# HpWang-whu/RoReg

Hardware: AMD Instinct MI355X
Metric: pair-registrations/sec (higher is better)
Workload: dtype f32 (every f32 operand enters the fp16 matrix cores as hi + lo fp16 under a per-keypoint power-of-two block scale: <= 22 significant bits relative to a CONSERVATIVE per-keypoint bound -- measured on the extractor: the bound sits 2^2..2^6 above the keypoint's true coefficient maximum (config.f16x2_sc

## Files before the change

include/roreg_hip.h:

```cpp
#ifndef ROREG_HIP_H
#define ROREG_HIP_H

#include <stdint.h>
#include <stddef.h>

#ifdef __cplusplus
extern "C" {
#endif

#define ROREG_ABI_VERSION 6
int roreg_abi_version(void);
const char *roreg_last_error(void);

int roreg_set_group_tables(const int32_t *P_host, const int32_t *Nei_host, const double *R_host);

size_t roreg_group_conv_packed_size(int Cin, int Cout, int KS);
int roreg_group_conv_pack_weights(const float *W_host , int Cin, int Cout, int KS,
                                  float *wpack_host );
size_t roreg_group_conv_workspace_size(int B, int Cin, int Cout, int Lin, int Lout, int KS);
int roreg_group_conv(const float *x, const float *wpack, const float *bias,
                     const float *bn_scale, const float *bn_shift, const float *residual,
                     float *out, const int32_t *gather,
                     int B, int Cin, int Cout, int Lin, int Lout, int KS,
                     float *workspace, size_t workspace_floats, void *stream);

int roreg_group_conv_split(const float *x, const void *wsplit, const float *bias, const float *bn_scale, const float *bn_shift,
                           float *out, const int32_t *gather,
                           const int32_t *lds_order , int lds_stride,
                           int B, int Cin, int Cout, int Lin, int Lout, int KS, void *stream);

int roreg_dense_split(const float *x, const void *wsplit, const float *bias, const float *scale, const float *shift,
                      const float *residual, int residual_stride, float *out, int B, int K, int O, void *stream);

int roreg_group_conv_f16x2(const float *x, const void *wsplit2, int w_exp, const float *bias, const float *bn_scale, const float *bn_shift,
                           float act_smax, float act_tmax, const float *in_rowmax_dev, float *out, float *out_rowmax_dev,
                           const int32_t *gather, const int32_t *lds_order , int lds_stride,
                           int B, int Cin, int Cout, int Lin, int Lout, int KS, void *stream);
int roreg_dense_f16x2(const float *x, const void *wsplit2, int w_exp, const float *bias, const float *scale, const float *shift,
                      float act_smax, float act_tmax, const float *in_rowmax_dev, const float *residual, int residual_stride, float *out,
                      float *out_rowmax_dev, int B, int K, int O, void *stream);
int roreg_group_conv_f16x2_packed(const uint32_t *x_words, const void *wsplit2, int w_exp, const float *bias, const float *in_bound_dev,
                                  float *out, float *out_rowmax_dev, const int32_t *gather, const int32_t *lds_order, int lds_stride,
                                  int B, int Cin, int Cout, int Lin, int Lout, int KS, void *stream);

int roreg_gf_finalize(const float *eqv_raw, void *eqv, int eqv_bf16 ,
                      float *inv, int B, void *stream);

int roreg_det_score(const float *enc, float *scores, int B, void *stream);

int roreg_inv_descriptor(const void *eqv, int eqv_bf16 , float *inv, int N,
                         void *stream);

int roreg_nn_search(const float *src, const int64_t *src_rows, int m,
                    const float *tgt, const int64_t *tgt_rows, int n, int F,
                    int64_t *idx_out, float *dist_out, uint64_t *scratch, void *stream);

int roreg_nn_search_ex(const float *src, const int64_t *src_rows, int m,
                       const float *tgt, const int64_t *tgt_rows, int n, int F, int squared,
                       int64_t *idx_out, float *dist_out, uint64_t *scratch, void *stream);

int roreg_pdist(const float *A, int m, const float *B, int n, int F, int squared, float *out, void *stream);

typedef struct {
    const float *desc0, *desc1;
    const int64_t *rows0, *rows1;
    int32_t m0, m1;
} roreg_match_task;
size_t roreg_mutual_match_batch_workspace(int n_tasks, int max_m);
int roreg_mutual_match_batch(const roreg_match_task *tasks_dev, int n_tasks, int max_m, int64_t *match_out, int32_t *counts_out,
                             void *workspace, size_t workspace_bytes, void *stream);

size_t roreg_knn_search_workspace(int m, int n);
int roreg_knn_search(const float *src, int m, const float *tgt, int n, int F, int k,
                     int64_t *idx_out, void *workspace , size_t workspace_bytes, void *stream);

int roreg_knn_search_ex(const float *src, int m, const float *tgt, int n, int F, int k, int squared, int64_t *idx_out, float *dist_out,
                        void *workspace, size_t workspace_bytes, void *stream);

size_t roreg_knn_search_seg_workspace(long long m_total, int n_seg, int max_m, int max_n);
int roreg_knn_search_seg(const float *src, const float *tgt, const int32_t *seg_src, const int32_t *seg_tgt, int n_seg, long long m_total,
                         int max_m, int max_n, int F, int k, int64_t *idx_out, void *workspace, size_t workspace_bytes, void *stream);

int roreg_mutual_matches(const int64_t *nn01, const int64_t *nn10, int m, int n ,
                         const int64_t *sample0, const int64_t *sample1,
                         int64_t *match_out, int32_t *count_out, void *stream);

int roreg_des2r(const float *feats1, const int64_t *rows1, const float *feats0, const int64_t *rows0,
                int M, int64_t *idx_out, float *cor_out, void *stream);

int roreg_group_corr(const float *perm_feats, const int64_t *perm_rows, const float *bcast_feats, const int64_t *bcast_rows,
                     int M, int transpose_table, int64_t *idx_out, float *cor_out, void *stream);

int roreg_group_corr_mfma(const float *perm_feats, const int64_t *perm_rows, const float *bcast_feats, const int64_t *bcast_rows, int M,
                          int transpose_table, float *cor_out, void *stream);

int roreg_set_des2r_tables(int transpose_table , const uint8_t *ia_host,
                           const uint8_t *ib_host, const uint8_t *cnt_host, const float *NT_host);
int roreg_group_corr_irrep(const float *perm_coefs, const int64_t *perm_rows, const float *bcast_coefs, const int64_t *bcast_rows, int M,
                           int transpose_table, float *cor_out, void *stream);
int roreg_des2r_irrep(const float *coef1, const int64_t *rows1, const float *coef0, const int64_t *rows0, const void *feats1,
                      const void *feats0, int feat_bf16, int M, int64_t *idx_out, void *stream);
int roreg_des2r_recheck_count(int reset, int32_t *count_out);
int roreg_feat_coefs(const void *x, int x_bf16, float *out, int B, int C, int split, void *stream);

int roreg_et_gather(const void *before0, const void *before1, const void *after0, const void *after1,
                    int feat_bf16 ,
                    const int64_t *rows0, const int64_t *rows1, const int64_t *pre_idx, int M,
                    float *x_out, void *stream);

int roreg_quat_to_trans(const float *q, const int64_t *anchor, const double *keys0, const int64_t *rows0,
                        const double *keys1, const int64_t *rows1, int M,
                        double *Trans_out, float *quat_out, void *stream);

int roreg_ransac_score(const double *k0, const double *k1, const double *w, int w_f32, int M,
                       const double *Trans, const int64_t *hyp_rows, int H, double ird,
                       double *overlap_out, int32_t *best_out, uint8_t *mask_out, void *stream);

int roreg_refine(const double *k0, const double *k1, const double *w, int w_f32, int M,
                 const double *T_in, int t_in_stride ,
                 const double *Trans, const int64_t *hyp_rows, const int32_t *best,
                 double dist, double *T_out, double *stats_out ,
                 void *stream);

typedef struct {
    const void *before0, *before1, *after0, *after1;
    const double *keys0, *keys1;
    const int64_t *matches;
    const int64_t *sel;
    int32_t n, pad_;
    int64_t off;
    const float *coef0, *coef1;
} roreg_lt_task;
int roreg_lt_prepare_batch(const roreg_lt_task *tasks_dev, int n_tasks, int max_n, int flags, int64_t *dr_out, float *x_out,
                           const float *bn_scale , const float *bn_shift, float *x_bound_out , void *stream);
int roreg_lt_finish_batch(const roreg_lt_task *tasks_dev, int n_tasks, int max_n, const float *q_all, const int64_t *dr_all,
                          double *Trans_out, void *stream);
int roreg_role_max(const void *before, const void *after, int feat_bf16, const float *bn_scale , const float *bn_shift, float *out,
                   int N, void *stream);
int roreg_row_bound_roles(const void *x_spatial, int x_bf16, float *bound_out, const float *role_scale, const float *role_shift, float *role_out, int B,
                          void *stream);
int roreg_inv_descriptor_roles(const void *eqv, int eqv_bf16, float *inv, const float *role_scale, const float *role_shift, float *role_out, int N,
                               void *stream);
int roreg_lt_prepare_rows(const roreg_lt_task *tasks_dev, const float *const *roles_dev, int n_tasks, int max_n, int flags, int64_t *dr_out,
                          uint64_t *rows_out, float *x_bound_out, void *stream);

typedef struct {
    const double *keys0, *keys1;
    const int64_t *matches;
    const double *w;
    const double *Trans;
    const int64_t *hyp_rows;
    int32_t M, H;
    int64_t koff;
} roreg_ransac_task;
size_t roreg_ransac_batch_workspace(int n_tasks, long long total_M, int max_H);
int roreg_ransac_batch(const roreg_ransac_task *tasks_dev, int n_tasks, long long total_M, int max_M, int max_H, double ird,
                       int w_f32 ,
                       int32_t *best_out, double *T1_out, double *stats1_out, double *T2_out, double *stats2_out,
                       void *workspace, size_t workspace_bytes, void *stream);

int roreg_refine_batch(const roreg_ransac_task *tasks_dev, const int32_t *sel_dev, int n_sel, long long total_M, const double *T_in,
                       double dist, int w_f32, double *T_out, double *stats_out, const void *workspace, void *stream);

int roreg_mt_shuffle_prefix(const uint32_t *seeds, int n_jobs, const int32_t *sizes, int per_job, int take, int64_t *out, int n_threads);

int roreg_mt_stream_shuffle_prefix(uint32_t *key, int32_t *pos, const int32_t *sizes, int n_lists, int take, int64_t *out);

int roreg_yohoc_draw(const uint32_t *words, long long n_words, const double *cdf, const int32_t *bin_size, int max_iter, int max_tries,
                     int32_t *bin_out, int64_t *pick_out, int32_t *n_hyp_out, long long *words_used);

typedef struct {
    const void *src;
    const int64_t *rows;
    void *dst;
    int32_t n, pad_;
} roreg_gather_task;
int roreg_gather_rows_batch(const roreg_gather_task *tasks_dev, int n_tasks, int max_n, int row_bytes, void *stream);

int roreg_gather_rows_f64(const double *src, const int64_t *rows, int M, int width, double *out, void *stream);

size_t roreg_topk_dot_workspace_size(int m, int n, int k);
int roreg_topk_dot(const float *A, int m, const float *B, int n, int k, int64_t *idx_out, float *val_out ,
                   float *ws, size_t ws_floats, const int32_t *segA, const int32_t *segB, int n_seg, int max_m, int max_n, void *stream);

int roreg_linear(const float *x, int L, int Cin, const float *W , const float *b, int Cout, float *y, void *stream);
int roreg_linear_path(int path);
int roreg_linear_cat3(const float *pos , const float *table , const int64_t *idx ,
                      const float *conf , int m, int k, const float *W , const float *b, int Cout, float *y, void *stream);
int roreg_linear_mfma(const float *x, int L, int Cin, const float *W , const float *b, int Cout, float *y, void *stream);

int roreg_instnorm_stats(const float *h, int L, int C, float eps, float *mean_rstd, double *ws, const int32_t *seg_off, int n_seg,
                         int mult, void *stream);

int roreg_mlp_tail(const float *h, int L, int Cmid, const float *mean_rstd, const float *W2 , const float *b2,
                   float *y, const int32_t *seg_off, int n_seg, int mult, void *stream);
int roreg_mlp_tail_mfma(const float *h, int L, int Cmid, const float *mean_rstd, const float *W2 , const float *b2,
                   float *y, const int32_t *seg_off, int n_seg, int mult, void *stream);

int roreg_context_colmax(const float *R, int L, const int32_t *seg_off, int n_seg, int max_len, float *ctx_out, float *ws, void *stream);

int roreg_knn_attention(const float *qp, const float *kp, const float *vp, const int64_t *idx, int k_is_table, int v_is_table,
                        int m, int k, float *x_out, void *stream);

int roreg_rm_elementwise(int op, const float *a, const float *b, const float *c, const int64_t *idx, int L, int k, int C,
                         float *out, float *ws, void *stream);

size_t roreg_sinkhorn_workspace_size(int m, int n);
int roreg_sinkhorn(const float *src_final, int m, const float *tgt_final, int n, float alpha, int iters, float *Z_out,
                   int64_t *matches0, int64_t *matches1, float *mscores0, float *mscores1, float *ws, size_t ws_floats, void *stream);

size_t roreg_sinkhorn_batch_workspace_size(int n_seg, int max_m, int max_n, long long total_m, long long total_n);
int roreg_sinkhorn_batch_consts(const int32_t *seg_src_host, const int32_t *seg_tgt_host, int n_seg, float *consts_host);
int roreg_sinkhorn_batch(const float *src_final, const float *tgt_final, const int32_t *seg_src, const int32_t *seg_tgt,
                         const int32_t *seg_src_host, const int32_t *seg_tgt_host, const float *consts, int n_seg, float alpha, int iters,
                         int64_t *matches0, int64_t *matches1, float *mscores0, float *mscores1, float *ws, size_t ws_floats,
                         void *stream);

size_t roreg_sinkhorn_batch2_workspace_size(int n_seg, int max_m, int max_n, long long total_m, long long total_n);
int roreg_sinkhorn_batch2(const float *src_final, const float *tgt_final, const int32_t *seg_src, const int32_t *seg_tgt,
                          const int32_t *seg_src_host, const int32_t *seg_tgt_host, const float *consts, int n_seg, float alpha, int iters,
                          int64_t *matches0, int64_t *matches1, float *mscores0, float *mscores1, float *ws, size_t ws_floats,
                          int recompute, void *stream);
size_t roreg_sinkhorn_batch3_workspace_size(int n_seg, int max_m, int max_n, long long total_m, long long total_n, int recompute, int want_Z);
int roreg_sinkhorn_batch3(const float *src_final, const float *tgt_final, const int32_t *seg_src, const int32_t *seg_tgt,
                          const int32_t *seg_src_host, const int32_t *seg_tgt_host, const float *consts, int n_seg, float alpha, int iters,
                          int64_t *matches0, int64_t *matches1, float *mscores0, float *mscores1, float *ws, size_t ws_floats,
                          int recompute, float *Z_out, void *stream);
int roreg_write_files(const char *const *paths, const void *const *headers, const int32_t *header_len, const void *const *data,
                      const int64_t *nbytes, int n, int n_threads);
int roreg_yohoc_draw_many(const uint32_t *seeds, int n_pairs, const int64_t *anchors, const int64_t *offsets, int max_iter, int max_tries,
                          int64_t *rows_out, int32_t *n_hyp_out, double *giveup_out, int n_threads);
size_t roreg_mlp_head_workspace(int L, int n_seg, int C1);
int roreg_mlp_head(const float *x, const float *pos, const float *table, const int64_t *idx, const float *conf, int m, int k, int L, int Cin,
                   const float *W1, const float *b1, int C1, const float *Wr, const float *br, float *h, float *y, const int32_t *seg_off,
                   int n_seg, int mult, float eps, float *mean_rstd, double *ws, void *stream);
int roreg_sinkhorn_early_exit(int on);
int roreg_sinkhorn_iteration_stats(long long *iterations, long long *pairs, int reset, void *stream);

int roreg_set_fourier_tables(const float *F_host);
size_t roreg_irrep_gemm_tiles(int O, int B, int32_t *tiles_host);
size_t roreg_irrep_gemm_tiles_m(int O, int B, int tile_m , int32_t *tiles_host);
int roreg_irrep_gemm(const float *const *X, float *const *Out, const float *const *Add, const float *const *Wpack, int C, int O, int B,
                     const int32_t *tiles_dev, int n_tiles, void *stream);
int roreg_irrep_gemm_split(const float *const *X, float *const *Out, const float *const *Add, const void *const *Wsplit, int C, int O, int B,
                           const int32_t *tiles_dev, int n_tiles, void *stream);
int roreg_irrep_gemm_f16x2(const float *const *X, float *const *Out, const float *const *Add, const void *const *Wsplit2,
                           const float *x_bound_dev, int w_exp, const float *next_u_dev, const float *next_v_dev, float *out_bound_dev,
                           int C, int O, int B, const int32_t *tiles_dev, int n_tiles,
                           int tile_m ,
                           int x_planes , void *stream);
int roreg_gemm_persistent(int on);
int roreg_row_bound(const void *x_spatial, int x_bf16 , const float *bn_scale, const float *bn_shift,
                    float *bound_out, int B, int C, void *stream);
int roreg_ft_nonlin(const float *Xin , const float *x_spatial, const float *bias,
                    const float *bias2, const float *bn_scale, const float *bn_shift, const float *resid_spatial,
                    float *Xout , float *out_spatial ,
                    const int32_t *g_map ,
                    int Lout , int Lvalid,
                    int B, int C, int split ,
                    const float *out_bound ,
                    float *out_rowmax ,
                    int spatial_bf16 ,
                    int out_planes ,
                    void *stream);
int roreg_ft_nonlin_packed(const float *Xin, const float *bias, const float *bn_scale, const float *bn_shift, uint32_t *out_words,
                           const int32_t *g_map, int Lout, int Lvalid, int B, int C, const float *out_bound, float *raw_col, int raw_g,
                           void *stream);
int roreg_ft_nonlin_gathered(const uint64_t *rows , const int64_t *dr , int feat_bf16, const float *bn_scale ,
                             const float *bn_shift, float *Xout, int B, const float *out_bound , int out_planes, void *stream);

typedef struct roreg_icp_grid_desc {
    double origin[3];
    double edge;
    int32_t dims[3];
    int32_t n;
    int64_t cells;
    int64_t reserved;
} roreg_icp_grid_desc;
size_t roreg_icp_grid_size(const double *lo_host, const double *hi_host, int n, double max_dist, roreg_icp_grid_desc *desc_host,
                           size_t *workspace_bytes);
int roreg_icp_grid_build(const float *points, const roreg_icp_grid_desc *desc_host, void *grid, void *workspace, size_t workspace_bytes,
                         void *stream);
typedef struct roreg_icp_task {
    const void *tgt_grid;
    const void *src_grid;
    const double *T0;
    int32_t n_src;
    int32_t slot0;
} roreg_icp_task;
size_t roreg_icp_batch_workspace(int n_tasks, long long total_slots);
int roreg_icp_batch(const roreg_icp_task *tasks, int n_tasks, const int32_t *work, int n_work, long long total_slots, double max_dist,
                    int max_iter, double tol_deg, double tol_t, double *T_out, int32_t *iters_out, int32_t *inliers_out, double *rmse_out,
                    int32_t *status_out, int32_t *assign_out, double *stats_out, void *workspace, size_t workspace_bytes, void *stream);

int roreg_profile_enable(int on);
int roreg_profile_read(int slot, double *total_ms, int *launches);

#ifdef __cplusplus
}
#endif
#endif
```

roreg_amd/_abi.py:

```python
import ctypes
from ctypes import c_int, c_void_p, c_size_t, c_double, c_float, c_char_p

import numpy as np

ABI_VERSION = 6

_P = c_void_p
PROTOTYPES = {
    'roreg_abi_version': (c_int, []),
    'roreg_last_error': (c_char_p, []),
    'roreg_set_group_tables': (c_int, [_P, _P, _P]),
    'roreg_group_conv_packed_size': (c_size_t, [c_int, c_int, c_int]),
    'roreg_group_conv_pack_weights': (c_int, [_P, c_int, c_int, c_int, _P]),
    'roreg_group_conv_workspace_size': (c_size_t, [c_int, c_int, c_int, c_int, c_int, c_int]),
    'roreg_group_conv': (c_int, [_P, _P, _P, _P, _P, _P, _P, _P, c_int, c_int, c_int, c_int, c_int, c_int, _P, c_size_t, _P]),
    'roreg_group_conv_split': (c_int, [_P, _P, _P, _P, _P, _P, _P, _P, c_int, c_int, c_int, c_int, c_int, c_int, c_int, _P]),
    'roreg_group_conv_f16x2': (c_int, [_P, _P, c_int, _P, _P, _P, c_float, c_float, _P, _P, _P, _P, _P, c_int, c_int, c_int, c_int, c_int, c_int, c_int, _P]),
    'roreg_group_conv_f16x2_packed': (c_int, [_P, _P, c_int, _P, _P, _P, _P, _P, _P, c_int, c_int, c_int, c_int, c_int, c_int, c_int, _P]),
    'roreg_dense_f16x2': (c_int, [_P, _P, c_int, _P, _P, _P, c_float, c_float, _P, _P, c_int, _P, _P, c_int, c_int, c_int, _P]),
    'roreg_dense_split': (c_int, [_P, _P, _P, _P, _P, _P, c_int, _P, c_int, c_int, c_int, _P]),
    'roreg_gf_finalize': (c_int, [_P, _P, c_int, _P, c_int, _P]),
    'roreg_det_score': (c_int, [_P, _P, c_int, _P]),
    'roreg_inv_descriptor': (c_int, [_P, c_int, _P, c_int, _P]),
    'roreg_nn_search': (c_int, [_P, _P, c_int, _P, _P, c_int, c_int, _P, _P, _P, _P]),
    'roreg_nn_search_ex': (c_int, [_P, _P, c_int, _P, _P, c_int, c_int, c_int, _P, _P, _P, _P]),
    'roreg_pdist': (c_int, [_P, c_int, _P, c_int, c_int, c_int, _P, _P]),
    'roreg_knn_search_workspace': (c_size_t, [c_int, c_int]),
    'roreg_knn_search': (c_int, [_P, c_int, _P, c_int, c_int, c_int, _P, _P, c_size_t, _P]),
    'roreg_knn_search_ex': (c_int, [_P, c_int, _P, c_int, c_int, c_int, c_int, _P, _P, _P, c_size_t, _P]),
    'roreg_knn_search_seg_workspace': (c_size_t, [ctypes.c_longlong, c_int, c_int, c_int]),
    'roreg_knn_search_seg': (c_int, [_P, _P, _P, _P, c_int, ctypes.c_longlong, c_int, c_int, c_int, c_int, _P, _P, c_size_t, _P]),
    'roreg_mutual_matches': (c_int, [_P, _P, c_int, c_int, _P, _P, _P, _P, _P]),
    'roreg_mutual_match_batch_workspace': (c_size_t, [c_int, c_int]),
    'roreg_mutual_match_batch': (c_int, [_P, c_int, c_int, _P, _P, _P, c_size_t, _P]),
    'roreg_des2r': (c_int, [_P, _P, _P, _P, c_int, _P, _P, _P]),
    'roreg_set_des2r_tables': (c_int, [c_int, _P, _P, _P, _P]),
    'roreg_group_corr_irrep': (c_int, [_P, _P, _P, _P, c_int, c_int, _P, _P]),
    'roreg_group_corr_mfma': (c_int, [_P, _P, _P, _P, c_int, c_int, _P, _P]),
    'roreg_des2r_irrep': (c_int, [_P, _P, _P, _P, _P, _P, c_int, c_int, _P, _P]),
    'roreg_des2r_recheck_count': (c_int, [c_int, _P]),
    'roreg_feat_coefs': (c_int, [_P, c_int, _P, c_int, c_int, c_int, _P]),
    'roreg_et_gather': (c_int, [_P, _P, _P, _P, c_int, _P, _P, _P, c_int, _P, _P]),
    'roreg_quat_to_trans': (c_int, [_P, _P, _P, _P, _P, _P, c_int, _P, _P, _P]),
    'roreg_ransac_score': (c_int, [_P, _P, _P, c_int, c_int, _P, _P, c_int, c_double, _P, _P, _P, _P]),
    'roreg_refine': (c_int, [_P, _P, _P, c_int, c_int, _P, c_int, _P, _P, _P, c_double, _P, _P, _P]),
    'roreg_lt_prepare_batch': (c_int, [_P, c_int, c_int, c_int, _P, _P, _P, _P, _P, _P]),
    'roreg_lt_finish_batch': (c_int, [_P, c_int, c_int, _P, _P, _P, _P]),
    'roreg_role_max': (c_int, [_P, _P, c_int, _P, _P, _P, c_int, _P]),
    'roreg_row_bound_roles': (c_int, [_P, c_int, _P, _P, _P, _P, c_int, _P]),
    'roreg_inv_descriptor_roles': (c_int, [_P, c_int, _P, _P, _P, _P, c_int, _P]),
    'roreg_lt_prepare_rows': (c_int, [_P, _P, c_int, c_int, c_int, _P, _P, _P, _P]),
    'roreg_ransac_batch_workspace': (c_size_t, [c_int, ctypes.c_longlong, c_int]),
    'roreg_ransac_batch': (c_int, [_P, c_int, ctypes.c_longlong, c_int, c_int, c_double, c_int, _P, _P, _P, _P, _P, _P, c_size_t, _P]),
    'roreg_refine_batch': (c_int, [_P, _P, c_int, ctypes.c_longlong, _P, ctypes.c_double, c_int, _P, _P, _P, _P]),
    'roreg_yohoc_draw': (c_int, [_P, ctypes.c_longlong, _P, _P, c_int, c_int, _P, _P, _P, _P]),
    'roreg_gather_rows_batch': (c_int, [_P, c_int, c_int, c_int, _P]),
    'roreg_gather_rows_f64': (c_int, [_P, _P, c_int, c_int, _P, _P]),
    'roreg_group_corr': (c_int, [_P, _P, _P, _P, c_int, c_int, _P, _P, _P]),
    'roreg_topk_dot_workspace_size': (c_size_t, [c_int, c_int, c_int]),
    'roreg_topk_dot': (c_int, [_P, c_int, _P, c_int, c_int, _P, _P, _P, c_size_t, _P, _P, c_int, c_int, c_int, _P]),
    'roreg_context_colmax': (c_int, [_P, c_int, _P, c_int, c_int, _P, _P, _P]),
    'roreg_sinkhorn_batch_workspace_size': (c_size_t, [c_int, c_int, c_int, ctypes.c_longlong, ctypes.c_longlong]),
    'roreg_sinkhorn_batch_consts': (c_int, [_P, _P, c_int, _P]),
    'roreg_sinkhorn_batch': (c_int, [_P, _P, _P, _P, _P, _P, _P, c_int, c_float, c_int, _P, _P, _P, _P, _P, c_size_t, _P]),
    'roreg_sinkhorn_batch2_workspace_size': (c_size_t, [c_int, c_int, c_int, ctypes.c_longlong, ctypes.c_longlong]),
    'roreg_sinkhorn_batch2': (c_int, [_P, _P, _P, _P, _P, _P, _P, c_int, c_float, c_int, _P, _P, _P, _P, _P, c_size_t, c_int, _P]),
    'roreg_sinkhorn_batch3_workspace_size': (c_size_t, [c_int, c_int, c_int, ctypes.c_longlong, ctypes.c_longlong, c_int, c_int]),
    'roreg_sinkhorn_batch3': (c_int, [_P, _P, _P, _P, _P, _P, _P, c_int, c_float, c_int, _P, _P, _P, _P, _P, c_size_t, c_int, _P, _P]),
    'roreg_write_files': (c_int, [_P, _P, _P, _P, _P, c_int, c_int]),
    'roreg_yohoc_draw_many': (c_int, [_P, c_int, _P, _P, c_int, c_int, _P, _P, _P, c_int]),
    'roreg_mlp_head_workspace': (c_size_t, [c_int, c_int, c_int]),
    'roreg_mlp_head': (c_int, [_P, _P, _P, _P, _P, c_int, c_int, c_int, c_int, _P, _P, c_int, _P, _P, _P, _P, _P, c_int, c_int, c_float, _P, _P, _P]),
    'roreg_sinkhorn_early_exit': (c_int, [c_int]),
    'roreg_sinkhorn_iteration_stats': (c_int, [_P, _P, c_int, _P]),
    'roreg_linear': (c_int, [_P, c_int, c_int, _P, _P, c_int, _P, _P]),
    'roreg_linear_mfma': (c_int, [_P, c_int, c_int, _P, _P, c_int, _P, _P]),
    'roreg_linear_path': (c_int, [c_int]),
    'roreg_linear_cat3': (c_int, [_P, _P, _P, _P, c_int, c_int, _P, _P, c_int, _P, _P]),
    'roreg_gemm_persistent': (c_int, [c_int]),
    'roreg_instnorm_stats': (c_int, [_P, c_int, c_int, c_float, _P, _P, _P, c_int, c_int, _P]),
    'roreg_mlp_tail': (c_int, [_P, c_int, c_int, _P, _P, _P, _P, _P, c_int, c_int, _P]),
    'roreg_mlp_tail_mfma': (c_int, [_P, c_int, c_int, _P, _P, _P, _P, _P, c_int, c_int, _P]),
    'roreg_knn_attention': (c_int, [_P, _P, _P, _P, c_int, c_int, c_int, c_int, _P, _P]),
    'roreg_rm_elementwise': (c_int, [c_int, _P, _P, _P, _P, c_int, c_int, c_int, _P, _P, _P]),
    'roreg_sinkhorn_workspace_size': (c_size_t, [c_int, c_int]),
    'roreg_sinkhorn': (c_int, [_P, c_int, _P, c_int, c_float, c_int, _P, _P, _P, _P, _P, _P, c_size_t, _P]),
    'roreg_icp_grid_size': (c_size_t, [_P, _P, c_int, c_double, _P, _P]),
    'roreg_icp_grid_build': (c_int, [_P, _P, _P, _P, c_size_t, _P]),
    'roreg_icp_batch_workspace': (c_size_t, [c_int, ctypes.c_longlong]),
    'roreg_icp_batch': (c_int, [_P, c_int, _P, c_int, ctypes.c_longlong, c_double, c_int, c_double, c_double, _P, _P, _P, _P, _P, _P, _P, _P, c_size_t, _P]),
    'roreg_profile_enable': (c_int, [c_int]),
    'roreg_profile_read': (c_int, [c_int, _P, _P]),
    'roreg_set_fourier_tables': (c_int, [_P]),
    'roreg_mt_shuffle_prefix': (c_int, [_P, c_int, _P, c_int, c_int, _P, c_int]),
    'roreg_mt_stream_shuffle_prefix': (c_int, [_P, _P, _P, c_int, c_int, _P]),
    'roreg_irrep_gemm_tiles': (c_size_t, [c_int, c_int, _P]),
    'roreg_irrep_gemm_tiles_m': (c_size_t, [c_int, c_int, c_int, _P]),
    'roreg_irrep_gemm': (c_int, [_P, _P, _P, _P, c_int, c_int, c_int, _P, c_int, _P]),
    'roreg_irrep_gemm_split': (c_int, [_P, _P, _P, _P, c_int, c_int, c_int, _P, c_int, _P]),
    'roreg_irrep_gemm_f16x2': (c_int, [_P, _P, _P, _P, _P, c_int, _P, _P, _P, c_int, c_int, c_int, _P, c_int, c_int, c_int, _P]),
    'roreg_row_bound': (c_int, [_P, c_int, _P, _P, _P, c_int, c_int, _P]),
    'roreg_ft_nonlin': (c_int, [_P, _P, _P, _P, _P, _P, _P, _P, _P, _P, c_int, c_int, c_int, c_int, c_int, _P, _P, c_int, c_int, _P]),
    'roreg_ft_nonlin_packed': (c_int, [_P, _P, _P, _P, _P, _P, c_int, c_int, c_int, c_int, _P, _P, c_int, _P]),
    'roreg_ft_nonlin_gathered': (c_int, [_P, _P, c_int, _P, _P, _P, c_int, _P, c_int, _P]),
}


_RANSAC_TASK = np.dtype([('keys0', np.uint64), ('keys1', np.uint64), ('matches', np.uint64), ('w', np.uint64), ('Trans', np.uint64),
                         ('hyp_rows', np.uint64), ('M', np.int32), ('H', np.int32), ('koff', np.int64)])

_MATCH_TASK = np.dtype([('desc0', np.uint64), ('desc1', np.uint64), ('rows0', np.uint64), ('rows1', np.uint64), ('m0', np.int32), ('m1', np.int32)])

_GATHER_TASK = np.dtype([('src', np.uint64), ('rows', np.uint64), ('dst', np.uint64), ('n', np.int32), ('pad', np.int32)])

_LT_TASK = np.dtype([('before0', np.uint64), ('before1', np.uint64), ('after0', np.uint64), ('after1', np.uint64), ('keys0', np.uint64),
                     ('keys1', np.uint64), ('matches', np.uint64), ('sel', np.uint64), ('n', np.int32), ('pad', np.int32), ('off', np.int64),
                     ('coef0', np.uint64), ('coef1', np.uint64)])

_ICP_GRID_DESC = np.dtype([('origin', np.float64, 3), ('edge', np.float64), ('dims', np.int32, 3), ('n', np.int32), ('cells', np.int64),
                           ('reserved', np.int64)])

_ICP_TASK = np.dtype([('tgt_grid', np.uint64), ('src_grid', np.uint64), ('T0', np.uint64), ('n_src', np.int32), ('slot0', np.int32)])
```

roreg_amd/_hip_fourier.py:

```python
import os
from ctypes import c_void_p

import numpy as np
import torch

from . import hip as _core
from .hip import HipError, _check, _feat, _ptr, _stream, lib

__all__ = ['DenseSplitLayer', 'IRREP_DIMS', 'IRREP_OFFSETS', '_bf16_split3', '_keypoint_of_columns', '_ptr_array', '_res_ptr', '_tile_cache', 'bf16_split3_frags', 'bf16_split3_pack', 'bound_exp', 'coef_pitch', 'coef_size', 'coef_views', 'dense_split', 'ensure_fourier', 'f16_scale_exp', 'f16_split2_frags', 'f16_split2_pack', 'frag_pack', 'ft_nonlin', 'ft_nonlin_gathered', 'ft_nonlin_packed', 'gemm_persistent', 'group_conv_split_pack', 'irrep_gemm', 'next_bound', 'next_bound_spatial', 'pack_coefs_f16x2', 'row_bound', 'unpack_coefs_f16x2', 'words_to_planes']


_fourier_ready = False
IRREP_DIMS = (1, 3, 3, 4, 5)
IRREP_OFFSETS = (0, 1, 10, 19, 35, 60)


def ensure_fourier():
    global _fourier_ready
    if not _fourier_ready:
        from .fourier import group_fourier
        F = np.ascontiguousarray(group_fourier().F, np.float32)
        _check(lib().roreg_set_fourier_tables(F.ctypes.data), 'roreg_set_fourier_tables')
        _fourier_ready = True


def _ptr_array(views):
    arr = (c_void_p * 5)(*[c_void_p(v.data_ptr()) for v in views])
    return arr


def coef_pitch(B):
    return (int(B) + 31) // 32 * 32


def coef_size(C, B):
    return 60 * C * coef_pitch(B)


def coef_views(buf, C, B):
    Bp = coef_pitch(B)
    return [buf[IRREP_OFFSETS[r] * C * Bp:IRREP_OFFSETS[r + 1] * C * Bp].view(IRREP_DIMS[r] * C, IRREP_DIMS[r] * Bp) for r in range(5)]


_tile_cache = {}


def irrep_gemm(X_buf, Wpacks, C, O, B, split=None, add=None, f16x2=None, x_bound=None, next_bound=None, x_planes=False):
    Bp = coef_pitch(B)
    if X_buf.numel() != 60 * C * Bp or (add is not None and add.numel() != 60 * O * Bp):
        raise HipError(f'irrep_gemm: coefficient buffers must hold 60*C*{Bp} floats (B={B} padded to the 32-keypoint pitch)')
    out = torch.empty(60 * O * Bp, dtype=torch.float32, device=X_buf.device)
    tile_m = 256 if (f16x2 is not None and O % 256 == 0 and not os.environ.get('ROREG_TILE_M128')) else 128
    key = (O, Bp, tile_m)
    t = _tile_cache.get(key)
    if t is None:
        n = lib().roreg_irrep_gemm_tiles_m(O, Bp, tile_m, None)
        host = np.empty((n, 3), np.int32)
        lib().roreg_irrep_gemm_tiles_m(O, Bp, tile_m, host.ctypes.data)
        t = torch.from_numpy(host).cuda()
        _tile_cache[key] = t
    xv = coef_views(X_buf, C, B); ov = coef_views(out, O, B)
    av = _ptr_array(coef_views(add, O, B)) if add is not None else None
    if _core.PROFILE is not None:
        e0 = torch.cuda.Event(enable_timing=True); e1 = torch.cuda.Event(enable_timing=True); e0.record()
    bound_out = None
    if f16x2 is not None:
        wl, w_exp = f16x2
        if x_bound is None or x_bound.numel() != Bp:
            raise HipError(f'irrep_gemm: the fp16 x 2 GEMM needs x_bound with one value per (padded) keypoint ({Bp})')
        nu = nv = None
        if next_bound is not None:
            nu, nv = next_bound
            if nu.numel() != O or nv.numel() != O:
                raise HipError('irrep_gemm: next_bound must hold one (u, v) per output channel')
            bound_out = torch.zeros(Bp, dtype=torch.float32, device=X_buf.device)
        _check(lib().roreg_irrep_gemm_f16x2(_ptr_array(xv), _ptr_array(ov), av, _ptr_array(wl), _ptr(x_bound, torch.float32), int(w_exp),
                                            _ptr(nu, torch.float32), _ptr(nv, torch.float32), _ptr(bound_out), C, O, Bp,
                                            _ptr(t, torch.int32), int(t.shape[0]), tile_m, (int(x_planes) if x_planes in (1, 2) and x_planes is not True else (2 if _core.MFMA16 else 1)) if x_planes else 0, _stream()), 'roreg_irrep_gemm_f16x2')
    elif split is not None:
        _check(lib().roreg_irrep_gemm_split(_ptr_array(xv), _ptr_array(ov), av, _ptr_array(split), C, O, Bp, _ptr(t, torch.int32), int(t.shape[0]),
                                            _stream()), 'roreg_irrep_gemm_split')
    else:
        _check(lib().roreg_irrep_gemm(_ptr_array(xv), _ptr_array(ov), av, _ptr_array(Wpacks), C, O, Bp, _ptr(t, torch.int32), int(t.shape[0]), _stream()),
               'roreg_irrep_gemm')
    if _core.PROFILE is not None:
        e1.record(); _core.PROFILE.append((('irrep_gemm_f16x2' if f16x2 is not None else 'irrep_gemm_split' if split is not None else 'irrep_gemm', Bp, C, O), e0, e1))
    return (out, bound_out) if next_bound is not None else out


class gemm_persistent:

    def __init__(self, on=True):
        self.on = int(on)

    def __enter__(self):
        self.prev = lib().roreg_gemm_persistent(self.on)

    def __exit__(self, *exc):
        lib().roreg_gemm_persistent(self.prev)
        return False


def row_bound(x, bn=None, roles=None):
    B, C = int(x.shape[0]), int(x.shape[1])
    out = torch.empty(coef_pitch(B), dtype=torch.float32, device=x.device)
    scale, shift = bn if bn is not None else (None, None)
    xp, bf = _feat(x)
    if roles is not None:
        if bn is not None or C != 32:
            raise HipError('row_bound: roles go with the 32-channel input features and no BatchNorm')
        r_scale, r_shift, role = _core._role_args(roles, B)
        _check(lib().roreg_row_bound_roles(xp, bf, _ptr(out), _ptr(r_scale), _ptr(r_shift), _ptr(role), B, _stream()), 'roreg_row_bound_roles')
        return out
    _check(lib().roreg_row_bound(xp, bf, _ptr(scale), _ptr(shift), _ptr(out), B, C, _stream()), 'roreg_row_bound')
    return out


def _keypoint_of_columns(d, Bp):
    n = torch.arange(d * Bp, device='cuda')
    return ((n // 32) // d) * 32 + (n % 32)


def bound_exp(bound):
    _, ex = torch.frexp(bound.float())
    e = torch.where((bound > 0) & torch.isfinite(bound), 14 - ex, torch.zeros_like(ex))
    return e.clamp(-100, 100)


def pack_coefs_f16x2(X_buf, C, B, bound=None):
    Bp = coef_pitch(B)
    views = coef_views(X_buf, C, B)
    if bound is None:
        bound = torch.zeros(Bp, dtype=torch.float32, device=X_buf.device)
        for r, v in enumerate(views):
            kp = _keypoint_of_columns(IRREP_DIMS[r], Bp)
            bound.scatter_reduce_(0, kp, v.abs().amax(0), 'amax')
    e = bound_exp(bound)
    out = torch.empty_like(X_buf)
    for r, (v, o) in enumerate(zip(views, coef_views(out, C, B))):
        kp = _keypoint_of_columns(IRREP_DIMS[r], Bp)
        y = torch.ldexp(v, e[kp][None, :])
        hi = y.half()
        lo = (y - hi.float()).half()
        w = (hi.view(torch.int16).to(torch.int32) & 0xffff) | (lo.view(torch.int16).to(torch.int32) << 16)
        o.copy_(w.view(torch.float32))
    return out, bound


def words_to_planes(X_words, C, B):
    w = X_words.contiguous().view(torch.int32).view(-1, 2, 16)
    hi = (w & 0xffff).to(torch.int16).transpose(1, 2); lo = (w >> 16).to(torch.int16).transpose(1, 2)
    return torch.cat([hi.reshape(-1, 32), lo.reshape(-1, 32)], 1).contiguous().view(torch.float32).view(-1)


def unpack_coefs_f16x2(X_words, bound, C, B):
    Bp = coef_pitch(B)
    e = bound_exp(bound)
    out = torch.empty_like(X_words)
    for r, (v, o) in enumerate(zip(coef_views(X_words, C, B), coef_views(out, C, B))):
        kp = _keypoint_of_columns(IRREP_DIMS[r], Bp)
        w = v.view(torch.int32)
        hi = (w & 0xffff).to(torch.int16).view(torch.float16).float()
        lo = (w >> 16).to(torch.int16).view(torch.float16).float()
        o.copy_(torch.ldexp(hi + lo, -e[kp][None, :]))
    return out


def next_bound_spatial(bn, bias):
    scale, shift = bn
    sc = scale.detach().double().abs().cpu(); sh = shift.detach().double().abs().cpu()
    b = bias.detach().double().cpu()
    k = 1.0 + 2.0 ** -9
    u = (np.sqrt(60.0) * k) * sc
    v = k * (sc * b.abs() + sh) + 1e-30
    return u.float().cuda().contiguous(), v.float().cuda().contiguous()


def ft_nonlin_packed(B, C, coef_in, bias, bn, out_bound, g_map=None, Lout=60, Lvalid=60, raw_g=None):
    ensure_fourier()
    dev = coef_in.device
    if coef_in.numel() != coef_size(C, B) or out_bound.numel() != coef_pitch(B):
        raise HipError('ft_nonlin_packed: coef_in / out_bound sizes')
    words = torch.empty((B, C, Lout if g_map is not None else 60), dtype=torch.int32, device=dev)
    raw = torch.empty((B, C), dtype=torch.float32, device=dev) if raw_g is not None else None
    scale, shift = bn if bn is not None else (None, None)
    _check(lib().roreg_ft_nonlin_packed(_ptr(coef_in, torch.float32), _ptr(bias), _ptr(scale), _ptr(shift), _ptr(words), _ptr(g_map, torch.int32),
                                        int(Lout), int(Lvalid), B, C, _ptr(out_bound, torch.float32), _ptr(raw), int(raw_g or 0), _stream()),
           'roreg_ft_nonlin_packed')
    return words, raw


def next_bound(bn, bias, bias2=None):
    scale, shift = bn
    sc = scale.detach().double().abs().cpu(); sh = shift.detach().double().abs().cpu()
    b = bias.detach().double().cpu() + (bias2.detach().double().cpu() if bias2 is not None else 0.0)
    k = 1.0 + 2.0 ** -9
    u = (60.0 * k) * sc
    v = (np.sqrt(60.0) * k) * (sc * b.abs() + sh) + 1e-30
    return u.float().cuda().contiguous(), v.float().cuda().contiguous()


def ft_nonlin(B, C, coef_in=None, x_spatial=None, bias=None, bias2=None, bn=None, resid_spatial=None, spatial_out=False,
              g_map=None, Lout=60, Lvalid=60, split=False, out_bound=None, want_rowmax=False, planes=False):
    ensure_fourier()
    dev = (coef_in if coef_in is not None else x_spatial).device
    if spatial_out:
        out = torch.empty((B, C, Lout if g_map is not None else 60), dtype=torch.float32, device=dev); xout = None; osp = _ptr(out)
    else:
        out = torch.empty(coef_size(C, B), dtype=torch.float32, device=dev); xout = _ptr(out); osp = None
    scale, shift = bn if bn is not None else (None, None)
    if want_rowmax and not spatial_out:
        raise HipError('ft_nonlin: want_rowmax goes with spatial_out')
    amax = torch.zeros(B, dtype=torch.float32, device=dev) if want_rowmax else None
    if coef_in is not None and coef_in.numel() != coef_size(C, B):
        raise HipError(f'ft_nonlin: coef_in must hold 60*C*{coef_pitch(B)} floats')
    if out_bound is not None and out_bound.numel() != coef_pitch(B):
        raise HipError(f'ft_nonlin: out_bound must hold one value per (padded) keypoint ({coef_pitch(B)})')
    xs, bf_x = _feat(x_spatial); rs, bf_r = _feat(resid_spatial)
    if x_spatial is not None and resid_spatial is not None and bf_x != bf_r:
        raise HipError('ft_nonlin: x_spatial and resid_spatial must share one dtype')
    _check(lib().roreg_ft_nonlin(_ptr(coef_in, torch.float32), xs, _ptr(bias),
                                 _ptr(bias2), _ptr(scale), _ptr(shift), rs, xout, osp,
                                 _ptr(g_map, torch.int32), int(Lout), int(Lvalid), B, C, 2 if split == 'f16x2' else (1 if split else 0),
                                 _ptr(out_bound, torch.float32), _ptr(amax), bf_x or bf_r, 1 if planes else 0, _stream()), 'roreg_ft_nonlin')
    return (out, amax) if want_rowmax else out


def ft_nonlin_gathered(g, bn=None, planes=False):
    ensure_fourier()
    _core.ensure_tables()
    B = g.shape[0]
    out = torch.empty(coef_size(128, B), dtype=torch.float32, device=g.rows.device)
    scale, shift = bn if bn is not None else (None, None)
    if g.bound.numel() != coef_pitch(B) or g.dr.numel() != B:
        raise HipError('ft_nonlin_gathered: rows / dr / bound sizes')
    _check(lib().roreg_ft_nonlin_gathered(_ptr(g.rows, torch.int64), _ptr(g.dr, torch.int64), 1 if g.bf16 else 0, _ptr(scale), _ptr(shift), _ptr(out), B,
                                          _ptr(g.bound, torch.float32), 1 if planes else 0, _stream()), 'roreg_ft_nonlin_gathered')
    return out


def _bf16_split3(x):
    out = []
    rem = np.ascontiguousarray(x, np.float32)
    for _ in range(3):
        u = rem.view(np.uint32)
        r = ((u >> 16) & 1) + 0x7fff
        hi = ((u + r) >> 16).astype(np.uint16)
        out.append(hi)
        rem = rem - (hi.astype(np.uint32) << 16).view(np.float32)
    return out


def f16_scale_exp(absmax):
    return 14 - int(np.frexp(float(absmax))[1]) if absmax > 0 else 0


def _f16_split2(W, w_exp):
    Ws = np.ldexp(np.ascontiguousarray(W, np.float32), w_exp).astype(np.float32)
    hi = Ws.astype(np.float16)
    return [hi.view(np.uint16), (Ws - hi.astype(np.float32)).astype(np.float16).view(np.uint16)]


def frag_pack(pieces):
    P = np.stack(pieces)
    O, K = P.shape[1:3]
    P = P.reshape(len(pieces), O, K // 16, 2, 8, *P.shape[3:])
    return np.ascontiguousarray(P.transpose(0, *range(5, P.ndim), 2, 3, 1, 4)).view(np.int16)


def f16_split2_frags(W, w_exp):
    return frag_pack(_f16_split2(W, w_exp))


def bf16_split3_frags(W):
    return frag_pack(_bf16_split3(W))


def f16_split2_pack(Wm, w_exp):
    return torch.from_numpy(f16_split2_frags(Wm, w_exp)).cuda()


def bf16_split3_pack(Wm):
    return torch.from_numpy(bf16_split3_frags(Wm)).cuda()


class DenseSplitLayer:

    @staticmethod
    def pack(W):
        O, K = np.shape(W)
        Wp = np.zeros(((O + 255) // 256 * 256, K), np.float32); Wp[:O] = W
        w_exp = f16_scale_exp(float(np.abs(Wp).max()))
        return bf16_split3_frags(Wp), f16_split2_frags(Wp, w_exp), w_exp

    def __init__(self, W, bias, scale=None, shift=None):
        self.O, self.K = np.shape(W)
        ws, ws2, self.w_exp = self.pack(W)
        self.ws = torch.from_numpy(ws).cuda()
        self.ws2 = torch.from_numpy(ws2).cuda()
        self.act_smax = float(np.abs(scale).max()) if scale is not None else 1.0
        self.act_tmax = float(np.abs(shift).max()) if shift is not None else 0.0
        self.bias = torch.from_numpy(np.ascontiguousarray(bias, np.float32)).cuda()
        self.scale = torch.from_numpy(np.ascontiguousarray(scale, np.float32)).cuda() if scale is not None else None
        self.shift = torch.from_numpy(np.ascontiguousarray(shift, np.float32)).cuda() if shift is not None else None


def _res_ptr(t):
    if t is None:
        return None
    if t.dtype != torch.float32 or not t.is_cuda:
        raise HipError('dense_split: residual must be a float32 device tensor')
    return c_void_p(t.data_ptr())


def dense_split(x, layer, residual=None, in_rowmax=None, want_rowmax=False, residual_stride=1):
    B, K = x.shape
    if K != layer.K:
        raise HipError(f'dense_split: K mismatch ({K} vs {layer.K})')
    out = torch.empty((B, layer.O), dtype=torch.float32, device=x.device)
    if in_rowmax is not None:
        if in_rowmax.numel() != B:
            raise HipError(f'dense_split: in_rowmax must hold one value per row ({B}), got {in_rowmax.numel()}')
        amax = torch.zeros(B, dtype=torch.float32, device=x.device) if want_rowmax else None
        _check(lib().roreg_dense_f16x2(_ptr(x, torch.float32), _ptr(layer.ws2), layer.w_exp, _ptr(layer.bias), _ptr(layer.scale), _ptr(layer.shift),
                                       layer.act_smax, layer.act_tmax, _ptr(in_rowmax, torch.float32), _res_ptr(residual), int(residual_stride), _ptr(out),
                                       _ptr(amax), B, K, layer.O, _stream()), 'roreg_dense_f16x2')
        return (out, amax) if want_rowmax else out
    _check(lib().roreg_dense_split(_ptr(x, torch.float32), _ptr(layer.ws), _ptr(layer.bias), _ptr(layer.scale), _ptr(layer.shift),
                                   _res_ptr(residual), int(residual_stride), _ptr(out), B, K, layer.O, _stream()), 'roreg_dense_split')
    return out


def group_conv_split_pack(W):
    Wn = W.detach().to('cpu', torch.float32).contiguous().numpy()
    return torch.from_numpy(bf16_split3_frags(Wn.reshape(Wn.shape[0], Wn.shape[1], -1))).cuda()
```

roreg_amd/csrc/fourier.hip:

```cpp
#include "common.h"
#include "primitives.h"
#include <algorithm>
#include <atomic>
#include <cmath>
#include <cstdlib>
#include <type_traits>
#include <utility>
#include <vector>

namespace {

constexpr int NIRR = 5;

struct GemmDescs {
    const float *X[NIRR];
    float *Out[NIRR];
    const float *Add[NIRR];
    const float4 *W[NIRR];
    int K[NIRR], M[NIRR], Mpad[NIRR], N[NIRR];
};

template <int CT>
__global__ __launch_bounds__(256, 2) void irrep_gemm_kernel(GemmDescs p, const int *__restrict__ tiles) {
    extern __shared__ __attribute__((aligned(16))) char smem[];
// ... 1110 lines not shown
    }
    const int wr_off = 4 * q * EP + 8 * (q >> 1);
    const int rl = lane & 15, rrow = lane >> 4;
    int e_mt = 0, e_M = 0, e_N = 0, e_dirr = 1;
    float *__restrict__ e_Out = nullptr;
    const float *__restrict__ e_Add = nullptr;
    const bool want_bound = p.out_bound != nullptr;
    int e_ncol[2];
    float osc[2][4], bm[2][4];
    auto epi_begin = [&]() {
        e_mt = mt; e_M = p.M[irr]; e_N = p.N[irr]; e_dirr = kIrrDim[irr];
        e_Out = p.Out[irr]; e_Add = p.Add[irr];
#pragma unroll
        for (int hf = 0; hf < 2; ++hf) {
            e_ncol[hf] = nt * NCOL + wb * 128 + hf * 64 + 4 * rl;
            const f32x4 xb = e_ncol[hf] < e_N ? *reinterpret_cast<const f32x4 *>(p.xbound + column_keypoint(e_ncol[hf], e_dirr)) : f32x4{0.f, 0.f, 0.f, 0.f};
#pragma unroll
            for (int e = 0; e < 4; ++e) {
                osc[hf][e] = e_ncol[hf] < e_N ? ldexpf(1.f, -(bound_exp(xb[e]) + p.w_exp)) : 1.f;
                bm[hf][e] = 0.f;
            }
        }
        if (want_bound) {
            for (int i = tid; i < OT; i += NT) {
                const int m = e_mt * OT + i;
                su[i] = m < e_M ? p.nb_u[m % p.O] : 0.f; sv[i] = m < e_M ? p.nb_v[m % p.O] : 0.f;
            }
            for (int i = tid; i < NCOL; i += NT) cm[i] = 0u;
            __syncthreads();
        }
    };
    auto epi_pass = [&](auto rb_c, auto hf_c) {
        constexpr int rb = decltype(rb_c)::value, hf = decltype(hf_c)::value;
        const bool col_ok = e_ncol[hf] < e_N;
        const int ncl = col_ok ? e_ncol[hf] : e_N - 4;
        size_t off[4];
        bool ok[4];
        f32x4 ad[4];
#pragma unroll
        for (int it = 0; it < 4; ++it) {
            const int m = e_mt * OT + wo * 64 + rb * 16 + 4 * it + rrow;
            ok[it] = m < e_M && col_ok;
            off[it] = (size_t)(m < e_M ? m : e_M - 1) * e_N + ncl;
        }
        if (e_Add) {
#pragma unroll
            for (int it = 0; it < 4; ++it) ad[it] = *reinterpret_cast<const f32x4 *>(e_Add + off[it]);
        }
#pragma unroll
        for (int cbl = 0; cbl < 4; ++cbl)
#pragma unroll
            for (int r = 0; r < 4; ++r) ebuf[wr_off + r * EP + cwl[cbl]] = acc[rb][4 * hf + cbl][r];
        f32x4 o[4];
#pragma unroll
        for (int it = 0; it < 4; ++it) {
            const f32x4 v = *reinterpret_cast<const f32x4 *>(ebuf + (4 * it + rrow) * EP + 8 * (it >> 1) + 4 * rl);
            o[it] = f32x4{v[0] * osc[hf][0], v[1] * osc[hf][1], v[2] * osc[hf][2], v[3] * osc[hf][3]};
        }
        if (e_Add) {
#pragma unroll
            for (int it = 0; it < 4; ++it) o[it] = o[it] + ad[it];
        }
#pragma unroll
        for (int it = 0; it < 4; ++it)
            if (ok[it]) *reinterpret_cast<f32x4 *>(e_Out + off[it]) = o[it];
        if (want_bound) {
#pragma unroll
            for (int it = 0; it < 4; ++it) {
                const int row = wo * 64 + rb * 16 + 4 * it + rrow;
                const float ur = su[row], vr = sv[row];
                if (ok[it]) {
#pragma unroll
                    for (int e = 0; e < 4; ++e) bm[hf][e] = fmaxf(bm[hf][e], fmaf(ur, fabsf(o[it][e]), vr));
                }
            }
        }
    };
    auto epi_end = [&]() {
        if (want_bound) {
            const int e_n0 = e_ncol[0] - (wb * 128 + 4 * rl);
#pragma unroll
            for (int hf = 0; hf < 2; ++hf)
#pragma unroll
                for (int e = 0; e < 4; ++e) {
                    float x = fmaxf(bm[hf][e], __shfl_xor(bm[hf][e], 16));
                    x = fmaxf(x, __shfl_xor(x, 32));
                    if (rrow == 0) atomicMax(cm + wb * 128 + hf * 64 + 4 * rl + e, __float_as_uint(x));
                }
            __syncthreads();
            for (int i = tid; i < NCOL; i += NT) {
                const int n = e_n0 + i;
                if (n < e_N) atomicMax(reinterpret_cast<unsigned *>(p.out_bound) + column_keypoint(n, e_dirr), cm[i]);
            }
        }
    };

    setup(); request_a(); request_b();
    for (;;) {
#pragma unroll
        for (int rb = 0; rb < 4; ++rb)
#pragma unroll
            for (int cb = 0; cb < 8; ++cb) acc[rb][cb] = f32x4{0.f, 0.f, 0.f, 0.f};
        asm volatile("s_waitcnt vmcnt(2)\n\ts_barrier" ::: "memory");
        static_for<8>([&](auto c) { read_a(0, integral_constant<int, decltype(c)::value / 2>{}, integral_constant<int, decltype(c)::value % 2>{}, aA); });
        read_b(0u, integral_constant<int, 0>{}, b0);
        asm volatile("s_waitcnt lgkmcnt(0)\n\ts_barrier" ::: "memory");
        for (int S = 0; S < nss; S += 2) {
            step(S, aA, aB);
            if (S + 1 < nss) step(S + 1, aB, aA);
        }
        asm volatile("s_waitcnt vmcnt(0) lgkmcnt(0)\n\ts_barrier" ::: "memory");
        pos += pos_step;
        int n_irr = -1, n_mt = 0, n_nt = 0;
        if (pos < longest) {
            const int *t = tiles + (size_t)(pos * 8 + stream_k) * 3;
            n_irr = t[0]; n_mt = t[1]; n_nt = t[2];
        }
        epi_begin();
        const bool more = n_irr >= 0;
        static_for<8>([&](auto ps) {
            constexpr int P = decltype(ps)::value;
            if constexpr (P == RA) {
                if (more) { irr = n_irr; mt = n_mt; nt = n_nt; setup(); request_a(); }
            }
            epi_pass(integral_constant<int, P / 2>{}, integral_constant<int, P % 2>{});
        });
        epi_end();
        __syncthreads();
        if (!more) break;
        request_b();
    }
#undef ROREG_PIN_B
}

struct NonlinParams {
    const float *Xin;
    float *Xout;
    const float *x_spatial;
    const float *r_spatial;
    float *out_spatial;
    const int *g_map;
    const float *bias, *bias2, *bn_scale, *bn_shift;
    const float *A1, *A2;
    const bf16x8 *A1s, *A2s;
    const f16x8 *A1h, *A2h;
    int f_exp;
    const float *out_bound;
    float *out_rowmax;
    int x_bf16;
    int out_planes;
    int sp_pack;
    float *raw_col;
    int raw_g;
    int B, Bp, C, tiles_per_c, Lout, Lvalid;
    const roreg::LtRow *g_rows;
    const int64_t *g_dr;
    const uint8_t *g_P8;
};

struct QRows { int alpha[64], d[64], i[64]; };
constexpr QRows make_qrows() {
    QRows t{};
    const int dims[NIRR] = {1, 3, 3, 4, 5};
    int off = 0, q = 0;
    for (int r = 0; r < NIRR; ++r) {
        for (int i = 0; i < dims[r]; ++i)
            for (int l = 0; l < dims[r]; ++l, ++q) { t.alpha[q] = off + l * dims[r]; t.d[q] = dims[r]; t.i[q] = i; }
        off += dims[r] * dims[r];
    }
    for (; q < 64; ++q) { t.alpha[q] = 0; t.d[q] = 1; t.i[q] = 0; }
    return t;
}
constexpr QRows kQ = make_qrows();

struct PairSlots {
    int qa[32], qb[32];
    int row[32];
    int i[32];
    int kind[32];
    int d[32];
    int row_alpha[16], row_d[16];
};
constexpr PairSlots make_pair_slots() {
    PairSlots t{};
    const int dims[NIRR] = {1, 3, 3, 4, 5};
    int off = 0, s = 0, row0 = 0;
    for (int r = 0; r < NIRR; ++r) {
        const int d = dims[r];
        for (int l = 0; l < d; ++l) {
            t.row_alpha[row0 + l] = off + l * d; t.row_d[row0 + l] = d;
            for (int i = d % 2; i < d; i += 2, ++s) {
                t.qa[s] = off + i * d + l; t.qb[s] = off + (i + 1) * d + l; t.row[s] = row0 + l; t.i[s] = i; t.kind[s] = 0; t.d[s] = d;
            }
        }
        if (d % 2)
            for (int l = 0; l < d; l += 2, ++s) {
                t.qa[s] = off + l; t.row[s] = row0 + l; t.i[s] = 0; t.d[s] = d;
                if (l + 1 < d) { t.qb[s] = off + l + 1; t.kind[s] = 1; } else { t.qb[s] = 64; t.kind[s] = 2; }
            }
        off += d * d; row0 += d;
    }
    return t;
}
constexpr PairSlots kPS = make_pair_slots();
constexpr int slot_out_q(int m) { const int mm = m & 31, s = (m >> 5) * 16 + (mm & 3) + 4 * (mm >> 3); return (mm & 4) ? kPS.qb[s] : kPS.qa[s]; }

template <int... I, class F>
__device__ __forceinline__ void static_for_impl(std::integer_sequence<int, I...>, F &&f) { (f(std::integral_constant<int, I>{}), ...); }
template <int N, class F>
__device__ __forceinline__ void static_for(F &&f) { static_for_impl(std::make_integer_sequence<int, N>{}, f); }

template <bool IN_SPATIAL, bool OUT_SPATIAL, int SPLIT , int NW , int MINW , bool OUT_ROWS = false, bool GATHER = false >
__global__ __launch_bounds__(NW * 64, MINW) void ft_nonlin_kernel(NonlinParams p) {
    constexpr int NT = NW * 64;
    const int lane = threadIdx.x & 63;
    const int jn = lane & 31, h = lane >> 5;
    const int wave_global = __builtin_amdgcn_readfirstlane((blockIdx.x * NT + threadIdx.x) >> 6);
    const int n_waves = gridDim.x * NW;
    const int B = p.B, C = p.C;
    const int n_tiles = C * p.tiles_per_c;

    constexpr int NPL = SPLIT == 2 ? 2 : 3;
    constexpr int NA1 = SPLIT ? 4 * 2 * NPL * 64 * 4 : 30 * 2 * 64, NA2 = SPLIT ? 4 * 2 * NPL * 64 * 4 : 32 * 2 * 64;
    __shared__ __attribute__((aligned(16))) float sA1[IN_SPATIAL ? 64 : NA1];
    __shared__ __attribute__((aligned(16))) float sA2[OUT_SPATIAL ? 64 : NA2];
    __shared__ float sT[(IN_SPATIAL || OUT_SPATIAL || OUT_ROWS) ? NW * 32 * 65 : 64];
    {
        const float *g1 = SPLIT == 3 ? reinterpret_cast<const float *>(p.A1s) : SPLIT == 2 ? reinterpret_cast<const float *>(p.A1h) : p.A1;
        const float *g2 = SPLIT == 3 ? reinterpret_cast<const float *>(p.A2s) : SPLIT == 2 ? reinterpret_cast<const float *>(p.A2h) : p.A2;
        if (!IN_SPATIAL)
            for (int i = threadIdx.x; i < NA1; i += NT) sA1[i] = g1[i];
        if (!OUT_SPATIAL)
            for (int i = threadIdx.x; i < NA2; i += NT) sA2[i] = g2[i];
    }
    __shared__ float sBias[512], sScale[512], sShift[512];
    __shared__ int sGmap[64];
    if (threadIdx.x < 64) sGmap[threadIdx.x] = (OUT_SPATIAL && p.g_map && threadIdx.x < ROREG_G) ? p.g_map[threadIdx.x] : (int)threadIdx.x;
    __shared__ uint8_t sP8[GATHER ? ROREG_G * ROREG_G : 4];
    if constexpr (GATHER)
        for (int i = threadIdx.x; i < ROREG_G * ROREG_G; i += NT) sP8[i] = p.g_P8[i];
    for (int i = threadIdx.x; i < p.C; i += NT) {
        sBias[i] = (p.bias ? p.bias[i] : 0.f) + (p.bias2 ? p.bias2[i] : 0.f);
        sScale[i] = p.bn_scale ? p.bn_scale[i] : 1.f;
        sShift[i] = p.bn_shift ? p.bn_shift[i] : 0.f;
    }
    __syncthreads();
    const bf16x8 *sA1s = reinterpret_cast<const bf16x8 *>(sA1), *sA2s = reinterpret_cast<const bf16x8 *>(sA2);
    const f16x8 *sA1h = reinterpret_cast<const f16x8 *>(sA1), *sA2h = reinterpret_cast<const f16x8 *>(sA2);
    const size_t Bp = (size_t)p.Bp;
    const size_t hmask = (size_t)0 - (size_t)h;
#define OFF_Q(Q, c, tb) ((size_t)(kQ.alpha[Q] * C + (c) * kQ.d[Q]) * Bp + (size_t)(tb) * (32 * kQ.d[Q]) + kQ.i[Q] * 32)
#define OFF_OF(Q0, Q1, c, tb) (OFF_Q(Q0, c, tb) + ((OFF_Q(Q1, c, tb) - OFF_Q(Q0, c, tb)) & hmask))
    const unsigned lane_next = (unsigned)lane * 4u;
    const unsigned lane_row3 = (unsigned)jn * 4u + (h ? 12u * (unsigned)C * (unsigned)p.Bp : 0u);
    const unsigned lane_row5 = (unsigned)jn * 4u + (h ? 20u * (unsigned)C * (unsigned)p.Bp : 0u);
    auto row_off = [&](auto rc, int c, int tb) -> size_t {
        constexpr int R = decltype(rc)::value;
        return ((size_t)(kPS.row_alpha[R] * C) + (size_t)(c * kPS.row_d[R])) * Bp + (size_t)tb * (32 * kPS.row_d[R]);
    };
    auto slot_ptr = [&](auto sc, const void *buf, int c, int tb) -> const char * {
        constexpr int S = decltype(sc)::value;
        const char *rb = reinterpret_cast<const char *>(buf) + 4 * row_off(std::integral_constant<int, kPS.row[S]>{}, c, tb) + 128 * kPS.i[S];
        return rb + (kPS.kind[S] == 1 ? (kPS.d[S] == 3 ? lane_row3 : lane_row5) : lane_next);
    };

    constexpr int NCV = IN_SPATIAL ? 32 : (SPLIT != 0 ? 32 : 30);
    constexpr bool PACK_OUT = SPLIT == 2 && !OUT_SPATIAL && !OUT_ROWS;
    auto ld_sp = [&](const float *base, size_t i) -> float {
        return p.x_bf16 ? __uint_as_float((unsigned)reinterpret_cast<const unsigned short *>(base)[i] << 16) : base[i];
    };
    float cn[NCV + 1];
    struct GDesc { unsigned lo, hi; int a; };
    auto load_desc = [&](int tile) -> GDesc {
        GDesc d{0u, 0u, 0};
        if constexpr (GATHER) {
            const int c = tile % C, tb = tile / C;
            const int row = min(tb * 32 + jn, B - 1);
            const uint2 w = *reinterpret_cast<const uint2 *>(&p.g_rows[row].src[c >> 5]);
            d.lo = w.x; d.hi = w.y;
            d.a = reinterpret_cast<const int *>(p.g_dr)[2 * (size_t)row];
        }
        return d;
    };
    auto load_rows_gathered = [&](int tile, const GDesc &d, float (&dst)[NCV + 1]) {
        if constexpr (GATHER) {
            const int c = tile % C, tb = tile / C;
            if constexpr (PACK_OUT) dst[NCV] = p.out_bound[tb * 32 + jn];
            const int cg = (c & 31) * ROREG_G, ln = lane < ROREG_G ? lane : 0;
            const bool permuted = !((c >> 5) & 1);
            auto rows = [&](auto bf16c, auto permc) {
                static_for<32>([&](auto ic) {
                    constexpr int i = decltype(ic)::value;
                    const unsigned long long base = ((unsigned long long)(unsigned)__builtin_amdgcn_readlane((int)d.hi, i) << 32) |
                                                    (unsigned)__builtin_amdgcn_readlane((int)d.lo, i);
                    int g = ln;
                    if constexpr (decltype(permc)::value) g = sP8[__builtin_amdgcn_readlane(d.a, i) * ROREG_G + ln];
                    if constexpr (decltype(bf16c)::value)
                        dst[i] = __uint_as_float(lane < ROREG_G ? (unsigned)reinterpret_cast<const unsigned short *>(base)[cg + g] : 0u);
                    else
                        dst[i] = lane < ROREG_G ? reinterpret_cast<const float *>(base)[cg + g] : 0.f;
                });
            };
            using T_ = std::true_type; using F_ = std::false_type;
            if (p.x_bf16) { if (permuted) rows(T_{}, T_{}); else rows(T_{}, F_{}); }
            else { if (permuted) rows(F_{}, T_{}); else rows(F_{}, F_{}); }
        }
    };
    auto load_coefs = [&](int tile, float (&dst)[NCV + 1]) {
        const int c = (IN_SPATIAL || OUT_SPATIAL) ? tile % C : tile / p.tiles_per_c;
        const int tb = (IN_SPATIAL || OUT_SPATIAL) ? tile / C : tile - c * p.tiles_per_c;
        if constexpr (PACK_OUT) dst[NCV] = p.out_bound[tb * 32 + jn];
        if constexpr (OUT_SPATIAL && SPLIT == 2) { if (p.sp_pack) dst[NCV] = p.out_bound[tb * 32 + jn]; }
        if constexpr (IN_SPATIAL) {
            const int b0 = tb * 32;
            if (p.x_bf16) {
                const unsigned short *xs16 = reinterpret_cast<const unsigned short *>(p.x_spatial);
                static_for<32>([&](auto ic) {
                    constexpr int i = decltype(ic)::value;
                    const size_t src = ((size_t)(b0 + i < B ? b0 + i : B - 1) * C + c) * ROREG_G;
                    dst[i] = __uint_as_float(lane < ROREG_G ? (unsigned)xs16[src + lane] : 0u);
                });
            } else {
                static_for<32>([&](auto ic) {
                    constexpr int i = decltype(ic)::value;
                    const size_t src = ((size_t)(b0 + i < B ? b0 + i : B - 1) * C + c) * ROREG_G;
                    dst[i] = lane < ROREG_G ? p.x_spatial[src + lane] : 0.f;
                });
            }
        } else if constexpr (SPLIT != 0) {
            static_for<32>([&](auto ic) {
                constexpr int st = decltype(ic)::value / 8, e = decltype(ic)::value % 8;
                constexpr int q0 = 16 * st + e, q1 = 16 * st + 8 + e;
                if constexpr (q1 < ROREG_G) dst[st * 8 + e] = __builtin_nontemporal_load(p.Xin + OFF_OF(q0, q1, c, tb) + jn);
                else dst[st * 8 + e] = __builtin_nontemporal_load(p.Xin + OFF_Q(q0, c, tb) + jn);
            });
        } else {
            static_for<30>([&](auto ic) {
                constexpr int s = decltype(ic)::value;
                constexpr int q0 = 2 * s, q1 = 2 * s + 1;
                dst[s] = p.Xin[OFF_OF(q0, q1, c, tb) + jn];
            });
        }
    };
    auto mfma6 = [&](const bf16x8 *a, const bf16x8 &b1, const bf16x8 &b2, const bf16x8 &b3, f32x16 c) {
        const bf16x8 a1 = a[0], a2 = a[64], a3 = a[128];
        c = __builtin_amdgcn_mfma_f32_32x32x16_bf16(a3, b1, c, 0, 0, 0);
        c = __builtin_amdgcn_mfma_f32_32x32x16_bf16(a2, b2, c, 0, 0, 0);
        c = __builtin_amdgcn_mfma_f32_32x32x16_bf16(a1, b3, c, 0, 0, 0);
        c = __builtin_amdgcn_mfma_f32_32x32x16_bf16(a2, b1, c, 0, 0, 0);
        c = __builtin_amdgcn_mfma_f32_32x32x16_bf16(a1, b2, c, 0, 0, 0);
        c = __builtin_amdgcn_mfma_f32_32x32x16_bf16(a1, b1, c, 0, 0, 0);
        return c;
    };
    auto mfma3 = [&](const f16x8 *a, const f16x8 &bh, const f16x8 &bl, f32x16 c) {
        const f16x8 ah = a[0], al = a[64];
        c = __builtin_amdgcn_mfma_f32_32x32x16_f16(al, bh, c, 0, 0, 0);
        c = __builtin_amdgcn_mfma_f32_32x32x16_f16(ah, bl, c, 0, 0, 0);
        c = __builtin_amdgcn_mfma_f32_32x32x16_f16(ah, bh, c, 0, 0, 0);
        return c;
    };
    auto column_scale = [&](float mx, float &xscale, float &oscale) {
        mx = fmaxf(mx, __shfl_xor(mx, 32));
        int e = 0;
        if (mx > 0.f && mx < __builtin_inff()) { int ex; (void)frexpf(mx, &ex); e = 14 - ex; }
        xscale = ldexpf(1.f, e); oscale = ldexpf(1.f, -(e + p.f_exp));
    };
    auto process = [&](int tile, int next_tile, float (&cv)[NCV + 1], float (&cnext)[NCV + 1], int next2_tile, const GDesc &dnext, GDesc &dnext2) {
        asm volatile("" ::: "memory");
        const int c = (IN_SPATIAL || OUT_SPATIAL) ? tile % C : tile / p.tiles_per_c;
        const int tbi = (IN_SPATIAL || OUT_SPATIAL) ? tile / C : tile - c * p.tiles_per_c;
        const int b = tbi * 32 + jn;
        const bool valid = b < B;
        const int bb = valid ? b : B - 1;
        f32x16 v[2];
        float wmax = 0.f;
        if (IN_SPATIAL) {
            if constexpr (GATHER) {
                dnext2 = load_desc(next2_tile);
                load_rows_gathered(next_tile, dnext, cnext);
            } else {
                load_coefs(next_tile, cnext);
            }
            __builtin_amdgcn_sched_barrier(0);
            float *ti = sT + (threadIdx.x >> 6) * (32 * 65);
#pragma unroll
            for (int i = 0; i < 32; ++i) ti[i * 65 + lane] = p.x_bf16 ? __uint_as_float(__float_as_uint(cv[i]) << 16) : cv[i];
            asm volatile("s_waitcnt lgkmcnt(0)" ::: "memory");
#pragma unroll
            for (int t = 0; t < 2; ++t)
#pragma unroll
                for (int r = 0; r < 16; ++r) {
                    const int g = t * 32 + (r & 3) + 8 * (r >> 2) + 4 * h;
                    v[t][r] = g < ROREG_G ? ti[jn * 65 + g] : 0.f;
                }
            asm volatile("s_waitcnt lgkmcnt(0)" ::: "memory");
        } else {
            load_coefs(next_tile, cnext);
            __builtin_amdgcn_sched_barrier(0);
#pragma unroll
            for (int t = 0; t < 2; ++t)
#pragma unroll
                for (int r = 0; r < 16; ++r) v[t][r] = 0.f;
            if constexpr (SPLIT == 3) {
#pragma unroll
                for (int st = 0; st < 4; ++st) {
                    float x8[8];
#pragma unroll
                    for (int e = 0; e < 8; ++e) x8[e] = (16 * st + 8 + e < ROREG_G || h == 0) ? cv[st * 8 + e] : 0.f;
                    bf16x8 b1, b2, b3;
                    split3(x8, b1, b2, b3);
                    v[0] = mfma6(sA1s + ((st * 2 + 0) * 3) * 64 + lane, b1, b2, b3, v[0]);
                    v[1] = mfma6(sA1s + ((st * 2 + 1) * 3) * 64 + lane, b1, b2, b3, v[1]);
                }
            } else if constexpr (SPLIT == 2) {
                float mx = 0.f;
#pragma unroll
                for (int s = 0; s < 32; ++s) mx = fmaxf(mx, ((16 * (s >> 3) + 8 + (s & 7) < ROREG_G || h == 0) ? fabsf(cv[s]) : 0.f));
                float xsc, osc;
                column_scale(mx, xsc, osc);
#pragma unroll
                for (int st = 0; st < 4; ++st) {
                    float x8[8];
#pragma unroll
                    for (int e = 0; e < 8; ++e) x8[e] = (16 * st + 8 + e < ROREG_G || h == 0) ? cv[st * 8 + e] : 0.f;
                    f16x8 bh, bl;
                    split2(x8, xsc, bh, bl);
                    v[0] = mfma3(sA1h + ((st * 2 + 0) * 2) * 64 + lane, bh, bl, v[0]);
                    v[1] = mfma3(sA1h + ((st * 2 + 1) * 2) * 64 + lane, bh, bl, v[1]);
                }
#pragma unroll
                for (int t = 0; t < 2; ++t)
#pragma unroll
                    for (int r = 0; r < 16; ++r) v[t][r] *= osc;
            } else {
#pragma unroll
                for (int s = 0; s < 30; ++s) {
                    v[0] = __builtin_amdgcn_mfma_f32_32x32x2f32(sA1[(s * 2 + 0) * 64 + lane], cv[s], v[0], 0, 0, 0);
                    v[1] = __builtin_amdgcn_mfma_f32_32x32x2f32(sA1[(s * 2 + 1) * 64 + lane], cv[s], v[1], 0, 0, 0);
                }
            }
        }
        const float bsum = sBias[c];
        const bool bn = p.bn_scale != nullptr;
        const float sc = sScale[c], sh = sShift[c];
        const bool has_rs = OUT_SPATIAL && p.r_spatial;
        const bool rs_late = has_rs && !bn && !p.g_map && !p.out_rowmax;
        const size_t rs = ((size_t)bb * C + c) * ROREG_G;
        float *tb = (OUT_SPATIAL || OUT_ROWS) ? sT + (threadIdx.x >> 6) * (32 * 65) : nullptr;
        const bool sp_pack = OUT_SPATIAL && SPLIT == 2 && p.sp_pack;
        const float pk_scale = sp_pack ? ldexpf(1.f, bound_exp(cv[NCV])) : 1.f;
#pragma unroll
        for (int t = 0; t < 2; ++t)
#pragma unroll
            for (int r = 0; r < 16; ++r) {
                const int g = t * 32 + (r & 3) + 8 * (r >> 2) + 4 * h;
                float x = v[t][r] + bsum;
                if (OUT_SPATIAL && has_rs && !rs_late && g < ROREG_G) x += ld_sp(p.r_spatial, rs + g);
                if (sp_pack && p.raw_col && g == p.raw_g && valid) p.raw_col[(size_t)bb * C + c] = x;
                if (bn) x = fmaxf(fmaf(x, sc, sh), 0.f);
                if (g >= ROREG_G || !valid) x = 0.f;
                v[t][r] = x;
                if (OUT_SPATIAL && g < ROREG_G) {
                    const int go = sGmap[g];
                    if (go >= 0) {
                        if (sp_pack) {
                            const float xs = x * pk_scale;
                            const _Float16 h1 = (_Float16)xs;
                            const _Float16 l1 = (_Float16)(xs - (float)h1);
                            tb[jn * 65 + go] = __uint_as_float((unsigned)__builtin_bit_cast(unsigned short, h1) | ((unsigned)__builtin_bit_cast(unsigned short, l1) << 16));
                        } else {
                            tb[jn * 65 + go] = x; wmax = fmaxf(wmax, fabsf(x));
                        }
                    }
                }
            }
        if (OUT_SPATIAL) {
            asm volatile("s_waitcnt lgkmcnt(0)" ::: "memory");
            const int b0 = tbi * 32;
            if (b0 + 32 <= B) {
                float *ob = p.out_spatial + ((size_t)b0 * C + c) * p.Lout + lane;
                const size_t ostep = (size_t)C * p.Lout;
                const size_t rb = ((size_t)b0 * C + c) * ROREG_G + (lane < ROREG_G ? lane : 0), rstep = (size_t)C * ROREG_G;
                const unsigned short *r16 = reinterpret_cast<const unsigned short *>(p.r_spatial);
#pragma unroll
                for (int g8 = 0; g8 < 4; ++g8) {
                    float tv[8], rv[8];
#pragma unroll
                    for (int q = 0; q < 8; ++q) tv[q] = tb[(g8 * 8 + q) * 65 + lane];
                    if (rs_late) {
                        if (p.x_bf16) {
#pragma unroll
                            for (int q = 0; q < 8; ++q) rv[q] = __uint_as_float((unsigned)r16[rb + (size_t)(g8 * 8 + q) * rstep]);
#pragma unroll
                            for (int q = 0; q < 8; ++q) tv[q] += __uint_as_float(__float_as_uint(rv[q]) << 16);
                        } else {
#pragma unroll
                            for (int q = 0; q < 8; ++q) rv[q] = p.r_spatial[rb + (size_t)(g8 * 8 + q) * rstep];
#pragma unroll
                            for (int q = 0; q < 8; ++q) tv[q] += rv[q];
                        }
                    }
#pragma unroll
                    for (int q = 0; q < 8; ++q)
                        if (lane < p.Lout) ob[(size_t)(g8 * 8 + q) * ostep] = lane < p.Lvalid ? tv[q] : 0.f;
                }
            } else {
                for (int bl = 0; bl < 32 && b0 + bl < B; ++bl)
                    if (lane < p.Lout) {
                        float tv = tb[bl * 65 + lane];
                        if (rs_late && lane < ROREG_G) tv += ld_sp(p.r_spatial, ((size_t)(b0 + bl) * C + c) * ROREG_G + lane);
                        p.out_spatial[((size_t)(b0 + bl) * C + c) * p.Lout + lane] = lane < p.Lvalid ? tv : 0.f;
                    }
            }
            asm volatile("s_waitcnt lgkmcnt(0)" ::: "memory");
            if (p.out_rowmax) {
                wmax = fmaxf(wmax, __shfl_xor(wmax, 32));
                atomicMax(reinterpret_cast<unsigned *>(p.out_rowmax) + bb, __float_as_uint(valid ? wmax : 0.f));
            }
        }
        if (!OUT_SPATIAL) {
            f32x16 o[2];
#pragma unroll
            for (int t = 0; t < 2; ++t)
#pragma unroll
                for (int r = 0; r < 16; ++r) o[t][r] = 0.f;
            if constexpr (SPLIT == 3) {
#pragma unroll
                for (int st = 0; st < 4; ++st) {
                    float x8[8];
#pragma unroll
                    for (int e = 0; e < 8; ++e) x8[e] = v[st >> 1][8 * (st & 1) + e];
                    bf16x8 b1, b2, b3;
                    split3(x8, b1, b2, b3);
                    o[0] = mfma6(sA2s + ((st * 2 + 0) * 3) * 64 + lane, b1, b2, b3, o[0]);
                    o[1] = mfma6(sA2s + ((st * 2 + 1) * 3) * 64 + lane, b1, b2, b3, o[1]);
                }
            } else if constexpr (SPLIT == 2) {
                float mx = 0.f;
#pragma unroll
                for (int t = 0; t < 2; ++t)
#pragma unroll
                    for (int r = 0; r < 16; ++r) mx = fmaxf(mx, fabsf(v[t][r]));
                float xsc, osc;
                column_scale(mx, xsc, osc);
#pragma unroll
                for (int st = 0; st < 4; ++st) {
                    float x8[8];
#pragma unroll
                    for (int e = 0; e < 8; ++e) x8[e] = v[st >> 1][8 * (st & 1) + e];
                    f16x8 bh, bl;
                    split2(x8, xsc, bh, bl);
                    o[0] = mfma3(sA2h + ((st * 2 + 0) * 2) * 64 + lane, bh, bl, o[0]);
                    o[1] = mfma3(sA2h + ((st * 2 + 1) * 2) * 64 + lane, bh, bl, o[1]);
                }
                if constexpr (PACK_OUT) {
                    const float psc = osc * ldexpf(1.f, bound_exp(cv[NCV]));
#pragma unroll
                    for (int t = 0; t < 2; ++t)
#pragma unroll
                        for (int r = 0; r < 16; ++r) {
                            const float x = o[t][r] * psc;
                            const _Float16 h1 = (_Float16)x;
                            const _Float16 l1 = (_Float16)(x - (float)h1);
                            o[t][r] = __uint_as_float((unsigned)__builtin_bit_cast(unsigned short, h1) | ((unsigned)__builtin_bit_cast(unsigned short, l1) << 16));
                        }
                } else {
#pragma unroll
                    for (int t = 0; t < 2; ++t)
#pragma unroll
                        for (int r = 0; r < 16; ++r) o[t][r] *= osc;
                }
            } else {
#pragma unroll
                for (int t = 0; t < 2; ++t)
#pragma unroll
                    for (int r = 0; r < 16; ++r) {
                        const int s = t * 16 + r;
                        o[0] = __builtin_amdgcn_mfma_f32_32x32x2f32(sA2[(s * 2 + 0) * 64 + lane], v[t][r], o[0], 0, 0, 0);
                        o[1] = __builtin_amdgcn_mfma_f32_32x32x2f32(sA2[(s * 2 + 1) * 64 + lane], v[t][r], o[1], 0, 0, 0);
                    }
            }
            if constexpr (OUT_ROWS) {
#pragma unroll
                for (int t = 0; t < 2; ++t)
#pragma unroll
                    for (int r = 0; r < 16; ++r) {
                        const int qq = h ? kPS.qb[t * 16 + r] : kPS.qa[t * 16 + r];
                        if (qq < ROREG_G) tb[jn * 65 + qq] = o[t][r];
                    }
                asm volatile("s_waitcnt lgkmcnt(0)" ::: "memory");
                const int b0 = tbi * 32;
                if (b0 + 32 <= B) {
                    float *ob = p.out_spatial + ((size_t)b0 * C + c) * ROREG_G + lane;
                    const size_t ostep = (size_t)C * ROREG_G;
#pragma unroll
                    for (int g8 = 0; g8 < 4; ++g8) {
                        float tv[8];
#pragma unroll
                        for (int q = 0; q < 8; ++q) tv[q] = tb[(g8 * 8 + q) * 65 + lane];
#pragma unroll
                        for (int q = 0; q < 8; ++q)
                            if (lane < ROREG_G) ob[(size_t)(g8 * 8 + q) * ostep] = tv[q];
                    }
                } else {
                    for (int bl = 0; bl < 32 && b0 + bl < B; ++bl)
                        if (lane < ROREG_G) p.out_spatial[((size_t)(b0 + bl) * C + c) * ROREG_G + lane] = tb[bl * 65 + lane];
                }
                asm volatile("s_waitcnt lgkmcnt(0)" ::: "memory");
            } else if (PACK_OUT && p.out_planes) {
                const int tb = tbi;
                const unsigned sel = (jn & 16) ? 0x07060302u : 0x05040100u;
                static_for<32>([&](auto ic) {
                    constexpr int S = decltype(ic)::value, t = S / 16, r = S % 16;
                    const unsigned own = __float_as_uint(o[t][r]);
                    const auto pr = __builtin_amdgcn_permlane16_swap(own, own, false, false);
                    const unsigned word = __builtin_amdgcn_perm(pr[1], pr[0], sel);
                    unsigned *dst = reinterpret_cast<unsigned *>(const_cast<char *>(slot_ptr(ic, p.Xout, c, tb)));
                    if (kPS.kind[S] != 2 || h == 0) __builtin_nontemporal_store(word, dst);
                });
            } else {
                const int tb = tbi;
                static_for<32>([&](auto ic) {
                    constexpr int S = decltype(ic)::value, t = S / 16, r = S % 16;
                    float *dst = reinterpret_cast<float *>(const_cast<char *>(slot_ptr(ic, p.Xout, c, tb)));
                    if (kPS.kind[S] != 2 || h == 0) __builtin_nontemporal_store(o[t][r], dst);
                });
            }
        }
    };
// ... 299 lines not shown
    if (tile_m == 256)
        return launch_gemm_split<2, 4>("roreg_irrep_gemm_f16x2", X, Out, Add, Wsplit2, x_bound_dev, w_exp, next_u_dev, next_v_dev, out_bound_dev, C, O, B,
                                       tiles_dev, n_tiles, stream, x_planes);
    return launch_gemm_split<2, 2>("roreg_irrep_gemm_f16x2", X, Out, Add, Wsplit2, x_bound_dev, w_exp, next_u_dev, next_v_dev, out_bound_dev, C, O, B,
                                   tiles_dev, n_tiles, stream);
}

__global__ __launch_bounds__(256) void row_bound_kernel(const float *__restrict__ x, int x_bf16, const float *__restrict__ bn_scale,
                                                        const float *__restrict__ bn_shift, float *__restrict__ bound, int B, int Bp, int C) {
    const int b = blockIdx.x * 4 + (threadIdx.x >> 6), lane = threadIdx.x & 63;
    if (b >= Bp) return;
    float mx = 0.f;
    if (b < B) {
        const size_t row = (size_t)b * C * ROREG_G;
        for (int i = lane; i < C * ROREG_G; i += 64) {
            float v = x_bf16 ? __uint_as_float((unsigned)reinterpret_cast<const unsigned short *>(x)[row + i] << 16) : x[row + i];
            if (bn_scale) { const int c = i / ROREG_G; v = fmaxf(fmaf(v, bn_scale[c], bn_shift[c]), 0.f); }
            mx = fmaxf(mx, fabsf(v));
        }
#pragma unroll
        for (int o = 32; o > 0; o >>= 1) mx = fmaxf(mx, __shfl_xor(mx, o));
    }
    if (lane == 0) bound[b] = mx * 7.7536f;
}

__global__ __launch_bounds__(256) void row_bound_roles_kernel(const float *__restrict__ x, int x_bf16, float *__restrict__ bound, int B, int Bp,
                                                              const float *__restrict__ role_scale, const float *__restrict__ role_shift,
                                                              float *__restrict__ role_out) {
    const int b = blockIdx.x * 4 + (threadIdx.x >> 6), lane = threadIdx.x & 63;
    if (b >= Bp) return;
    float mx = 0.f, m1 = 0.f, m0 = 0.f;
    if (b < B) {
        const size_t row = (size_t)b * ROREG_F * ROREG_G;
        for (int i = lane; i < ROREG_F * ROREG_G; i += 64) {
            const float v = x_bf16 ? __uint_as_float((unsigned)reinterpret_cast<const unsigned short *>(x)[row + i] << 16) : x[row + i];
            const int c = i / ROREG_G;
            mx = fmaxf(mx, fabsf(v));
            m1 = fmaxf(m1, fmaxf(fmaf(v, role_scale[c], role_shift[c]), 0.f));
            m0 = fmaxf(m0, fmaxf(fmaf(v, role_scale[ROREG_F + c], role_shift[ROREG_F + c]), 0.f));
        }
#pragma unroll
        for (int o = 32; o > 0; o >>= 1) { mx = fmaxf(mx, __shfl_xor(mx, o)); m1 = fmaxf(m1, __shfl_xor(m1, o)); m0 = fmaxf(m0, __shfl_xor(m0, o)); }
        if (lane == 0) { role_out[(size_t)b * 4] = m1; role_out[(size_t)b * 4 + 1] = m0; }
    }
    if (lane == 0) bound[b] = mx * 7.7536f;
}

extern "C" int roreg_row_bound_roles(const void *x_spatial, int x_bf16, float *bound_out, const float *role_scale, const float *role_shift, float *role_out,
                                     int B, void *stream) {
    ROREG_REQUIRE(x_spatial && bound_out && role_scale && role_shift && role_out && B > 0, "roreg_row_bound_roles: bad arguments");
    const int Bp = (B + 31) / 32 * 32;
    hipLaunchKernelGGL(row_bound_roles_kernel, dim3((Bp + 3) / 4), dim3(256), 0, roreg::as_stream(stream), reinterpret_cast<const float *>(x_spatial), x_bf16, bound_out,
                       B, Bp, role_scale, role_shift, role_out);
    ROREG_CHECK_LAUNCH("roreg_row_bound_roles");
    return 0;
}

extern "C" int roreg_row_bound(const void *x_spatial, int x_bf16, const float *bn_scale, const float *bn_shift, float *bound_out, int B, int C,
                               void *stream) {
    ROREG_REQUIRE(x_spatial && bound_out && B > 0 && C > 0, "roreg_row_bound: bad arguments");
    ROREG_REQUIRE((bn_scale == nullptr) == (bn_shift == nullptr), "roreg_row_bound: bn_scale and bn_shift go together");
    const int Bp = (B + 31) / 32 * 32;
    hipLaunchKernelGGL(row_bound_kernel, dim3((Bp + 3) / 4), dim3(256), 0, roreg::as_stream(stream), reinterpret_cast<const float *>(x_spatial), x_bf16, bn_scale, bn_shift,
                       bound_out, B, Bp, C);
    ROREG_CHECK_LAUNCH("roreg_row_bound");
    return 0;
}

template <void (*KERN)(NonlinParams)>
static void launch_ft(const NonlinParams &p, long long n_tiles, hipStream_t s) {
    static const int resident = [] {
        int per_cu = 0, dev = 0, cus = 256;
        if (hipOccupancyMaxActiveBlocksPerMultiprocessor(&per_cu, KERN, 256, 0) != hipSuccess || per_cu < 1) per_cu = 2;
        if (hipGetDevice(&dev) == hipSuccess) (void)hipDeviceGetAttribute(&cus, hipDeviceAttributeMultiprocessorCount, dev);
        return per_cu * cus;
    }();
    static const int rounds = [] { const char *e = getenv("ROREG_FT_ROUNDS"); const int r = e ? atoi(e) : 0; return r > 0 ? r : 4; }();
    const long long want = (n_tiles + 3) / 4, cap = (long long)resident * rounds;
    hipLaunchKernelGGL(KERN, dim3((unsigned)(want > cap ? cap : want)), dim3(256), 0, s, p);
}

extern "C" int roreg_ft_nonlin(const float *Xin, const float *x_spatial, const float *bias, const float *bias2,
                               const float *bn_scale, const float *bn_shift, const float *resid_spatial, float *Xout, float *out_spatial,
                               const int32_t *g_map, int Lout, int Lvalid, int B, int C, int split, const float *out_bound, float *out_rowmax,
                               int spatial_bf16, int out_planes, void *stream) {
    ROREG_REQUIRE(g_A1 && g_A2, "roreg_ft_nonlin: roreg_set_fourier_tables has not been called");
    ROREG_REQUIRE((Xin != nullptr) != (x_spatial != nullptr), "roreg_ft_nonlin: exactly one of Xin / x_spatial");
    ROREG_REQUIRE((Xout != nullptr) != (out_spatial != nullptr), "roreg_ft_nonlin: exactly one of Xout / out_spatial");
    ROREG_REQUIRE((bn_scale == nullptr) == (bn_shift == nullptr) && B > 0 && C > 0 && C <= 512, "roreg_ft_nonlin: bad arguments (C <= 512)");
    ROREG_REQUIRE((long long)60 * C * B < (1ll << 40), "roreg_ft_nonlin: tensor too large");
    ROREG_REQUIRE(!g_map || (Lout >= Lvalid && Lvalid > 0 && Lout <= 64), "roreg_ft_nonlin: bad Lout/Lvalid");
    NonlinParams p;
    memset(&p, 0, sizeof(p));
    p.Xin = Xin; p.Xout = Xout;
    p.x_spatial = x_spatial; p.r_spatial = resid_spatial; p.out_spatial = out_spatial;
    p.g_map = g_map; p.Lout = g_map ? Lout : ROREG_G; p.Lvalid = g_map ? Lvalid : ROREG_G;
    p.bias = bias; p.bias2 = bias2; p.bn_scale = bn_scale; p.bn_shift = bn_shift; p.A1 = g_A1; p.A2 = g_A2;
    p.A1s = reinterpret_cast<const bf16x8 *>(g_A1s); p.A2s = reinterpret_cast<const bf16x8 *>(g_A2s); p.out_bound = out_bound; p.out_rowmax = out_rowmax; p.x_bf16 = spatial_bf16;
    p.A1h = reinterpret_cast<const f16x8 *>(g_A1h); p.A2h = reinterpret_cast<const f16x8 *>(g_A2h); p.f_exp = g_f_exp;
    p.B = B; p.Bp = (B + 31) / 32 * 32; p.C = C; p.tiles_per_c = (B + 31) / 32;
    p.out_planes = out_planes;
    ROREG_REQUIRE((unsigned long long)C * p.Bp * 20ull < (1ull << 32), "roreg_ft_nonlin: C * round_up(B, 32) must stay below 2^32 / 20 (32-bit lane offsets)");
    ROREG_REQUIRE(!out_planes || (split == 2 && Xout), "roreg_ft_nonlin: out_planes is a layout of the fp16 x 2 coefficient output");
    const long long n_tiles = (long long)C * p.tiles_per_c;
    hipStream_t s = roreg::as_stream(stream);
    roreg::ProfScope prof(roreg::PROF_FT_NONLIN, s);
    const bool in_sp = x_spatial != nullptr, out_sp = out_spatial != nullptr;
    if (in_sp && out_sp) { roreg::set_error("roreg_ft_nonlin: spatial -> spatial is not a transform"); return 2; }
    ROREG_REQUIRE(split != 2 || out_sp || out_bound, "roreg_ft_nonlin: split = 2 writes the coefficients as fp16 hi/lo pairs and needs out_bound");
    ROREG_REQUIRE(!spatial_bf16 || in_sp || resid_spatial, "roreg_ft_nonlin: spatial_bf16 refers to x_spatial / resid_spatial");
    ROREG_REQUIRE(!out_rowmax || out_sp, "roreg_ft_nonlin: out_rowmax goes with a group-domain output");
    ROREG_REQUIRE(split >= 0 && split <= 2, "roreg_ft_nonlin: split must be 0 (f32 MFMA), 1 (bf16 x 3) or 2 (fp16 x 2)");
    if (split == 2) {
        if (in_sp) launch_ft<ft_nonlin_kernel<true, false, 2, 4, 1>>(p, n_tiles, s);
        else if (!out_sp) launch_ft<ft_nonlin_kernel<false, false, 2, 4, 1>>(p, n_tiles, s);
        else launch_ft<ft_nonlin_kernel<false, true, 2, 4, 1>>(p, n_tiles, s);
    } else if (split == 1) {
        if (in_sp) launch_ft<ft_nonlin_kernel<true, false, 3, 4, 1>>(p, n_tiles, s);
        else if (!out_sp) launch_ft<ft_nonlin_kernel<false, false, 3, 4, 1>>(p, n_tiles, s);
        else launch_ft<ft_nonlin_kernel<false, true, 3, 4, 1>>(p, n_tiles, s);
    } else {
        if (in_sp) launch_ft<ft_nonlin_kernel<true, false, 0, 4, 1>>(p, n_tiles, s);
        else if (!out_sp) launch_ft<ft_nonlin_kernel<false, false, 0, 4, 1>>(p, n_tiles, s);
        else launch_ft<ft_nonlin_kernel<false, true, 0, 4, 1>>(p, n_tiles, s);
    }
    ROREG_CHECK_LAUNCH("roreg_ft_nonlin");
    return 0;
}

extern "C" int roreg_ft_nonlin_packed(const float *Xin, const float *bias, const float *bn_scale, const float *bn_shift, uint32_t *out_words,
                                      const int32_t *g_map, int Lout, int Lvalid, int B, int C, const float *out_bound, float *raw_col, int raw_g,
                                      void *stream) {
    ROREG_REQUIRE(g_A1 && g_A2, "roreg_ft_nonlin_packed: roreg_set_fourier_tables has not been called");
    ROREG_REQUIRE(Xin && out_words && out_bound && B > 0 && C > 0 && C <= 512 && (bn_scale == nullptr) == (bn_shift == nullptr), "roreg_ft_nonlin_packed: bad arguments");
    ROREG_REQUIRE(!g_map || (Lout >= Lvalid && Lvalid > 0 && Lout <= 64), "roreg_ft_nonlin_packed: bad Lout/Lvalid");
    ROREG_REQUIRE(!raw_col || (raw_g >= 0 && raw_g < ROREG_G), "roreg_ft_nonlin_packed: raw_g out of range");
    NonlinParams p;
    memset(&p, 0, sizeof(p));
    p.Xin = Xin; p.out_spatial = reinterpret_cast<float *>(out_words);
    p.g_map = g_map; p.Lout = g_map ? Lout : ROREG_G; p.Lvalid = g_map ? Lvalid : ROREG_G;
    p.bias = bias; p.bn_scale = bn_scale; p.bn_shift = bn_shift; p.A1 = g_A1; p.A2 = g_A2;
    p.A1s = reinterpret_cast<const bf16x8 *>(g_A1s); p.A2s = reinterpret_cast<const bf16x8 *>(g_A2s);
    p.A1h = reinterpret_cast<const f16x8 *>(g_A1h); p.A2h = reinterpret_cast<const f16x8 *>(g_A2h); p.f_exp = g_f_exp;
    p.out_bound = out_bound; p.sp_pack = 1; p.raw_col = raw_col; p.raw_g = raw_g;
    p.B = B; p.Bp = (B + 31) / 32 * 32; p.C = C; p.tiles_per_c = (B + 31) / 32;
    ROREG_REQUIRE((unsigned long long)C * p.Bp * 20ull < (1ull << 32), "roreg_ft_nonlin_packed: C * round_up(B, 32) must stay below 2^32 / 20 (32-bit lane offsets)");
    hipStream_t s = roreg::as_stream(stream);
    roreg::ProfScope prof(roreg::PROF_FT_NONLIN, s);
    launch_ft<ft_nonlin_kernel<false, true, 2, 4, 1>>(p, (long long)C * p.tiles_per_c, s);
    ROREG_CHECK_LAUNCH("roreg_ft_nonlin_packed");
    return 0;
}

extern "C" int roreg_ft_nonlin_gathered(const uint64_t *rows, const int64_t *dr, int feat_bf16, const float *bn_scale, const float *bn_shift, float *Xout,
                                        int B, const float *out_bound, int out_planes, void *stream) {
    ROREG_REQUIRE(g_A1 && g_A2, "roreg_ft_nonlin_gathered: roreg_set_fourier_tables has not been called");
    ROREG_REQUIRE(roreg::group_tables().ready, "roreg_ft_nonlin_gathered: group tables not set");
    ROREG_REQUIRE(rows && dr && Xout && out_bound && B > 0 && (bn_scale == nullptr) == (bn_shift == nullptr), "roreg_ft_nonlin_gathered: bad arguments");
    constexpr int C = 4 * ROREG_F;
    ROREG_REQUIRE((long long)60 * C * B < (1ll << 40), "roreg_ft_nonlin_gathered: tensor too large");
    NonlinParams p;
    memset(&p, 0, sizeof(p));
    p.Xout = Xout; p.Lout = ROREG_G; p.Lvalid = ROREG_G;
    p.bn_scale = bn_scale; p.bn_shift = bn_shift; p.A1 = g_A1; p.A2 = g_A2;
    p.A1s = reinterpret_cast<const bf16x8 *>(g_A1s); p.A2s = reinterpret_cast<const bf16x8 *>(g_A2s);
    p.A1h = reinterpret_cast<const f16x8 *>(g_A1h); p.A2h = reinterpret_cast<const f16x8 *>(g_A2h); p.f_exp = g_f_exp;
    p.out_bound = out_bound; p.x_bf16 = feat_bf16; p.out_planes = out_planes;
    p.g_rows = reinterpret_cast<const roreg::LtRow *>(rows); p.g_dr = dr; p.g_P8 = roreg::group_tables().P8;
    p.B = B; p.Bp = (B + 31) / 32 * 32; p.C = C; p.tiles_per_c = (B + 31) / 32;
    ROREG_REQUIRE((unsigned long long)C * p.Bp * 20ull < (1ull << 32), "roreg_ft_nonlin_gathered: 128 * round_up(B, 32) must stay below 2^32 / 20 (32-bit lane offsets)");
    hipStream_t s = roreg::as_stream(stream);
    roreg::ProfScope prof(roreg::PROF_FT_NONLIN, s);
    launch_ft<ft_nonlin_kernel<true, false, 2, 4, 1, false, true>>(p, (long long)C * p.tiles_per_c, s);
    ROREG_CHECK_LAUNCH("roreg_ft_nonlin_gathered");
    return 0;
}

extern "C" int roreg_feat_coefs(const void *x, int x_bf16, float *out, int B, int C, int split, void *stream) {
    if (B == 0) return 0;
    ROREG_REQUIRE(g_A1 && g_A2, "roreg_feat_coefs: roreg_set_fourier_tables has not been called");
    ROREG_REQUIRE(x && out && B > 0 && C > 0 && C <= 512 && split >= 0 && split <= 2, "roreg_feat_coefs: bad arguments");
    NonlinParams p;
    memset(&p, 0, sizeof(p));
    p.x_spatial = reinterpret_cast<const float *>(x); p.x_bf16 = x_bf16; p.out_spatial = out;
    p.Lout = ROREG_G; p.Lvalid = ROREG_G; p.A1 = g_A1; p.A2 = g_A2;
    p.A1s = reinterpret_cast<const bf16x8 *>(g_A1s); p.A2s = reinterpret_cast<const bf16x8 *>(g_A2s);
    p.A1h = reinterpret_cast<const f16x8 *>(g_A1h); p.A2h = reinterpret_cast<const f16x8 *>(g_A2h); p.f_exp = g_f_exp;
    p.B = B; p.Bp = (B + 31) / 32 * 32; p.C = C; p.tiles_per_c = (B + 31) / 32;
    const long long n_tiles = (long long)C * p.tiles_per_c;
    hipStream_t s = roreg::as_stream(stream);
    if (split == 2) launch_ft<ft_nonlin_kernel<true, false, 2, 4, 1, true>>(p, n_tiles, s);
    else if (split == 1) launch_ft<ft_nonlin_kernel<true, false, 3, 4, 1, true>>(p, n_tiles, s);
    else launch_ft<ft_nonlin_kernel<true, false, 0, 4, 1, true>>(p, n_tiles, s);
    ROREG_CHECK_LAUNCH("roreg_feat_coefs");
    return 0;
}
```

roreg_amd/csrc/group_conv.hip:

```cpp
#include "common.h"
#include "primitives.h"
#include <type_traits>


namespace {

struct GCParams {
    const float *x;
    const float4 *wp;
    const float *bias;
    const float *bn_scale;
    const float *bn_shift;
    const float *residual;
    float *out;
    const int32_t *gather;
    float *partial;
    int B, Cin, Cout, CoutPad, Lout, ncols, gt_bytes;
    int ksplit, cin_per_slice;
};

template <int KS, int LIN, int CT, int WO, int WB, int OTW>
__global__ __launch_bounds__(256, 2) void group_conv_kernel(GCParams p) {
    extern __shared__ __attribute__((aligned(16))) char smem[];
    int *gt = reinterpret_cast<int *>(smem);
// ... 33 lines not shown
    for (int a = 0; a < OTW; ++a)
#pragma unroll
        for (int t = 0; t < 4; ++t)
#pragma unroll
            for (int r = 0; r < 16; ++r) acc[a][t][r] = 0.f;

    const bool has_bn = p.bn_scale != nullptr;

    const int c_begin = blockIdx.y * p.cin_per_slice, c_end = c_begin + p.cin_per_slice;
    for (int c0 = c_begin; c0 < c_end; c0 += CT) {
        __syncthreads();
        if constexpr (LIN % 4 == 0) {
            constexpr int PER_KP4 = CT * LIN / 4;
            const int total4 = nkp * PER_KP4;
            const float4 *x4 = reinterpret_cast<const float4 *>(p.x);
            float4 *xs4 = reinterpret_cast<float4 *>(xs);
            for (int i = tid; i < total4; i += 256) {
                const int kp = i / PER_KP4, e4 = i - kp * PER_KP4;
                const int c = (e4 * 4) / LIN;
                float4 v = x4[((size_t)(b_first + kp) * p.Cin + c0) * (LIN / 4) + e4];
                if (has_bn) {
                    const float s = p.bn_scale[c0 + c], sh = p.bn_shift[c0 + c];
                    v.x = fmaxf(fmaf(v.x, s, sh), 0.f);
                    v.y = fmaxf(fmaf(v.y, s, sh), 0.f);
                    v.z = fmaxf(fmaf(v.z, s, sh), 0.f);
                    v.w = fmaxf(fmaf(v.w, s, sh), 0.f);
                }
                xs4[i] = v;
            }
        } else {
            constexpr int PER_KP = CT * LIN;
            const int total = nkp * PER_KP;
            for (int i = tid; i < total; i += 256) {
                const int kp = i / PER_KP, e = i - kp * PER_KP;
                const int c = e / LIN;
                float v = p.x[((size_t)(b_first + kp) * p.Cin + c0) * LIN + e];
                if (has_bn) v = fmaxf(fmaf(v, p.bn_scale[c0 + c], p.bn_shift[c0 + c]), 0.f);
                xs[i] = v;
            }
        }
        __syncthreads();

        constexpr int NQ = CT / 8;
        float4 a_cur[NQ][OTW], a_nxt[NQ][OTW];
        auto load_a = [&](int k, float4 (&a)[NQ][OTW]) {
            const float4 *wk = p.wp + ((size_t)(k * (p.Cin / 8) + c0 / 8) * p.CoutPad + o_wave + j) * 2 + h;
#pragma unroll
            for (int q = 0; q < NQ; ++q)
#pragma unroll
                for (int ot = 0; ot < OTW; ++ot) a[q][ot] = wk[((size_t)q * p.CoutPad + ot * 32) * 2];
        };
        load_a(0, a_cur);
#pragma unroll 1
        for (int k = 0; k < KS; ++k) {
            if (k + 1 < KS) load_a(k + 1, a_nxt);
            int off[4];
#pragma unroll
            for (int t = 0; t < 4; ++t) off[t] = rowbase[t] + gt[gi[t] * KS + k];
#pragma unroll
            for (int q = 0; q < NQ; ++q) {
#pragma unroll
                for (int r = 0; r < 4; ++r) {
                    float bv[4];
#pragma unroll
                    for (int t = 0; t < 4; ++t) bv[t] = xs[off[t] + (q * 8 + r * 2) * LIN];
#pragma unroll
                    for (int ot = 0; ot < OTW; ++ot) {
                        const float av = r == 0 ? a_cur[q][ot].x : r == 1 ? a_cur[q][ot].y : r == 2 ? a_cur[q][ot].z : a_cur[q][ot].w;
#pragma unroll
                        for (int t = 0; t < 4; ++t)
                            acc[ot][t] = __builtin_amdgcn_mfma_f32_32x32x2f32(av, bv[t], acc[ot][t], 0, 0, 0);
                    }
                }
            }
            if (k + 1 < KS) {
#pragma unroll
                for (int q = 0; q < NQ; ++q)
#pragma unroll
                    for (int ot = 0; ot < OTW; ++ot) a_cur[q][ot] = a_nxt[q][ot];
            }
        }
    }

    if (p.ksplit > 1) {
        float *part = p.partial + (size_t)blockIdx.y * ((size_t)p.B * p.Cout * p.Lout);
#pragma unroll
        for (int ot = 0; ot < OTW; ++ot) {
#pragma unroll
            for (int t = 0; t < 4; ++t) {
                if (!valid[t]) continue;
#pragma unroll
                for (int r = 0; r < 16; ++r) {
                    const int o = o_wave + ot * 32 + (r & 3) + 8 * (r >> 2) + 4 * h;
                    if (o < p.Cout) part[((size_t)bcol[t] * p.Cout + o) * p.Lout + gi[t]] = acc[ot][t][r];
                }
            }
        }
        return;
    }
#pragma unroll
    for (int ot = 0; ot < OTW; ++ot) {
#pragma unroll
        for (int t = 0; t < 4; ++t) {
            if (!valid[t]) continue;
#pragma unroll
            for (int r = 0; r < 16; ++r) {
                const int o = o_wave + ot * 32 + (r & 3) + 8 * (r >> 2) + 4 * h;
                if (o < p.Cout) {
                    const size_t idx = ((size_t)bcol[t] * p.Cout + o) * p.Lout + gi[t];
                    float v = acc[ot][t][r] + p.bias[o];
                    if (p.residual) v += p.residual[idx];
                    p.out[idx] = v;
                }
            }
        }
    }
}

__global__ __launch_bounds__(256) void splitk_reduce_kernel(const float *__restrict__ partial, const float *__restrict__ bias,
                                                            const float *__restrict__ residual, float *__restrict__ out,
                                                            size_t n, int Cout, int Lout, int ksplit) {
    const size_t i = (size_t)blockIdx.x * 256 + threadIdx.x;
    if (i >= n) return;
    const int o = (int)((i / Lout) % Cout);
    float v = 0.f;
    for (int s = 0; s < ksplit; ++s) v += partial[(size_t)s * n + i];
    v += bias[o];
    if (residual) v += residual[i];
    out[i] = v;
}


struct SplitScale {
    const float *in_rowmax;
    float act_smax, act_tmax;
    int w_exp;
    float *out_rowmax;
};
__device__ __forceinline__ int row_scale_exp(const SplitScale &q, int b) {
    return bound_exp(q.act_smax * q.in_rowmax[b] + q.act_tmax);
}

struct GCSplitParams {
    const float *x;
    const void *ws;
    const float *bias, *bn_scale, *bn_shift;
    float *out;
    const int32_t *gather;
    int B, Cin, Cout, CoutPad, Lin, Lout, ncols, gt_bytes, nkp_max;
    SplitScale sc;
    const int32_t *order;
    int S;
    int packed;
};

template <int KS, int NP, int PK = 0>
__global__ __launch_bounds__(256, 2) void group_conv_split_kernel(GCSplitParams p) {
    constexpr bool PACKED = PK != 0;
    static_assert(!PACKED || NP == 2, "packed input words are fp16 hi / lo pairs");
    using frag = typename std::conditional<NP == 3, bf16x8, f16x8>::type;
    extern __shared__ __attribute__((aligned(16))) char smem[];
    int *gt = reinterpret_cast<int *>(smem);
    frag *slab = reinterpret_cast<frag *>(smem + p.gt_bytes);
    constexpr int OT = 256, NCOL = 128;
    const int tid = threadIdx.x, lane = tid & 63, w = tid >> 6;
    const int j = lane & 31, h = lane >> 5;
    const int Lin = p.Lin, Lout = p.Lout;
    const int n_ot = p.CoutPad / OT;
    const int ot_idx = blockIdx.x % n_ot, ct_idx = blockIdx.x / n_ot;
    const int o_wave = ot_idx * OT + w * 64;
    const int col0 = ct_idx * NCOL;
    const int b_first = col0 / Lout;
    const int col_last = min(col0 + NCOL, p.ncols) - 1;
    const int nkp = col_last / Lout - b_first + 1;
    const int S = p.S;
    const int plane_stride = 2 * p.nkp_max * S, h_stride = p.nkp_max * S;
    int *slot_of = gt + Lout * KS;

    const bool has_bn = p.bn_scale != nullptr;
    for (int i = tid; i < Lout * KS; i += 256) gt[i] = p.order ? p.order[p.gather[i]] : p.gather[i];
    for (int i = tid; i < Lin; i += 256) slot_of[i] = p.order ? p.order[i] : i;

    int rowbase[4], gi[4], bcol[4];
    bool valid[4];
#pragma unroll
    for (int t = 0; t < 4; ++t) {
        const int n = col0 + t * 32 + j;
        valid[t] = n < p.ncols;
        const int nn = valid[t] ? n : col0;
        const int b = nn / Lout;
        gi[t] = nn - b * Lout;
        bcol[t] = b;
        rowbase[t] = h * h_stride + (b - b_first) * S;
    }

    f32x16 acc[2][4];
#pragma unroll
    for (int a = 0; a < 2; ++a)
#pragma unroll
        for (int t = 0; t < 4; ++t)
#pragma unroll
            for (int r = 0; r < 16; ++r) acc[a][t][r] = 0.f;

    float oscale[4] = {1.f, 1.f, 1.f, 1.f};
    if constexpr (NP == 2) {
#pragma unroll
        for (int t = 0; t < 4; ++t) oscale[t] = ldexpf(1.f, -(row_scale_exp(p.sc, bcol[t]) + p.sc.w_exp));
    }
    const frag *wsb = reinterpret_cast<const frag *>(p.ws);
    const size_t ws_plane = (size_t)KS * (p.Cin / 16) * 2 * p.CoutPad;

    float *raw = reinterpret_cast<float *>(slab + (size_t)NP * plane_stride);
    const int raw_floats = p.nkp_max * 16 * Lin;
    float *bn_s = raw + raw_floats, *bn_h = bn_s + p.Cin, *kp_scale = bn_h + p.Cin;
    for (int i = tid; i < p.Cin; i += 256) { bn_s[i] = has_bn ? p.bn_scale[i] : 1.f; bn_h[i] = has_bn ? p.bn_shift[i] : 0.f; }
    if constexpr (NP == 2)
        for (int i = tid; i < nkp; i += 256) kp_scale[i] = ldexpf(1.f, row_scale_exp(p.sc, b_first + i));
    const int pieces = nkp * 4 * Lin;
    constexpr int RAW_ITERS = 9;
    int raw_off[RAW_ITERS];
#pragma unroll
    for (int q = 0; q < RAW_ITERS; ++q) {
        const int pc = w * 64 + q * 256 + lane;
        raw_off[q] = -1;
        if (pc < pieces) {
            const int kp = pc / (4 * Lin), r = pc - kp * (4 * Lin);
            raw_off[q] = ((b_first + kp) * p.Cin) * Lin + 4 * r;
        }
    }
    auto issue_raw = [&](int c0) {
        const float *xc = p.x + (size_t)c0 * Lin;
        float *dst0 = raw + (size_t)(w * 64) * 4;
#pragma unroll
        for (int q = 0; q < RAW_ITERS; ++q) {
            if (w * 64 + q * 256 < pieces) {
                if (raw_off[q] >= 0)
                    __builtin_amdgcn_global_load_lds((const __attribute__((address_space(1))) void *)(xc + raw_off[q]),
                                                     (__attribute__((address_space(3))) void *)(dst0 + (size_t)q * 1024), 16, 0, 0);
            }
        }
    };
    constexpr int CV_ITEMS = 5;
    int cv_src[CV_ITEMS], cv_dst[CV_ITEMS];
    {
        const int items = nkp * 2 * Lin;
#pragma unroll
        for (int q = 0; q < CV_ITEMS; ++q) {
            const int i = tid + q * 256;
            cv_src[q] = -1; cv_dst[q] = 0;
            if (i < items) {
                const int col = i % Lin, r = i / Lin;
                const int ho = r & 1, kp = r >> 1;
                const int sl = p.order ? p.order[col] : col;
                if (sl >= 0) { cv_src[q] = (kp * 16 + 8 * ho) * Lin + col; cv_dst[q] = ho * h_stride + kp * S + sl; }
            }
        }
    }
    auto cv_load = [&](int q, unsigned (&wv)[8]) {
        if (cv_src[q] < 0) return;
        const float *src = raw + cv_src[q];
#pragma unroll
        for (int e = 0; e < 8; ++e) wv[e] = __float_as_uint(src[e * Lin]);
    };
    auto cv_store = [&](int q, const unsigned (&wv)[8]) {
        if (cv_src[q] < 0) return;
        unsigned hw[4], lw[4];
#pragma unroll
        for (int e = 0; e < 4; ++e) {
            hw[e] = __builtin_amdgcn_perm(wv[2 * e + 1], wv[2 * e], 0x05040100u);
            lw[e] = __builtin_amdgcn_perm(wv[2 * e + 1], wv[2 * e], 0x07060302u);
        }
        struct Q4 { unsigned a, b, c, d; };
        frag *dst = slab + cv_dst[q];
        dst[0] = __builtin_bit_cast(frag, Q4{hw[0], hw[1], hw[2], hw[3]});
        dst[plane_stride] = __builtin_bit_cast(frag, Q4{lw[0], lw[1], lw[2], lw[3]});
    };
    auto convert_packed = [&]() {
#pragma unroll
        for (int q = 0; q < CV_ITEMS; ++q) {
            unsigned wv[8];
            cv_load(q, wv);
            cv_store(q, wv);
        }
    };
    auto convert_float = [&](int c0) {
        const int items = nkp * 2 * Lin;
        for (int i = tid; i < items; i += 256) {
            const int col = i % Lin, r = i / Lin;
            const int ho = r & 1, kp = r >> 1;
            const int sl = slot_of[col];
            if (sl < 0) continue;
            const float *src = raw + (kp * 16 + 8 * ho) * Lin + col;
            float v[8];
#pragma unroll
            for (int e = 0; e < 8; ++e) v[e] = src[e * Lin];
            if (has_bn) {
                const float4 *sc4 = reinterpret_cast<const float4 *>(bn_s + c0 + 8 * ho), *sh4 = reinterpret_cast<const float4 *>(bn_h + c0 + 8 * ho);
                const float4 s0 = sc4[0], s1 = sc4[1], h0 = sh4[0], h1 = sh4[1];
                const float scv[8] = {s0.x, s0.y, s0.z, s0.w, s1.x, s1.y, s1.z, s1.w}, shv[8] = {h0.x, h0.y, h0.z, h0.w, h1.x, h1.y, h1.z, h1.w};
#pragma unroll
                for (int e = 0; e < 8; ++e) v[e] = fmaxf(fmaf(v[e], scv[e], shv[e]), 0.f);
            }
            frag *dst = slab + ho * h_stride + kp * S + sl;
            if constexpr (NP == 3) {
                bf16x8 b1, b2, b3;
                split3(v, b1, b2, b3);
                dst[0] = b1; dst[plane_stride] = b2; dst[2 * plane_stride] = b3;
            } else {
                f16x8 hi, lo;
                split2(v, kp_scale[kp], hi, lo);
                dst[0] = hi; dst[plane_stride] = lo;
            }
        }
    };
    auto convert = [&](int c0) {
        if constexpr (PACKED) convert_packed(); else convert_float(c0);
    };
    issue_raw(0);
    asm volatile("s_waitcnt vmcnt(0)" ::: "memory");
    __syncthreads();
    convert(0);
    int gix0[4];
#pragma unroll
    for (int t = 0; t < 4; ++t) gix0[t] = gt[gi[t] * KS];

    for (int c0 = 0; c0 < p.Cin; c0 += 16) {
        const bool more = c0 + 16 < p.Cin;
        __syncthreads();
        const frag *slab_cur = slab;

        frag aw[2][2][NP];
        auto load_a = [&](int k, frag (&a)[2][NP]) {
            const frag *wk = wsb + (((size_t)k * (p.Cin / 16) + c0 / 16) * 2 + h) * p.CoutPad + o_wave + j;
#pragma unroll
            for (int ot = 0; ot < 2; ++ot)
#pragma unroll
                for (int sp = 0; sp < NP; ++sp) a[ot][sp] = wk[sp * ws_plane + ot * 32];
        };
        load_a(0, aw[0]);
        int gix[2][4];
        frag fb[2][NP];
#pragma unroll
        for (int t = 0; t < 4; ++t) gix[0][t] = gix0[t];
        auto read_frags = [&](int slot, int t, int set) {
            const frag *bp = slab_cur + rowbase[t] + slot;
#pragma unroll
            for (int sp = 0; sp < NP; ++sp) fb[set][sp] = bp[sp * plane_stride];
        };
        read_frags(gix[0][0], 0, 0);
#pragma unroll
        for (int k = 0; k < KS; ++k) {
            const frag (&a_cur)[2][NP] = aw[k & 1];
            if (k + 1 < KS) load_a(k + 1, aw[(k + 1) & 1]);
            if (k == 0 && more) issue_raw(c0 + 16);
            if (k + 1 < KS) {
#pragma unroll
                for (int t = 0; t < 4; ++t) gix[(k + 1) & 1][t] = gt[gi[t] * KS + k + 1];
            }
            __builtin_amdgcn_sched_barrier(0);
#pragma unroll
            for (int t = 0; t < 4; ++t) {
                const int s = k * 4 + t;
                if (t < 3) read_frags(gix[k & 1][t + 1], t + 1, (s + 1) & 1);
                else if (k + 1 < KS) read_frags(gix[(k + 1) & 1][0], 0, (s + 1) & 1);
                __builtin_amdgcn_sched_barrier(0);
                const frag (&f)[NP] = fb[s & 1];
                f32x16 c0v = acc[0][t], c1v = acc[1][t];
                if constexpr (NP == 3) {
                    const bf16x8 b1 = f[0], b2 = f[1], b3 = f[2];
                    c0v = __builtin_amdgcn_mfma_f32_32x32x16_bf16(a_cur[0][2], b1, c0v, 0, 0, 0);
                    c1v = __builtin_amdgcn_mfma_f32_32x32x16_bf16(a_cur[1][2], b1, c1v, 0, 0, 0);
                    c0v = __builtin_amdgcn_mfma_f32_32x32x16_bf16(a_cur[0][1], b2, c0v, 0, 0, 0);
                    c1v = __builtin_amdgcn_mfma_f32_32x32x16_bf16(a_cur[1][1], b2, c1v, 0, 0, 0);
                    c0v = __builtin_amdgcn_mfma_f32_32x32x16_bf16(a_cur[0][0], b3, c0v, 0, 0, 0);
                    c1v = __builtin_amdgcn_mfma_f32_32x32x16_bf16(a_cur[1][0], b3, c1v, 0, 0, 0);
                    c0v = __builtin_amdgcn_mfma_f32_32x32x16_bf16(a_cur[0][1], b1, c0v, 0, 0, 0);
                    c1v = __builtin_amdgcn_mfma_f32_32x32x16_bf16(a_cur[1][1], b1, c1v, 0, 0, 0);
                    c0v = __builtin_amdgcn_mfma_f32_32x32x16_bf16(a_cur[0][0], b2, c0v, 0, 0, 0);
                    c1v = __builtin_amdgcn_mfma_f32_32x32x16_bf16(a_cur[1][0], b2, c1v, 0, 0, 0);
                    c0v = __builtin_amdgcn_mfma_f32_32x32x16_bf16(a_cur[0][0], b1, c0v, 0, 0, 0);
                    c1v = __builtin_amdgcn_mfma_f32_32x32x16_bf16(a_cur[1][0], b1, c1v, 0, 0, 0);
                } else {
                    const f16x8 bh = f[0], bl = f[1];
                    c0v = __builtin_amdgcn_mfma_f32_32x32x16_f16(a_cur[0][1], bh, c0v, 0, 0, 0);
                    c1v = __builtin_amdgcn_mfma_f32_32x32x16_f16(a_cur[1][1], bh, c1v, 0, 0, 0);
                    c0v = __builtin_amdgcn_mfma_f32_32x32x16_f16(a_cur[0][0], bl, c0v, 0, 0, 0);
                    c1v = __builtin_amdgcn_mfma_f32_32x32x16_f16(a_cur[1][0], bl, c1v, 0, 0, 0);
                    c0v = __builtin_amdgcn_mfma_f32_32x32x16_f16(a_cur[0][0], bh, c0v, 0, 0, 0);
                    c1v = __builtin_amdgcn_mfma_f32_32x32x16_f16(a_cur[1][0], bh, c1v, 0, 0, 0);
                }
                acc[0][t] = c0v; acc[1][t] = c1v;
                __builtin_amdgcn_sched_barrier(0);
            }
        }
        if (more) {
            asm volatile("s_waitcnt vmcnt(0)" ::: "memory");
            __syncthreads();
            convert(c0 + 16);
        }
    }

    float wmax[4] = {0.f, 0.f, 0.f, 0.f};
    float bv[2][16];
#pragma unroll
    for (int ot = 0; ot < 2; ++ot)
#pragma unroll
        for (int r = 0; r < 16; ++r) {
            const int o = o_wave + ot * 32 + (r & 3) + 8 * (r >> 2) + 4 * h;
            bv[ot][r] = o < p.Cout ? p.bias[o] : 0.f;
        }
#pragma unroll
    for (int ot = 0; ot < 2; ++ot) {
#pragma unroll
        for (int t = 0; t < 4; ++t) {
            if (!valid[t]) continue;
#pragma unroll
            for (int r = 0; r < 16; ++r) {
                const int o = o_wave + ot * 32 + (r & 3) + 8 * (r >> 2) + 4 * h;
                if (o < p.Cout) {
                    const float v = (NP == 2 ? acc[ot][t][r] * oscale[t] : acc[ot][t][r]) + bv[ot][r];
                    p.out[((size_t)bcol[t] * p.Cout + o) * Lout + gi[t]] = v;
                    wmax[t] = fmaxf(wmax[t], fabsf(v));
                }
            }
        }
    }
    if constexpr (NP == 2) {
        if (p.sc.out_rowmax) {
#pragma unroll
            for (int t = 0; t < 4; ++t) {
                const float m = fmaxf(wmax[t], __shfl_xor(wmax[t], 32));
                if (h == 0 && valid[t]) atomicMax(reinterpret_cast<unsigned *>(p.sc.out_rowmax) + bcol[t], __float_as_uint(m));
            }
        }
    }
}

struct DenseParams {
    const float *x;
    const void *ws;
    const float *bias;
    const float *scale, *shift;
    const float *res;
    int res_stride;
    float *out;
    int B, K, O, Opad;
    SplitScale sc;
};

template <int NP>
__global__ __launch_bounds__(256, 2) void dense_split_kernel(DenseParams p) {
    using frag = typename std::conditional<NP == 3, bf16x8, f16x8>::type;
    extern __shared__ __attribute__((aligned(16))) char smem[];
    constexpr int TB = 128, TO = 256;
    constexpr int XBUF = NP * 2 * TB, WBUF = NP * 2 * TO;
    frag *xs = reinterpret_cast<frag *>(smem);
    frag *wsm = xs + 2 * XBUF;
    const int tid = threadIdx.x, lane = tid & 63, w = tid >> 6;
    const int j = lane & 31, h = lane >> 5;
    const int wr = w & 1, wc = w >> 1;
    const int n_ot = p.Opad / TO;
    const int ot = blockIdx.x % n_ot, bt = blockIdx.x / n_ot;
    const int b0 = bt * TB, o0 = ot * TO;
    const int nsteps = p.K / 16;
    const size_t wplane = (size_t)nsteps * 2 * p.Opad;
    const frag *wsb = reinterpret_cast<const frag *>(p.ws);

    f32x16 acc[2][4];
#pragma unroll
    for (int a = 0; a < 2; ++a)
#pragma unroll
        for (int t = 0; t < 4; ++t)
#pragma unroll
            for (int r = 0; r < 16; ++r) acc[a][t][r] = 0.f;

    const int srow = tid >> 1, sho = tid & 1;
    int brow = b0 + srow;
    if (brow >= p.B) brow = p.B - 1;
    const float *xrow = p.x + (size_t)brow * p.K + 8 * sho;
    float xscale = 1.f;
    if constexpr (NP == 2) xscale = ldexpf(1.f, row_scale_exp(p.sc, brow));
    const bool has_act = p.scale != nullptr;
    float4 xa, xb, s0, s1, t0, t1;
    auto load_x = [&](int ks) {
        const int kk = (ks < nsteps ? ks : nsteps - 1) * 16;
        xa = *reinterpret_cast<const float4 *>(xrow + kk);
        xb = *reinterpret_cast<const float4 *>(xrow + kk + 4);
        if (has_act) {
            const int kq = kk + 8 * sho;
            s0 = *reinterpret_cast<const float4 *>(p.scale + kq); s1 = *reinterpret_cast<const float4 *>(p.scale + kq + 4);
            t0 = *reinterpret_cast<const float4 *>(p.shift + kq); t1 = *reinterpret_cast<const float4 *>(p.shift + kq + 4);
        }
    };
    auto convert_store = [&](int ks, int buf) {
        float v[8] = {xa.x, xa.y, xa.z, xa.w, xb.x, xb.y, xb.z, xb.w};
        if (has_act) {
            const float sc[8] = {s0.x, s0.y, s0.z, s0.w, s1.x, s1.y, s1.z, s1.w}, sh[8] = {t0.x, t0.y, t0.z, t0.w, t1.x, t1.y, t1.z, t1.w};
#pragma unroll
            for (int e = 0; e < 8; ++e) v[e] = fmaxf(fmaf(v[e], sc[e], sh[e]), 0.f);
        }
        frag *dst = xs + buf * XBUF + sho * TB + srow;
        if constexpr (NP == 3) {
            bf16x8 b1, b2, b3;
            split3(v, b1, b2, b3);
            dst[0] = b1; dst[2 * TB] = b2; dst[4 * TB] = b3;
        } else {
            f16x8 hi, lo;
            split2(v, xscale, hi, lo);
            dst[0] = hi; dst[2 * TB] = lo;
        }
    };
    auto issue_w = [&](int ks, int buf) {
        const frag *q = wsb + (size_t)(ks < nsteps ? ks : nsteps - 1) * 2 * p.Opad + o0;
#pragma unroll
        for (int sp = 0; sp < NP; ++sp)
#pragma unroll
            for (int ho = 0; ho < 2; ++ho)
                __builtin_amdgcn_global_load_lds((const __attribute__((address_space(1))) void *)(q + sp * wplane + (size_t)ho * p.Opad + tid),
                                                 (__attribute__((address_space(3))) void *)(wsm + buf * WBUF + sp * (2 * TO) + ho * TO + w * 64), 16, 0, 0);
    };

    load_x(0);
    issue_w(0, 0);
    convert_store(0, 0);
    asm volatile("s_waitcnt vmcnt(0)" ::: "memory");
    __syncthreads();
    int buf = 0;
    for (int ks = 0; ks < nsteps; ++ks) {
        issue_w(ks + 1, buf ^ 1);
        load_x(ks + 1);
        __builtin_amdgcn_sched_barrier(0);
        const frag *xt = xs + buf * XBUF + h * TB + wr * 64 + j;
        const frag *wt = wsm + buf * WBUF + h * TO + wc * 128 + j;
        frag a[2][NP];
#pragma unroll
        for (int rt = 0; rt < 2; ++rt)
#pragma unroll
            for (int sp = 0; sp < NP; ++sp) a[rt][sp] = xt[sp * (2 * TB) + rt * 32];
#pragma unroll
        for (int t = 0; t < 4; ++t) {
            f32x16 c0 = acc[0][t], c1 = acc[1][t];
            if constexpr (NP == 3) {
                const bf16x8 b1 = wt[t * 32], b2 = wt[2 * TO + t * 32], b3 = wt[4 * TO + t * 32];
                c0 = __builtin_amdgcn_mfma_f32_32x32x16_bf16(a[0][2], b1, c0, 0, 0, 0);
                c1 = __builtin_amdgcn_mfma_f32_32x32x16_bf16(a[1][2], b1, c1, 0, 0, 0);
                c0 = __builtin_amdgcn_mfma_f32_32x32x16_bf16(a[0][1], b2, c0, 0, 0, 0);
                c1 = __builtin_amdgcn_mfma_f32_32x32x16_bf16(a[1][1], b2, c1, 0, 0, 0);
                c0 = __builtin_amdgcn_mfma_f32_32x32x16_bf16(a[0][0], b3, c0, 0, 0, 0);
                c1 = __builtin_amdgcn_mfma_f32_32x32x16_bf16(a[1][0], b3, c1, 0, 0, 0);
                c0 = __builtin_amdgcn_mfma_f32_32x32x16_bf16(a[0][1], b1, c0, 0, 0, 0);
                c1 = __builtin_amdgcn_mfma_f32_32x32x16_bf16(a[1][1], b1, c1, 0, 0, 0);
                c0 = __builtin_amdgcn_mfma_f32_32x32x16_bf16(a[0][0], b2, c0, 0, 0, 0);
                c1 = __builtin_amdgcn_mfma_f32_32x32x16_bf16(a[1][0], b2, c1, 0, 0, 0);
                c0 = __builtin_amdgcn_mfma_f32_32x32x16_bf16(a[0][0], b1, c0, 0, 0, 0);
                c1 = __builtin_amdgcn_mfma_f32_32x32x16_bf16(a[1][0], b1, c1, 0, 0, 0);
            } else {
                const f16x8 wh = wt[t * 32], wl = wt[2 * TO + t * 32];
                c0 = __builtin_amdgcn_mfma_f32_32x32x16_f16(a[0][1], wh, c0, 0, 0, 0);
                c1 = __builtin_amdgcn_mfma_f32_32x32x16_f16(a[1][1], wh, c1, 0, 0, 0);
                c0 = __builtin_amdgcn_mfma_f32_32x32x16_f16(a[0][0], wl, c0, 0, 0, 0);
                c1 = __builtin_amdgcn_mfma_f32_32x32x16_f16(a[1][0], wl, c1, 0, 0, 0);
                c0 = __builtin_amdgcn_mfma_f32_32x32x16_f16(a[0][0], wh, c0, 0, 0, 0);
                c1 = __builtin_amdgcn_mfma_f32_32x32x16_f16(a[1][0], wh, c1, 0, 0, 0);
            }
            acc[0][t] = c0; acc[1][t] = c1;
        }
        __builtin_amdgcn_sched_barrier(0);
        asm volatile("s_waitcnt vmcnt(0)" ::: "memory");
        convert_store(ks + 1, buf ^ 1);
        __syncthreads();
        buf ^= 1;
    }
    float *so = reinterpret_cast<float *>(smem);
    unsigned *rm = reinterpret_cast<unsigned *>(so + TB);
    if constexpr (NP == 2) {
        if (tid < TB) {
            const int b = min(b0 + tid, p.B - 1);
            so[tid] = ldexpf(1.f, -(row_scale_exp(p.sc, b) + p.sc.w_exp));
// ... 56 lines not shown
        if (p.sc.out_rowmax) {
#pragma unroll
            for (int rt = 0; rt < 2; ++rt)
#pragma unroll
                for (int r = 0; r < 16; ++r) atomicMax(rm + wr * 64 + rt * 32 + (r & 3) + 8 * (r >> 2) + 4 * h, __float_as_uint(wmax[rt][r]));
            __syncthreads();
            if (tid < TB && b0 + tid < p.B) atomicMax(reinterpret_cast<unsigned *>(p.sc.out_rowmax) + b0 + tid, rm[tid]);
        }
    }
}


inline int choose_ksplit(int KS, int Lout, int n_chunks) {
    if (KS != 13 || Lout != 1) return 1;
    int s = 1;
    for (int d = 1; d <= n_chunks && d <= 8; ++d)
        if (n_chunks % d == 0) s = d;
    return s;
}

template <int KS, int LIN, int CT, int WO, int WB, int OTW>
int launch(GCParams p, hipStream_t stream, float *ws, size_t ws_floats, size_t *query_ws) {
    constexpr int OT = WO * OTW * 32;
    constexpr int NCOL = WB * 128;
    if (p.CoutPad % OT != 0) {
        roreg::set_error("roreg_group_conv: Cout pad %d not a multiple of the %d-row tile", p.CoutPad, OT);
        return 2;
    }
    if (p.Cin % CT != 0) {
        roreg::set_error("roreg_group_conv: Cin %d not a multiple of the %d-channel chunk", p.Cin, CT);
        return 2;
    }
    p.gt_bytes = round_up(p.Lout * KS * 4, 16);
    int nkp_max = (NCOL - 1) / p.Lout + 2;
    if (nkp_max > p.B) nkp_max = p.B;
    const size_t lds = (size_t)p.gt_bytes + (size_t)nkp_max * CT * LIN * 4;
    if (lds > 160 * 1024) {
        roreg::set_error("roreg_group_conv: tile needs %zu B of LDS", lds);
        return 2;
    }
    const int n_ct = (p.ncols + NCOL - 1) / NCOL;
    const int grid = n_ct * (p.CoutPad / OT);
    const int ksplit = choose_ksplit(KS, p.Lout, p.Cin / CT);
    const size_t n_out = (size_t)p.B * p.Cout * p.Lout;
    if (query_ws) { *query_ws = ksplit > 1 ? (size_t)ksplit * n_out : 0; return 0; }
    auto kern = group_conv_kernel<KS, LIN, CT, WO, WB, OTW>;
    if (lds > 48 * 1024) {
        hipError_t e = hipFuncSetAttribute(reinterpret_cast<const void *>(kern),
                                           hipFuncAttributeMaxDynamicSharedMemorySize, (int)lds);
        if (e != hipSuccess) {
            roreg::set_error("roreg_group_conv: hipFuncSetAttribute(%zu): %s", lds, hipGetErrorString(e));
            return 1;
        }
    }
    p.ksplit = ksplit; p.cin_per_slice = p.Cin / ksplit;
    if (ksplit > 1) {
        if (!ws || ws_floats < (size_t)ksplit * n_out) {
            roreg::set_error("roreg_group_conv: split-K needs a workspace of %zu floats (got %zu)", (size_t)ksplit * n_out, ws_floats);
            return 2;
        }
        p.partial = ws;
    }
    hipLaunchKernelGGL(kern, dim3(grid, ksplit), dim3(256), lds, stream, p);
    if (ksplit > 1)
        hipLaunchKernelGGL(splitk_reduce_kernel, dim3((unsigned)((n_out + 255) / 256)), dim3(256), 0, stream, ws, p.bias, p.residual,
                           p.out, n_out, p.Cout, p.Lout, ksplit);
    ROREG_CHECK_LAUNCH("roreg_group_conv");
    return 0;
}

}

extern "C" size_t roreg_group_conv_packed_size(int Cin, int Cout, int KS) {
    return (size_t)KS * Cin * round_up(Cout, 32);
}

extern "C" int roreg_group_conv_pack_weights(const float *W, int Cin, int Cout, int KS, float *wp) {
    ROREG_REQUIRE(W && wp, "roreg_group_conv_pack_weights: null pointer");
    ROREG_REQUIRE(Cin % 8 == 0 && Cin > 0 && Cout > 0 && (KS == 13 || KS == 1),
                  "roreg_group_conv_pack_weights: unsupported shape Cin=%d Cout=%d KS=%d", Cin, Cout, KS);
    const int CoutPad = round_up(Cout, 32);
    memset(wp, 0, sizeof(float) * roreg_group_conv_packed_size(Cin, Cout, KS));
    for (int k = 0; k < KS; ++k)
        for (int cb = 0; cb < Cin / 8; ++cb)
            for (int o = 0; o < Cout; ++o)
                for (int h = 0; h < 2; ++h)
                    for (int r = 0; r < 4; ++r) {
                        const int c = cb * 8 + 2 * r + h;
                        wp[((((size_t)k * (Cin / 8) + cb) * CoutPad + o) * 2 + h) * 4 + r] =
                            W[((size_t)o * Cin + c) * KS + k];
                    }
    return 0;
}

static int dispatch(GCParams p, int Lin, int KS, hipStream_t s, float *ws, size_t wsf, size_t *q);

extern "C" size_t roreg_group_conv_workspace_size(int B, int Cin, int Cout, int Lin, int Lout, int KS) {
    GCParams p;
    memset(&p, 0, sizeof(p));
    p.B = B; p.Cin = Cin; p.Cout = Cout; p.CoutPad = round_up(Cout, 32); p.Lout = Lout; p.ncols = B * Lout;
    size_t q = 0;
    if (B <= 0 || dispatch(p, Lin, KS, nullptr, nullptr, 0, &q) != 0) return 0;
    return q;
}

extern "C" int roreg_group_conv(const float *x, const float *wpack, const float *bias, const float *bn_scale,
                                const float *bn_shift, const float *residual, float *out, const int32_t *gather,
                                int B, int Cin, int Cout, int Lin, int Lout, int KS, float *workspace, size_t workspace_floats,
                                void *stream) {
    if (B == 0) return 0;
    ROREG_REQUIRE(x && wpack && bias && out && gather, "roreg_group_conv: null pointer");
    ROREG_REQUIRE((bn_scale == nullptr) == (bn_shift == nullptr), "roreg_group_conv: bn_scale/bn_shift must come together");
    ROREG_REQUIRE(B >= 0 && Cin > 0 && Cout > 0 && Lout > 0 && Lin > 0, "roreg_group_conv: bad sizes");
    if (B == 0) return 0;
    ROREG_REQUIRE((long long)B * Lout < (1ll << 31), "roreg_group_conv: too many columns");
    GCParams p;
    p.x = x; p.wp = reinterpret_cast<const float4 *>(wpack); p.bias = bias; p.bn_scale = bn_scale; p.bn_shift = bn_shift;
    p.residual = residual; p.out = out; p.gather = gather;
    p.B = B; p.Cin = Cin; p.Cout = Cout; p.CoutPad = round_up(Cout, 32); p.Lout = Lout; p.ncols = B * Lout; p.gt_bytes = 0;
    p.partial = nullptr; p.ksplit = 1; p.cin_per_slice = Cin;
    return dispatch(p, Lin, KS, roreg::as_stream(stream), workspace, workspace_floats, nullptr);
}

static int dispatch(GCParams p, int Lin, int KS, hipStream_t s, float *ws, size_t wsf, size_t *q) {
    const int cp = p.CoutPad;
    if (KS == 13 && Lin == 60) {
        if (cp % 128 == 0) return launch<13, 60, 32, 2, 2, 2>(p, s, ws, wsf, q);
        if (cp % 64 == 0) return launch<13, 60, 16, 1, 4, 2>(p, s, ws, wsf, q);
        return launch<13, 60, 16, 1, 4, 1>(p, s, ws, wsf, q);
    }
    if (KS == 13 && Lin == 48) {
        if (cp % 256 == 0) return launch<13, 48, 32, 4, 1, 2>(p, s, ws, wsf, q);
        if (cp % 128 == 0) return launch<13, 48, 16, 2, 2, 2>(p, s, ws, wsf, q);
        return launch<13, 48, 16, 1, 4, 1>(p, s, ws, wsf, q);
    }
    if (KS == 13 && Lin == 45) {
        if (cp % 128 == 0) return launch<13, 45, 16, 2, 2, 2>(p, s, ws, wsf, q);
        return launch<13, 45, 16, 1, 4, 1>(p, s, ws, wsf, q);
    }
    if (KS == 13 && Lin == 13) {
        if (cp % 256 == 0) return launch<13, 13, 8, 4, 1, 2>(p, s, ws, wsf, q);
        return launch<13, 13, 8, 1, 4, 1>(p, s, ws, wsf, q);
    }
    if (KS == 1 && Lin == 1) {
        if (cp % 128 == 0) return launch<1, 1, 32, 2, 2, 2>(p, s, ws, wsf, q);
        return launch<1, 1, 32, 1, 4, 1>(p, s, ws, wsf, q);
    }
    roreg::set_error("roreg_group_conv: unsupported (KS=%d, Lin=%d)", KS, Lin);
    return 2;
}

template <int NP>
static int launch_conv_split(GCSplitParams p, hipStream_t s) {
    const size_t lds = (size_t)p.gt_bytes + (size_t)NP * 2 * p.nkp_max * p.S * 16 + (size_t)p.nkp_max * 16 * p.Lin * 4
                       + (size_t)(2 * p.Cin + p.nkp_max) * 4;
    ROREG_REQUIRE(lds <= 160 * 1024, "roreg_group_conv_split: tile needs %zu B of LDS", lds);
    ROREG_REQUIRE((size_t)p.nkp_max * 2 * p.Lin <= 5 * 256 && (size_t)p.nkp_max * 4 * p.Lin <= 9 * 256, "roreg_group_conv_split: %d keypoints x %d columns per tile exceed the staging plan", p.nkp_max, p.Lin);
    ROREG_REQUIRE((long long)p.B * p.Cin * p.Lin < (1ll << 31), "roreg_group_conv_split: input tensor beyond 2^31 elements");
    void (*kern)(GCSplitParams) = group_conv_split_kernel<13, NP>;
    if constexpr (NP == 2) { if (p.packed) kern = group_conv_split_kernel<13, 2, 1>; }
    hipError_t e = hipFuncSetAttribute(reinterpret_cast<const void *>(kern), hipFuncAttributeMaxDynamicSharedMemorySize, (int)lds);
    if (e != hipSuccess) { roreg::set_error("roreg_group_conv_split: hipFuncSetAttribute(%zu): %s", lds, hipGetErrorString(e)); return 1; }
    const int grid = ((p.ncols + 127) / 128) * (p.Cout / 256);
    hipLaunchKernelGGL(kern, dim3(grid), dim3(256), lds, s, p);
    ROREG_CHECK_LAUNCH("roreg_group_conv_split");
    return 0;
}

static int conv_split_common(int np, const float *x, const void *wsplit, const float *bias, const float *bn_scale, const float *bn_shift,
                             float *out, const int32_t *gather, const int32_t *lds_order, int lds_stride, int B, int Cin, int Cout, int Lin, int Lout,
                             int KS, SplitScale sc, void *stream, int packed = 0) {
    if (B == 0) return 0;
    ROREG_REQUIRE(x && wsplit && bias && out && gather && B > 0, "roreg_group_conv_split: bad arguments");
    ROREG_REQUIRE(!packed || (np == 2 && !bn_scale), "roreg_group_conv_split: packed input words go with the fp16 x 2 kernel and carry their activation");
    ROREG_REQUIRE((bn_scale == nullptr) == (bn_shift == nullptr), "roreg_group_conv_split: bn_scale/bn_shift must come together");
    ROREG_REQUIRE(KS == 13 && Cin % 16 == 0 && Cout % 256 == 0 && Lin > 0 && Lin <= 64 && Lout > 0 && Lout <= 64,
                  "roreg_group_conv_split: unsupported shape (KS=%d Cin=%d Cout=%d Lin=%d Lout=%d)", KS, Cin, Cout, Lin, Lout);
    ROREG_REQUIRE((long long)B * Lout < (1ll << 31), "roreg_group_conv_split: too many columns");
    GCSplitParams p;
    p.x = x; p.ws = wsplit; p.bias = bias; p.bn_scale = bn_scale; p.bn_shift = bn_shift; p.out = out;
    p.gather = gather; p.B = B; p.Cin = Cin; p.Cout = Cout; p.CoutPad = Cout; p.Lin = Lin; p.Lout = Lout; p.ncols = B * Lout;
    ROREG_REQUIRE(!lds_order || (lds_stride >= 1 && lds_stride <= 64), "roreg_group_conv_split: lds_stride %d out of range", lds_stride);
    p.order = lds_order; p.S = lds_order ? lds_stride : Lin;
    p.gt_bytes = round_up((Lout * KS + Lin) * 4, 16);
    p.nkp_max = (128 - 1) / Lout + 2;
    if (p.nkp_max > B) p.nkp_max = B;
    p.sc = sc; p.packed = packed;
    return np == 3 ? launch_conv_split<3>(p, roreg::as_stream(stream)) : launch_conv_split<2>(p, roreg::as_stream(stream));
}

extern "C" int roreg_group_conv_split(const float *x, const void *wsplit, const float *bias, const float *bn_scale, const float *bn_shift,
                                      float *out, const int32_t *gather, const int32_t *lds_order, int lds_stride, int B, int Cin, int Cout, int Lin,
                                      int Lout, int KS, void *stream) {
    SplitScale sc = {nullptr, 1.f, 0.f, 0, nullptr};
    return conv_split_common(3, x, wsplit, bias, bn_scale, bn_shift, out, gather, lds_order, lds_stride, B, Cin, Cout, Lin, Lout, KS, sc, stream);
}

extern "C" int roreg_group_conv_f16x2(const float *x, const void *wsplit2, int w_exp, const float *bias, const float *bn_scale, const float *bn_shift,
                                      float act_smax, float act_tmax, const float *in_rowmax_dev, float *out, float *out_rowmax_dev,
                                      const int32_t *gather, const int32_t *lds_order, int lds_stride, int B, int Cin, int Cout, int Lin, int Lout,
                                      int KS, void *stream) {
    ROREG_REQUIRE(in_rowmax_dev, "roreg_group_conv_f16x2: in_rowmax_dev is required");
    SplitScale sc = {in_rowmax_dev, act_smax, act_tmax, w_exp, out_rowmax_dev};
    return conv_split_common(2, x, wsplit2, bias, bn_scale, bn_shift, out, gather, lds_order, lds_stride, B, Cin, Cout, Lin, Lout, KS, sc, stream);
}

extern "C" int roreg_group_conv_f16x2_packed(const uint32_t *x_words, const void *wsplit2, int w_exp, const float *bias, const float *in_bound_dev,
                                             float *out, float *out_rowmax_dev, const int32_t *gather, const int32_t *lds_order, int lds_stride, int B,
                                             int Cin, int Cout, int Lin, int Lout, int KS, void *stream) {
    ROREG_REQUIRE(in_bound_dev, "roreg_group_conv_f16x2_packed: in_bound_dev is required");
    SplitScale sc = {in_bound_dev, 1.f, 0.f, w_exp, out_rowmax_dev};
    return conv_split_common(2, reinterpret_cast<const float *>(x_words), wsplit2, bias, nullptr, nullptr, out, gather, lds_order, lds_stride, B, Cin, Cout, Lin,
                             Lout, KS, sc, stream, 1);
}

template <int NP>
static int launch_dense(DenseParams p, hipStream_t s) {
    const size_t lds = (size_t)2 * (NP * 2 * 128 + NP * 2 * 256) * 16;
    auto kern = dense_split_kernel<NP>;
    hipError_t e = hipFuncSetAttribute(reinterpret_cast<const void *>(kern), hipFuncAttributeMaxDynamicSharedMemorySize, (int)lds);
    if (e != hipSuccess) { roreg::set_error("roreg_dense_split: hipFuncSetAttribute(%zu): %s", lds, hipGetErrorString(e)); return 1; }
    const int grid = ((p.B + 127) / 128) * (p.Opad / 256);
    hipLaunchKernelGGL(kern, dim3(grid), dim3(256), lds, s, p);
    ROREG_CHECK_LAUNCH("roreg_dense_split");
    return 0;
}

static int dense_common(int np, const float *x, const void *wsplit, const float *bias, const float *scale, const float *shift,
                        const float *residual, int residual_stride, float *out, int B, int K, int O, SplitScale sc, void *stream) {
    if (B == 0) return 0;
    ROREG_REQUIRE(x && wsplit && bias && out && B > 0 && K > 0 && O > 0, "roreg_dense_split: bad arguments");
    ROREG_REQUIRE((scale == nullptr) == (shift == nullptr), "roreg_dense_split: scale/shift must come together");
    ROREG_REQUIRE(K % 16 == 0, "roreg_dense_split: K must be a multiple of 16 (got %d)", K);
    ROREG_REQUIRE(!residual || residual_stride >= 1, "roreg_dense_split: residual_stride must be >= 1 (got %d)", residual_stride);
    DenseParams p;
    p.x = x; p.ws = wsplit; p.bias = bias; p.scale = scale; p.shift = shift; p.res = residual; p.res_stride = residual_stride; p.out = out;
    p.B = B; p.K = K; p.O = O; p.Opad = round_up(O, 256); p.sc = sc;
    return np == 3 ? launch_dense<3>(p, roreg::as_stream(stream)) : launch_dense<2>(p, roreg::as_stream(stream));
}

extern "C" int roreg_dense_split(const float *x, const void *wsplit, const float *bias, const float *scale, const float *shift,
                                 const float *residual, int residual_stride, float *out, int B, int K, int O, void *stream) {
    SplitScale sc = {nullptr, 1.f, 0.f, 0, nullptr};
    return dense_common(3, x, wsplit, bias, scale, shift, residual, residual_stride, out, B, K, O, sc, stream);
}

extern "C" int roreg_dense_f16x2(const float *x, const void *wsplit2, int w_exp, const float *bias, const float *scale, const float *shift,
                                 float act_smax, float act_tmax, const float *in_rowmax_dev, const float *residual, int residual_stride,
                                 float *out, float *out_rowmax_dev, int B, int K, int O, void *stream) {
    ROREG_REQUIRE(in_rowmax_dev, "roreg_dense_f16x2: in_rowmax_dev is required");
    SplitScale sc = {in_rowmax_dev, act_smax, act_tmax, w_exp, out_rowmax_dev};
    return dense_common(2, x, wsplit2, bias, scale, shift, residual, residual_stride, out, B, K, O, sc, stream);
}
```

roreg_amd/hip.py:

```python
import ctypes
import os
import threading
from ctypes import c_int, c_void_p, c_size_t, c_double, c_float, c_char_p

import numpy as np
import torch

from .group import tables

_LIB_PATH = os.environ.get('ROREG_HIP_LIB') or os.path.join(os.path.dirname(os.path.abspath(__file__)), 'libroreg_hip.so')

GEMM_MODES = ('f16x2', 'bf16x3', 'f32')
GEMM_MODE = os.environ.get('ROREG_GEMM', 'f16x2')
if GEMM_MODE == 'split':
    GEMM_MODE = 'bf16x3'
if GEMM_MODE not in GEMM_MODES:
    raise ValueError(f"ROREG_GEMM must be one of {GEMM_MODES}, got {GEMM_MODE!r}")
XDMA = os.environ.get('ROREG_GEMM_XDMA', '1') == '1'
MFMA16 = os.environ.get('ROREG_GEMM_MFMA16', '1') == '1'


def use_planes(O):
    return bool(XDMA and O % 256 == 0 and not os.environ.get('ROREG_TILE_M128'))
_lib = None
_tables_uploaded = False

from ._abi import ABI_VERSION, PROTOTYPES, _P, _LT_TASK, _RANSAC_TASK, _MATCH_TASK, _GATHER_TASK


class HipError(RuntimeError):
    pass


def lib():
    global _lib
    if _lib is None:
        if not os.path.exists(_LIB_PATH):
            raise HipError(f'{_LIB_PATH} is missing -- build it with `make -C roreg_amd/csrc` '
                           f'(or __graft_entry__.build()); there is no CPU fallback')
        L = ctypes.CDLL(_LIB_PATH)
        for name, (res, args) in PROTOTYPES.items():
            fn = getattr(L, name)
            fn.restype = res
            fn.argtypes = args
        got = L.roreg_abi_version()
        if got != ABI_VERSION:
            raise HipError(f'{_LIB_PATH} reports C-ABI version {got}, this binding was written against {ABI_VERSION} '
                           f'(include/roreg_hip.h ROREG_ABI_VERSION): rebuild with `make -C roreg_amd/csrc`')
        _lib = L
    return _lib


def _check(rc, what):
    if rc != 0:
        raise HipError(f'{what} failed ({rc}): {lib().roreg_last_error().decode()}')


def ensure_tables():
    global _tables_uploaded
    if not _tables_uploaded:
        T = tables()
        P = np.ascontiguousarray(T.P, np.int32)
        Nei = np.ascontiguousarray(T.Nei, np.int32)
        R = np.ascontiguousarray(T.R, np.float64)
        _check(lib().roreg_set_group_tables(P.ctypes.data, Nei.ctypes.data, R.ctypes.data), 'roreg_set_group_tables')
        _tables_uploaded = True


def _stream():
    return c_void_p(torch.cuda.current_stream().cuda_stream)


class PinnedPool:

    def __init__(self, max_bytes=None):
        self.lock = threading.Lock()
        self.free = {}
        self.held = 0
        self.max_bytes = int(os.environ.get('ROREG_PINNED_POOL_GB', 12)) << 30 if max_bytes is None else max_bytes

    @staticmethod
    def size_class(nbytes):
        if nbytes <= 4096:
            return 4096
        step = 1 << max(int(nbytes - 1).bit_length() - 4, 0)
        return -(-nbytes // step) * step

    def acquire(self, nbytes):
        c = self.size_class(max(int(nbytes), 1))
        with self.lock:
            got = self.free.get(c)
            if got:
                self.held -= c
                return got.pop()
        return torch.empty(c, dtype=torch.uint8, pin_memory=True)

    def release(self, buf):
        c = int(buf.shape[0])
        with self.lock:
            if self.held + c <= self.max_bytes:
                self.free.setdefault(c, []).append(buf)
                self.held += c


pinned_pool = PinnedPool()
_named_streams = {}


def named_stream(name, priority=0):
    st = _named_streams.get(name)
    if st is None:
        st = _named_streams[name] = torch.cuda.Stream(priority=priority)
    return st


class _StagingRing:

    def __init__(self, slots=64):
        self.bufs = [None] * slots
        self.events = [None] * slots
        self.next = 0

    def upload(self, array):
        a = np.ascontiguousarray(array)
        nbytes = a.nbytes
        if nbytes == 0:
            return torch.from_numpy(a).cuda()
        k = self.next
        self.next = (k + 1) % len(self.bufs)
        if self.events[k] is not None:
            self.events[k].synchronize()
        if self.bufs[k] is None or self.bufs[k].shape[0] < nbytes or self.bufs[k].shape[0] > 4 * PinnedPool.size_class(nbytes):
            if self.bufs[k] is not None:
                pinned_pool.release(self.bufs[k])
            self.bufs[k] = pinned_pool.acquire(nbytes)
        host = self.bufs[k][:nbytes]
        host.numpy()[:] = a.reshape(-1).view(np.uint8)
        dev = host.cuda(non_blocking=True).view(torch.from_numpy(a[:0].reshape(-1)).dtype).reshape(a.shape)
        if self.events[k] is None:
            self.events[k] = torch.cuda.Event()
        self.events[k].record()
        return dev


_staging = threading.local()


def upload(array):
    ring = getattr(_staging, 'ring', None)
    if ring is None:
        ring = _staging.ring = _StagingRing()
    return ring.upload(array)


def _ptr(t, dtype=None):
    if t is None:
        return None
    if not t.is_cuda:
        raise HipError('expected a device tensor (the HIP path has no host fallback)')
    if not t.is_contiguous():
        raise HipError('expected a contiguous tensor')
    if dtype is not None and t.dtype != dtype:
        raise HipError(f'expected dtype {dtype}, got {t.dtype}')
    return c_void_p(t.data_ptr())


def _feat(t):
    if t is None:
        return None, 0
    if t.dtype == torch.bfloat16:
        return _ptr(t, torch.bfloat16), 1
    return _ptr(t, torch.float32), 0


def pack_conv_weights(W):
    Wn = W.detach().to('cpu', torch.float32).contiguous().numpy()
    Cout, Cin = Wn.shape[0], Wn.shape[1]
    KS = int(np.prod(Wn.shape[2:]))
    Wn = np.ascontiguousarray(Wn.reshape(Cout, Cin, KS))
    n = lib().roreg_group_conv_packed_size(Cin, Cout, KS)
    out = np.empty(n, np.float32)
    _check(lib().roreg_group_conv_pack_weights(Wn.ctypes.data, Cin, Cout, KS, out.ctypes.data), 'roreg_group_conv_pack_weights')
    return torch.from_numpy(out).cuda()


class ConvLayer:

    def __init__(self, weight, bias, bn=None, eps=1e-5, device='cuda'):
        self.Cout, self.Cin = int(weight.shape[0]), int(weight.shape[1])
        self.KS = int(np.prod(weight.shape[2:]))
        self.wpack = pack_conv_weights(weight)
        self._weight = weight.detach().to('cpu', torch.float32).clone()
        self._wsplit = None
        self.bias = bias.detach().to(device, torch.float32).contiguous()
        if bn is not None:
            g, b, m, v = [t.detach().to('cpu', torch.float32) for t in bn]
            scale = g / torch.sqrt(v + eps)
            shift = b - m * scale
            self.scale = scale.to(device).contiguous()
            self.shift = shift.to(device).contiguous()
        else:
            self.scale = self.shift = None


_gather_cache = {}


def _conv_wsplit(layer):
    if layer._wsplit is None:
        layer._wsplit = group_conv_split_pack(layer._weight)
    return layer._wsplit


def _conv_wsplit2(layer):
    if getattr(layer, '_wsplit2', None) is None:
        Wn = layer._weight.numpy()
        w_exp = f16_scale_exp(float(np.abs(Wn).max()))
        out = f16_split2_frags(Wn.reshape(Wn.shape[0], Wn.shape[1], -1), w_exp)
        smax = float(layer.scale.abs().max()) if layer.scale is not None else 1.0
        tmax = float(layer.shift.abs().max()) if layer.shift is not None else 0.0
        layer._wsplit2 = (torch.from_numpy(out).cuda(), w_exp, smax, tmax)
    return layer._wsplit2

PROFILE = None


WORK = None

PROFILE_SLOTS = {'mm_tile': 0, 'ransac_score': 1, 'des2r': 2, 'ft_nonlin': 3, 'sinkhorn': 4, 'topk_dot': 5, 'icp_search': 6}


def profile_enable(on=True):
    _check(lib().roreg_profile_enable(1 if on else 0), 'roreg_profile_enable')


def profile_read(name):
    ms = c_double(0.0); n = c_int(0)
    _check(lib().roreg_profile_read(PROFILE_SLOTS[name], ctypes.byref(ms), ctypes.byref(n)), 'roreg_profile_read')
    return ms.value, n.value


def gather_table(key, array):
    t = _gather_cache.get(key)
    if t is None:
        t = torch.from_numpy(np.ascontiguousarray(array, np.int32)).cuda()
        _gather_cache[key] = t
    return t


def full_gather():
    return gather_table('nei60', tables().Nei)


_lds_order_ok = set()


def _check_lds_order(order_t, stride, gather, Lin):
    key = (order_t.data_ptr(), int(stride), gather.data_ptr())
    if key in _lds_order_ok:
        return
    if order_t.numel() != Lin or not 1 <= int(stride) <= 64:
        raise HipError(f'group_conv: lds_order must hold one slot per input column ({Lin}) and a stride in 1..64')
    o = order_t.cpu().numpy(); cols = np.unique(gather.cpu().numpy())
    if cols.min() < 0 or cols.max() >= Lin:
        raise HipError('group_conv: the gather table reads a column outside the input')
    slots = o[cols]
    if slots.min() < 0 or slots.max() >= stride or np.unique(slots).size != slots.size:
        raise HipError(f'group_conv: lds_order must give the {cols.size} gathered columns distinct slots in [0, {stride})')
    _lds_order_ok.add(key)


def group_conv(x, layer, gather=None, Lout=None, residual=None, out=None, split=False, in_rowmax=None, want_rowmax=False, lds_order=None):
    ensure_tables()
    B, Cin, Lin = x.shape
    assert Cin == layer.Cin, (Cin, layer.Cin)
    if gather is None:
        gather = full_gather() if layer.KS == 13 else gather_table(('id', Lin), np.arange(Lin)[:, None])
    Lout = int(gather.shape[0]) if Lout is None else Lout
    if out is None:
        out = torch.empty((B, layer.Cout, Lout), dtype=torch.float32, device=x.device)
    split_ok = residual is None and layer.KS == 13 and Cin % 16 == 0 and layer.Cout % 256 == 0 and Lin <= 64 and Lout <= 64 and B > 0
    nkp = min((128 - 1) // max(Lout, 1) + 2, max(B, 1))
    split_ok = split_ok and nkp * 2 * Lin <= 5 * 256 and nkp * 4 * Lin <= 9 * 256
    order_t, order_s = (None, 0) if lds_order is None else lds_order
    if order_t is not None:
        _check_lds_order(order_t, order_s, gather, Lin)
    if in_rowmax is not None:
        if not split_ok:
            raise HipError('group_conv: the fp16 x 2 kernel does not support this shape')
        if in_rowmax.numel() != B:
            raise HipError(f'group_conv: in_rowmax must hold one value per row ({B}), got {in_rowmax.numel()}')
        w2, w_exp, smax, tmax = _conv_wsplit2(layer)
        amax = torch.zeros(B, dtype=torch.float32, device=x.device) if want_rowmax else None
        _check(lib().roreg_group_conv_f16x2(_ptr(x, torch.float32), _ptr(w2), w_exp, _ptr(layer.bias), _ptr(layer.scale), _ptr(layer.shift), smax, tmax,
                                            _ptr(in_rowmax, torch.float32), _ptr(out, torch.float32), _ptr(amax), _ptr(gather, torch.int32),
                                            _ptr(order_t, torch.int32), order_s, B, Cin, layer.Cout, Lin, Lout, layer.KS, _stream()), 'roreg_group_conv_f16x2')
        return (out, amax) if want_rowmax else out
    if split and split_ok:
        _check(lib().roreg_group_conv_split(_ptr(x, torch.float32), _ptr(_conv_wsplit(layer)), _ptr(layer.bias), _ptr(layer.scale), _ptr(layer.shift),
                                            _ptr(out, torch.float32), _ptr(gather, torch.int32), _ptr(order_t, torch.int32), order_s, B, Cin, layer.Cout, Lin, Lout,
                                            layer.KS, _stream()), 'roreg_group_conv_split')
        return out
    ws_n = lib().roreg_group_conv_workspace_size(B, Cin, layer.Cout, Lin, Lout, layer.KS)
    ws = torch.empty(ws_n, dtype=torch.float32, device=x.device) if ws_n else None
    if PROFILE is not None:
        e0 = torch.cuda.Event(enable_timing=True); e1 = torch.cuda.Event(enable_timing=True)
        e0.record()
    _check(lib().roreg_group_conv(_ptr(x, torch.float32), _ptr(layer.wpack), _ptr(layer.bias), _ptr(layer.scale), _ptr(layer.shift),
                                  _ptr(residual, torch.float32), _ptr(out, torch.float32), _ptr(gather, torch.int32),
                                  B, Cin, layer.Cout, Lin, Lout, layer.KS, _ptr(ws), ws_n, _stream()), 'roreg_group_conv')
    if PROFILE is not None:
        e1.record()
        PROFILE.append(((B, Cin, layer.Cout, Lout, layer.KS), e0, e1))
    return out


def group_conv_packed(x_words, layer, in_bound, gather, want_rowmax=False, lds_order=None):
    ensure_tables()
    B, Cin, Lin = x_words.shape
    assert Cin == layer.Cin and x_words.dtype == torch.int32, (Cin, layer.Cin, x_words.dtype)
    Lout = int(gather.shape[0])
    if not (layer.KS == 13 and Cin % 16 == 0 and layer.Cout % 256 == 0 and Lin <= 64 and Lout <= 64 and B > 0):
        raise HipError('group_conv_packed: the fp16 x 2 kernel does not support this shape')
    if in_bound.numel() < B:
        raise HipError(f'group_conv_packed: in_bound must hold one value per row ({B}), got {in_bound.numel()}')
    order_t, order_s = (None, 0) if lds_order is None else lds_order
    if order_t is not None:
        _check_lds_order(order_t, order_s, gather, Lin)
    w2, w_exp, _, _ = _conv_wsplit2(layer)
    out = torch.empty((B, layer.Cout, Lout), dtype=torch.float32, device=x_words.device)
    amax = torch.zeros(B, dtype=torch.float32, device=x_words.device) if want_rowmax else None
    _check(lib().roreg_group_conv_f16x2_packed(_ptr(x_words, torch.int32), _ptr(w2), w_exp, _ptr(layer.bias), _ptr(in_bound, torch.float32), _ptr(out),
                                               _ptr(amax), _ptr(gather, torch.int32), _ptr(order_t, torch.int32), order_s, B, Cin, layer.Cout, Lin, Lout,
                                               layer.KS, _stream()), 'roreg_group_conv_f16x2_packed')
    return (out, amax) if want_rowmax else out


def gf_finalize(eqv_raw, want_inv=True, out_dtype=torch.float32):
    B = eqv_raw.shape[0]
    eqv = torch.empty(eqv_raw.shape, dtype=out_dtype, device=eqv_raw.device)
    inv = torch.empty((B, 32), dtype=torch.float32, device=eqv_raw.device) if want_inv else None
    ep, bf = _feat(eqv)
    _check(lib().roreg_gf_finalize(_ptr(eqv_raw, torch.float32), ep, bf, _ptr(inv), B, _stream()), 'roreg_gf_finalize')
    return eqv, inv


def det_score(enc):
    ensure_tables()
    B = enc.shape[0]
    assert enc.shape[1:] == (16, 60)
    out = torch.empty(B, dtype=torch.float32, device=enc.device)
    _check(lib().roreg_det_score(_ptr(enc, torch.float32), _ptr(out), B, _stream()), 'roreg_det_score')
    return out


def inv_descriptor(eqv, roles=None):
    N = eqv.shape[0]
    assert eqv.shape[1:] == (32, 60)
    out = torch.empty((N, 32), dtype=torch.float32, device=eqv.device)
    ep, bf = _feat(eqv)
    if roles is not None:
        scale, shift, role = _role_args(roles, N)
        _check(lib().roreg_inv_descriptor_roles(ep, bf, _ptr(out), _ptr(scale[64:]), _ptr(shift[64:]), _ptr(role), N, _stream()), 'roreg_inv_descriptor_roles')
        return out
    _check(lib().roreg_inv_descriptor(ep, bf, _ptr(out), N, _stream()), 'roreg_inv_descriptor')
    return out


def _role_args(roles, N):
    scale, shift, role = roles
    if scale.numel() != 128 or shift.numel() != 128 or scale.dtype != torch.float32 or shift.dtype != torch.float32:
        raise HipError('roles: scale / shift must hold the 128 float32 channels of Conv_init')
    if role.shape != (N, 4) or role.dtype != torch.float32:
        raise HipError('roles: the table must be float32 [keypoints, 4]')
    return scale, shift, role


def nn_search(src, tgt, src_rows=None, tgt_rows=None, want_dist=False, squared=False):
    F = src.shape[1]
    m = int(src_rows.shape[0]) if src_rows is not None else int(src.shape[0])
    n = int(tgt_rows.shape[0]) if tgt_rows is not None else int(tgt.shape[0])
    idx = torch.empty(m, dtype=torch.int64, device=src.device)
    dist = torch.empty(m, dtype=torch.float32, device=src.device) if want_dist else None
    scratch = torch.empty(max(m, 1), dtype=torch.int64, device=src.device)
    _check(lib().roreg_nn_search_ex(_ptr(src, torch.float32), _ptr(src_rows, torch.int64), m, _ptr(tgt, torch.float32),
                                    _ptr(tgt_rows, torch.int64), n, F, 1 if squared else 0, _ptr(idx), _ptr(dist), _ptr(scratch), _stream()), 'roreg_nn_search')
    return (idx, dist) if want_dist else idx


def knn_search(src, tgt, k, want_dist=False, squared=False):
    m, F = src.shape
    n = tgt.shape[0]
    idx = torch.empty((m, k), dtype=torch.int64, device=src.device)
    dist = torch.empty((m, k), dtype=torch.float32, device=src.device) if want_dist else None
    ws_n = lib().roreg_knn_search_workspace(m, n)
    ws = torch.empty(ws_n // 4, dtype=torch.int32, device=src.device) if ws_n else None
    _check(lib().roreg_knn_search_ex(_ptr(src, torch.float32), m, _ptr(tgt, torch.float32), n, F, k, 1 if squared else 0, _ptr(idx), _ptr(dist),
                                     _ptr(ws), ws_n, _stream()), 'roreg_knn_search')
    return (idx, dist) if want_dist else idx


def pdist(A, B, squared=False):
    m, F = A.shape
    n = B.shape[0]
    if B.shape[1] != F:
        raise HipError(f'pdist: feature widths differ ({F} vs {B.shape[1]})')
    out = torch.empty((m, n), dtype=torch.float32, device=A.device)
    _check(lib().roreg_pdist(_ptr(A, torch.float32), m, _ptr(B, torch.float32), n, F, 1 if squared else 0, _ptr(out), _stream()), 'roreg_pdist')
    return out


def knn_search_seg(pts, seg, k):
    total, F = pts.shape
    idx = torch.empty((total, k), dtype=torch.int64, device=pts.device)
    if seg.min < k:
        raise HipError(f'knn_search_seg: a segment has fewer than k={k} points')
    ws_n = lib().roreg_knn_search_seg_workspace(total, seg.n, seg.max, seg.max)
    ws = torch.empty(ws_n // 4, dtype=torch.int32, device=pts.device)
    sp = _ptr(seg.dev, torch.int32)
    _check(lib().roreg_knn_search_seg(_ptr(pts, torch.float32), _ptr(pts, torch.float32), sp, sp, seg.n, total, seg.max, seg.max, F, k, _ptr(idx),
                                      _ptr(ws), ws_n, _stream()), 'roreg_knn_search_seg')
    return idx


def mutual_matches(nn01, nn10, sample0=None, sample1=None):
    m = nn01.shape[0]
    out = torch.empty((max(m, 1), 2), dtype=torch.int64, device=nn01.device)
    cnt = torch.zeros(1, dtype=torch.int32, device=nn01.device)
    _check(lib().roreg_mutual_matches(_ptr(nn01, torch.int64), _ptr(nn10, torch.int64), m, int(nn10.shape[0]), _ptr(sample0, torch.int64),
                                      _ptr(sample1, torch.int64), _ptr(out), _ptr(cnt), _stream()), 'roreg_mutual_matches')
    return out, cnt




class GatheredRows:

    def __init__(self, rows, dr, bound, bf16, keep):
        self.rows, self.dr, self.bound, self.bf16, self.keep = rows, dr, bound, bf16, keep
        self.shape = (int(rows.shape[0]), 128, 60)


def role_max(before, after, bn):
    (bp, bf_b), (ap, bf_a) = _feat(before), _feat(after)
    if bf_b != bf_a or before.shape != after.shape:
        raise HipError('role_max: before and after must share dtype and shape')
    scale, shift = bn
    if scale.numel() != 128 or shift.numel() != 128:
        raise HipError('role_max: bn must hold the 128 channels of Conv_init')
    N = int(before.shape[0])
    out = torch.empty((N, 4), dtype=torch.float32, device=before.device)
    _check(lib().roreg_role_max(bp, ap, bf_b, _ptr(scale, torch.float32), _ptr(shift, torch.float32), _ptr(out), N, _stream()), 'roreg_role_max')
    return out


class LtBatch:

    def __init__(self, tasks):
        self.n_tasks = len(tasks)
        table = np.zeros(self.n_tasks, _LT_TASK)
        off = 0
        self.offsets = []
        n_coef = 0; n_bf16 = 0
        seen = {}

        def feat(t):
            r = seen.get(id(t))
            if r is None:
                r = seen[id(t)] = (t.data_ptr(), _feat(t)[1])
            return r

        def vptr(t, dtype):
            r = seen.get(id(t))
            if r is None:
                _ptr(t, dtype)
                r = seen[id(t)] = (t.data_ptr(), False)
            return r[0]

        cols = [[] for _ in range(12)]
        n_role = 0
        role_ptrs = []
        for task in tasks:
            b0, b1, a0, a1, k0, k1, m, sel = task[:8]
            c0, c1 = (task[8], task[9]) if len(task) > 8 else (None, None)
# ... 438 lines not shown
```

roreg_amd/network/eqv_trans.py:

```python
import os

import numpy as np
import torch
import torch.nn as nn

from .. import hip
from ..group import tables
from .ops import Comb_Conv, Residual_Comb_Conv, _Branch, _version_key


class ET_test(nn.Module):
    def __init__(self, cfg):
        super().__init__()
        self.cfg = cfg
        self.Conv_init = Comb_Conv(32 * 4, 256)
        self.PartII_SO3_Conv_layers = nn.ModuleList([Residual_Comb_Conv(256, 512, 256)])
        d = [256, 512, 128, 4]
        self.PartII_To_R_dims = d
        self.PartII_To_R_FC = nn.Sequential(
            nn.Conv2d(d[0], d[1], 1, 1), nn.BatchNorm2d(d[1]), nn.ReLU(),
            nn.Conv2d(d[1], d[2], 1, 1), nn.BatchNorm2d(d[2]), nn.ReLU(),
            nn.Conv2d(d[2], d[3], 1, 1))
        self.pruned = True
        self.fourier_init = True
        self.gemm = hip.GEMM_MODE
        self.packed_trunk = os.environ.get('ROREG_ET_PACKED', '1') != '0'

    def _head_plans(self):
        fc = self.PartII_To_R_FC
        key = _version_key(fc)
        if getattr(self, '_head_key', None) != key:
            def bn(m):
                return (m.weight, m.bias, m.running_mean, m.running_var)
            self._head = [hip.ConvLayer(fc[0].weight, fc[0].bias, None),
                          hip.ConvLayer(fc[3].weight, fc[3].bias, bn(fc[1]), eps=fc[1].eps),
                          hip.ConvLayer(fc[6].weight, fc[6].bias, bn(fc[4]), eps=fc[4].eps)]
            self._head_key = key
        return self._head

    def _dense_plans(self):
        res = self.PartII_SO3_Conv_layers[0]
        fc = self.PartII_To_R_FC
        key = _version_key(res.comb_layer_out, fc)
        if getattr(self, '_dense_key', None) != key:
            def fold(bn):
                g, b, m, v = [t.detach().to('cpu', torch.float32).numpy() for t in (bn.weight, bn.bias, bn.running_mean, bn.running_var)]
                sc = g / np.sqrt(v + bn.eps)
                return sc, b - m * sc
            T = tables()
            l0, l1 = T.live_sets(2)[0], T.live_sets(2)[1]
            pos1 = {g: i for i, g in enumerate(l1)}
            cols = [pos1[int(v)] for v in T.Nei[l0[0]]]
            Wc = res.comb_layer_out[2].weight.detach().to('cpu', torch.float32).numpy()[:, :, 0, :]
            Wd = np.zeros((Wc.shape[0], Wc.shape[1], 13), np.float32)
            for k, col in enumerate(cols):
                Wd[:, :, col] += Wc[:, :, k]
            sc, sh = fold(res.comb_layer_out[0])
            out = hip.DenseSplitLayer(Wd.reshape(Wd.shape[0], -1), res.comb_layer_out[2].bias.detach().cpu().numpy(), np.repeat(sc, 13), np.repeat(sh, 13))
            def w1(conv):
                return conv.weight.detach().to('cpu', torch.float32).numpy()[:, :, 0, 0], conv.bias.detach().cpu().numpy()
            h0 = hip.DenseSplitLayer(*w1(fc[0]))
            h1 = hip.DenseSplitLayer(*w1(fc[3]), *fold(fc[1]))
            h2 = hip.DenseSplitLayer(*w1(fc[6]), *fold(fc[4]))
            self._dense = (out, h0, h1, h2)
            self._dense_key = key
        return self._dense

    LIVE_PAD = 48

    _LDS_ORDER_45 = (32, 12, 28, 30, 42, 35, 15, 40, 17, 39, 29, 22, 26, 4, 11, 18, 6, 9, 33, 24, 8, 2, 7, 1, 14, 34, 37, 27, 13, 38, 20, 25, 10, 21, 43, 16,
                     36, 0, 19, 5, 41, 3, 31, 23, 44)

    @classmethod
    def _trunk_lds_order(cls):
        order = np.full(cls.LIVE_PAD, -1, np.int32)
        order[:45] = cls._LDS_ORDER_45
        assert sorted(order[:45].tolist()) == list(range(45))
        return hip.gather_table('et_lds_order', order), 45

    @staticmethod
    def _pruned_gathers():
        T = tables()
        live = T.live_sets(2)
        l0, l1, l2 = live[0], live[1], live[2]
        pos2 = {g: i for i, g in enumerate(l2)}
        pos1 = {g: i for i, g in enumerate(l1)}
        ga = T.Nei[l2]
        gb = np.array([[pos2[int(v)] for v in T.Nei[g]] for g in l1])
        gc = np.array([[pos1[int(v)] for v in T.Nei[g]] for g in l0])
        gmap = np.full(60, -1, np.int32)
        for g, i in pos2.items():
            gmap[g] = i
        return (hip.gather_table('et_a', ga), hip.gather_table('et_b', gb), hip.gather_table('et_c', gc), pos2[0],
                hip.gather_table('et_gmap', gmap))

    def _fourier_init(self):
        from .gf_fourier import _Layer, _fold_bn
        key = _version_key(self.Conv_init)
        if getattr(self, '_finit_key', None) != key:
            self._finit = (_Layer(self.Conv_init.comb_layer[2]), _fold_bn(self.Conv_init.comb_layer[0]))
            self._finit_key = key
        return self._finit

    def _trunk_bn(self):
        from .gf_fourier import _fold_bn
        res = self.PartII_SO3_Conv_layers[0]
        key = _version_key(res.comb_layer_in[0], self.Conv_init)
        if getattr(self, '_tbn_key', None) != key:
            bn = _fold_bn(res.comb_layer_in[0])
            self._tbn = (bn, hip.next_bound_spatial(bn, self._fourier_init()[0].bias))
            self._tbn_key = key
        return self._tbn

    def assemble(self, data):
        dev = 'cuda'
        b0 = data['before_eqv0'].to(dev, torch.float32).contiguous(); b1 = data['before_eqv1'].to(dev, torch.float32).contiguous()
        a0 = data['after_eqv0'].to(dev, torch.float32).contiguous(); a1 = data['after_eqv1'].to(dev, torch.float32).contiguous()
        pre = data['pre_idx'].to(dev, torch.int64).contiguous()
        return hip.et_gather(b1, b0, a1, a0, pre), pre

    def conv_init_bn(self):
        if self.pruned and self.fourier_init and self.gemm == 'f16x2':
            return self._fourier_init()[1]
        return None

    def trunk_and_head(self, x, x_bound=None):
        res = self.PartII_SO3_Conv_layers[0]
        h0p, h1p, h2p = self._head_plans()
        if isinstance(x, hip.GatheredRows) and self.conv_init_bn() is None:
            raise hip.HipError('trunk_and_head: rows by reference need the pruned f16x2 irrep path')
        if self.pruned:
            ga, gb, gc, p0, gmap = self._pruned_gathers()
            B = x.shape[0]
            if self.fourier_init:
                layer, bn = self._fourier_init()
                hip.ensure_fourier()
                sp = self.gemm != 'f32'
                if self.gemm == 'f16x2':
                    if isinstance(x, hip.GatheredRows):
                        b0 = x.bound
                        X0 = hip.ft_nonlin_gathered(x, bn=bn, planes=hip.use_planes(256))
                    else:
                        b0 = x_bound if x_bound is not None else hip.row_bound(x, bn=bn)
                        X0 = hip.ft_nonlin(B, 128, x_spatial=x, bn=bn, split='f16x2', out_bound=b0, planes=hip.use_planes(256))
                    d_out, d0, d1, d2 = self._dense_plans()
                    if self.packed_trunk:
                        bn_t, nb_t = self._trunk_bn()
                        T0, b1 = hip.irrep_gemm(X0, None, 128, 256, B, f16x2=layer.wsplit2, x_bound=b0, next_bound=nb_t, x_planes=hip.use_planes(256))
                        del X0
                        hw, h0 = hip.ft_nonlin_packed(B, 256, T0, layer.bias, bn_t, b1, g_map=gmap, Lout=self.LIVE_PAD, Lvalid=45, raw_g=0)
                        del T0
                        m, am = hip.group_conv_packed(hw, res._b_in.plan(), b1, gb, want_rowmax=True, lds_order=self._trunk_lds_order())
                        t, at = hip.dense_split(m.view(B, -1), d_out, residual=h0, in_rowmax=am, want_rowmax=True)
                    else:
                        T0 = hip.irrep_gemm(X0, None, 128, 256, B, f16x2=layer.wsplit2, x_bound=b0, x_planes=hip.use_planes(256))
                        del X0
                        h, ah = hip.ft_nonlin(B, 256, coef_in=T0, bias=layer.bias, spatial_out=True, g_map=gmap, Lout=self.LIVE_PAD, Lvalid=45, split='f16x2',
                                              want_rowmax=True)
                        del T0
                        m, am = res._b_in(h, gather=gb, in_rowmax=ah, want_rowmax=True, lds_order=self._trunk_lds_order())
                        t, at = hip.dense_split(m.view(B, -1), d_out, residual=h[:, :, p0:], residual_stride=self.LIVE_PAD, in_rowmax=am, want_rowmax=True)
                    z, az = hip.dense_split(t, d0, in_rowmax=at, want_rowmax=True)
                    z, az = hip.dense_split(z, d1, in_rowmax=az, want_rowmax=True)
                    return hip.dense_split(z, d2, in_rowmax=az)
                X0 = hip.ft_nonlin(B, 128, x_spatial=x, bn=bn, split=sp)
                T0 = hip.irrep_gemm(X0, layer.wpack, 128, 256, B, split=layer.wsplit if sp else None)
                del X0
                h = hip.ft_nonlin(B, 256, coef_in=T0, bias=layer.bias, spatial_out=True, g_map=gmap, Lout=self.LIVE_PAD, Lvalid=45, split=sp)
                del T0
            else:
                h = self.Conv_init(x, gather=ga)
            m = res._b_in(h, gather=gb, split=self.gemm != 'f32',
                          lds_order=self._trunk_lds_order() if (self.fourier_init and self.gemm != 'f32') else None)
            sc = h[:, :, p0:p0 + 1].contiguous()
            if self.gemm != 'f32':
                d_out, d0, d1, d2 = self._dense_plans()
                t = hip.dense_split(m.view(B, -1), d_out, residual=sc.view(B, -1))
                return hip.dense_split(hip.dense_split(hip.dense_split(t, d0), d1), d2)
            t = res._b_out(m, gather=gc, residual=sc)
        else:
            h = self.Conv_init(x)
            t = res(h)[:, :, 0:1].contiguous()
        z = hip.group_conv(t, h0p)
        z = hip.group_conv(z, h1p)
        z = hip.group_conv(z, h2p)
        return z[:, :, 0].contiguous()

    def forward(self, data):
        x, pre = self.assemble(data)
        q = self.trunk_and_head(x)
        q = q / torch.norm(q, dim=1)[:, None]
        return {'quaternion_pre': q, 'pre_idxs': pre}
```

Before: 1093.

## Write trunk activations as a fragment image and add line-store conv epilogue

The Fourier nonlinearity kernel gains an image mode. It writes the packed fp16 hi/lo activations straight into a 48-slot, k-octet fragment layout that follows the conv's LDS slot order, so the group conv can stage its input without re-gathering and re-splitting words. The group conv also gets a line-store epilogue for the 13-column output, and both paths are on by default. This adds LDS staging, extra syncthreads and new kernel instantiations, and it ties the image layout to a fixed slot count.

```diff
diff --git a/include/roreg_hip.h b/include/roreg_hip.h
--- a/include/roreg_hip.h
+++ b/include/roreg_hip.h
@@ -42,6 +42,9 @@
 int roreg_group_conv_f16x2_packed(const uint32_t *x_words, const void *wsplit2, int w_exp, const float *bias, const float *in_bound_dev,
                                   float *out, float *out_rowmax_dev, const int32_t *gather, const int32_t *lds_order, int lds_stride,
                                   int B, int Cin, int Cout, int Lin, int Lout, int KS, void *stream);
+int roreg_group_conv_f16x2_packed_ex(const uint32_t *x, const void *wsplit2, int w_exp, const float *bias, const float *in_bound_dev,
+                                     float *out, float *out_rowmax_dev, const int32_t *gather, const int32_t *lds_order, int lds_stride,
+                                     int B, int Cin, int Cout, int Lin, int Lout, int KS, int image, int line_stores, void *stream);
 
 int roreg_gf_finalize(const float *eqv_raw, void *eqv, int eqv_bf16 ,
                       float *inv, int B, void *stream);
@@ -266,6 +269,9 @@
 int roreg_ft_nonlin_packed(const float *Xin, const float *bias, const float *bn_scale, const float *bn_shift, uint32_t *out_words,
                            const int32_t *g_map, int Lout, int Lvalid, int B, int C, const float *out_bound, float *raw_col, int raw_g,
                            void *stream);
+int roreg_ft_nonlin_image(const float *Xin, const float *bias, const float *bn_scale, const float *bn_shift, uint32_t *out_image,
+                          const int32_t *g_map, const int32_t *lds_order, int Lout, int B, int C, const float *out_bound, float *raw_col, int raw_g,
+                          void *stream);
 int roreg_ft_nonlin_gathered(const uint64_t *rows , const int64_t *dr , int feat_bf16, const float *bn_scale ,
                              const float *bn_shift, float *Xout, int B, const float *out_bound , int out_planes, void *stream);
 
diff --git a/roreg_amd/_abi.py b/roreg_amd/_abi.py
--- a/roreg_amd/_abi.py
+++ b/roreg_amd/_abi.py
@@ -17,6 +17,7 @@
     'roreg_group_conv_split': (c_int, [_P, _P, _P, _P, _P, _P, _P, _P, c_int, c_int, c_int, c_int, c_int, c_int, c_int, _P]),
     'roreg_group_conv_f16x2': (c_int, [_P, _P, c_int, _P, _P, _P, c_float, c_float, _P, _P, _P, _P, _P, c_int, c_int, c_int, c_int, c_int, c_int, c_int, _P]),
     'roreg_group_conv_f16x2_packed': (c_int, [_P, _P, c_int, _P, _P, _P, _P, _P, _P, c_int, c_int, c_int, c_int, c_int, c_int, c_int, _P]),
+    'roreg_group_conv_f16x2_packed_ex': (c_int, [_P, _P, c_int, _P, _P, _P, _P, _P, _P, c_int, c_int, c_int, c_int, c_int, c_int, c_int, c_int, c_int, _P]),
     'roreg_dense_f16x2': (c_int, [_P, _P, c_int, _P, _P, _P, c_float, c_float, _P, _P, c_int, _P, _P, c_int, c_int, c_int, _P]),
     'roreg_dense_split': (c_int, [_P, _P, _P, _P, _P, _P, c_int, _P, c_int, c_int, c_int, _P]),
     'roreg_gf_finalize': (c_int, [_P, _P, c_int, _P, c_int, _P]),
@@ -102,6 +103,7 @@
     'roreg_row_bound': (c_int, [_P, c_int, _P, _P, _P, c_int, c_int, _P]),
     'roreg_ft_nonlin': (c_int, [_P, _P, _P, _P, _P, _P, _P, _P, _P, _P, c_int, c_int, c_int, c_int, c_int, _P, _P, c_int, c_int, _P]),
     'roreg_ft_nonlin_packed': (c_int, [_P, _P, _P, _P, _P, _P, c_int, c_int, c_int, c_int, _P, _P, c_int, _P]),
+    'roreg_ft_nonlin_image': (c_int, [_P, _P, _P, _P, _P, _P, _P, c_int, c_int, c_int, _P, _P, c_int, _P]),
     'roreg_ft_nonlin_gathered': (c_int, [_P, _P, c_int, _P, _P, _P, c_int, _P, c_int, _P]),
 }
 
diff --git a/roreg_amd/_hip_fourier.py b/roreg_amd/_hip_fourier.py
--- a/roreg_amd/_hip_fourier.py
+++ b/roreg_amd/_hip_fourier.py
@@ -1,4 +1,5 @@
 import os
+import weakref
 from ctypes import c_void_p
 
 import numpy as np
@@ -7,7 +8,7 @@
 from . import hip as _core
 from .hip import HipError, _check, _feat, _ptr, _stream, lib
 
-__all__ = ['DenseSplitLayer', 'IRREP_DIMS', 'IRREP_OFFSETS', '_bf16_split3', '_keypoint_of_columns', '_ptr_array', '_res_ptr', '_tile_cache', 'bf16_split3_frags', 'bf16_split3_pack', 'bound_exp', 'coef_pitch', 'coef_size', 'coef_views', 'dense_split', 'ensure_fourier', 'f16_scale_exp', 'f16_split2_frags', 'f16_split2_pack', 'frag_pack', 'ft_nonlin', 'ft_nonlin_gathered', 'ft_nonlin_packed', 'gemm_persistent', 'group_conv_split_pack', 'irrep_gemm', 'next_bound', 'next_bound_spatial', 'pack_coefs_f16x2', 'row_bound', 'unpack_coefs_f16x2', 'words_to_planes']
+__all__ = ['DenseSplitLayer', 'IMAGE_SLOTS', 'IRREP_DIMS', 'IRREP_OFFSETS', '_bf16_split3', '_keypoint_of_columns', '_ptr_array', '_res_ptr', '_tile_cache', 'bf16_split3_frags', 'bf16_split3_pack', 'bound_exp', 'coef_pitch', 'coef_size', 'coef_views', 'dense_split', 'ensure_fourier', 'f16_scale_exp', 'f16_split2_frags', 'f16_split2_pack', 'frag_pack', 'ft_nonlin', 'ft_nonlin_gathered', 'ft_nonlin_packed', 'gemm_persistent', 'group_conv_split_pack', 'image_index', 'irrep_gemm', 'next_bound', 'next_bound_spatial', 'pack_coefs_f16x2', 'row_bound', 'unpack_coefs_f16x2', 'words_to_image', 'words_to_planes']
 
 
 _fourier_ready = False
@@ -176,13 +177,77 @@
     return u.float().cuda().contiguous(), v.float().cuda().contiguous()
 
 
-def ft_nonlin_packed(B, C, coef_in, bias, bn, out_bound, g_map=None, Lout=60, Lvalid=60, raw_g=None):
+_image_order_ok = {}
+IMAGE_SLOTS = 48
+
+
+def image_index(C, slot_of_col):
+    slot_of_col = np.asarray(slot_of_col, np.int64)
+    Lout = slot_of_col.size
+    col_of = np.full(IMAGE_SLOTS, -1, np.int64)
+    for col, s in enumerate(slot_of_col):
+        if 0 <= s < IMAGE_SLOTS:
+            if col_of[s] >= 0:
+                raise ValueError(f'image_index: columns {col_of[s]} and {col} share slot {s}')
+            col_of[s] = col
+    live = col_of >= 0
+    ch = (16 * np.arange(C // 16)[:, None, None, None] + 8 * np.arange(2)[None, :, None, None] + np.arange(8)[None, None, None, :])
+    src = np.where(live[None, None, :, None], ch * Lout + np.maximum(col_of, 0)[None, None, :, None], 0)
+    return src, live
+
+
+def words_to_image(words, slot_of_col):
+    w = np.ascontiguousarray(words).view(np.uint32)
+    B, C, Lout = w.shape
+    src, live = image_index(C, slot_of_col)
+    g = w.reshape(B, C * Lout)[:, src.reshape(-1)].reshape(B, C // 16, 2, IMAGE_SLOTS, 8)
+    g = np.where(live[None, None, None, :, None], g, 0).astype(np.uint32)
+    halves = np.stack([(g & 0xffff).astype(np.uint16), (g >> 16).astype(np.uint16)], axis=2)
+    return np.ascontiguousarray(halves).view(np.uint32).view(np.int32)
+
+
+def _packed_out(out, words_shape, raw_shape, dev):
+    if out is None:
+        return (torch.empty(words_shape, dtype=torch.int32, device=dev),
+                torch.empty(raw_shape, dtype=torch.float32, device=dev) if raw_shape is not None else None)
+    words, raw = out
+    ok = tuple(words.shape) == tuple(words_shape) and words.dtype == torch.int32 and words.is_contiguous()
+    if raw_shape is not None:
+        ok = ok and raw is not None and tuple(raw.shape) == tuple(raw_shape) and raw.dtype == torch.float32 and raw.is_contiguous()
+    if not ok:
+        raise HipError(f'ft_nonlin_packed: out must be contiguous int32 {tuple(words_shape)} and float32 {raw_shape}')
+    return words, (raw if raw_shape is not None else None)
+
+
+def ft_nonlin_packed(B, C, coef_in, bias, bn, out_bound, g_map=None, Lout=60, Lvalid=60, raw_g=None, image_order=None, out=None):
     ensure_fourier()
     dev = coef_in.device
     if coef_in.numel() != coef_size(C, B) or out_bound.numel() != coef_pitch(B):
         raise HipError('ft_nonlin_packed: coef_in / out_bound sizes')
-    words = torch.empty((B, C, Lout if g_map is not None else 60), dtype=torch.int32, device=dev)
-    raw = torch.empty((B, C), dtype=torch.float32, device=dev) if raw_g is not None else None
+    if image_order is not None:
+        order_t, stride = image_order
+        Lo = Lout if g_map is not None else 60
+        if C % 16 or order_t.numel() != Lo or not 1 <= int(stride) <= IMAGE_SLOTS:
+            raise HipError(f'ft_nonlin_packed: the image form needs C % 16 == 0, one slot per column ({Lo}) and a stride in 1..{IMAGE_SLOTS}')
+        ent = _image_order_ok.get(id(order_t))
+        if ent is None or ent[0]() is not order_t:
+            for k in [k for k, v in _image_order_ok.items() if v[0]() is None]:
+                del _image_order_ok[k]
+            ent = _image_order_ok[id(order_t)] = (weakref.ref(order_t), set())
+        if (int(stride), int(Lvalid)) not in ent[1]:
+            o_all = order_t.cpu().numpy(); o = o_all[o_all >= 0]
+            if o.size and (o.max() >= int(stride) or np.unique(o).size != o.size):
+                raise HipError(f'ft_nonlin_packed: the image form needs distinct slots in [0, {int(stride)})')
+            if g_map is not None and (o_all[int(Lvalid):] >= 0).any():
+                raise HipError(f'ft_nonlin_packed: columns from Lvalid = {int(Lvalid)} on must not have a slot in the image form')
+            ent[1].add((int(stride), int(Lvalid)))
+        image, raw = _packed_out(out, (B, C, IMAGE_SLOTS), (B, C) if raw_g is not None else None, dev)
+        scale, shift = bn if bn is not None else (None, None)
+        _check(lib().roreg_ft_nonlin_image(_ptr(coef_in, torch.float32), _ptr(bias), _ptr(scale), _ptr(shift), _ptr(image), _ptr(g_map, torch.int32),
+                                           _ptr(order_t, torch.int32), int(Lo), B, C, _ptr(out_bound, torch.float32), _ptr(raw), int(raw_g or 0), _stream()),
+               'roreg_ft_nonlin_image')
+        return image, raw
+    words, raw = _packed_out(out, (B, C, Lout if g_map is not None else 60), (B, C) if raw_g is not None else None, dev)
     scale, shift = bn if bn is not None else (None, None)
     _check(lib().roreg_ft_nonlin_packed(_ptr(coef_in, torch.float32), _ptr(bias), _ptr(scale), _ptr(shift), _ptr(words), _ptr(g_map, torch.int32),
                                         int(Lout), int(Lvalid), B, C, _ptr(out_bound, torch.float32), _ptr(raw), int(raw_g or 0), _stream()),
diff --git a/roreg_amd/csrc/fourier.hip b/roreg_amd/csrc/fourier.hip
--- a/roreg_amd/csrc/fourier.hip
+++ b/roreg_amd/csrc/fourier.hip
@@ -1286,6 +1286,7 @@
     int sp_pack;
     float *raw_col;
     int raw_g;
+    const int *img_order;
     int B, Bp, C, tiles_per_c, Lout, Lvalid;
     const roreg::LtRow *g_rows;
     const int64_t *g_dr;
@@ -1344,7 +1345,8 @@
 template <int N, class F>
 __device__ __forceinline__ void static_for(F &&f) { static_for_impl(std::make_integer_sequence<int, N>{}, f); }
 
-template <bool IN_SPATIAL, bool OUT_SPATIAL, int SPLIT , int NW , int MINW , bool OUT_ROWS = false, bool GATHER = false >
+template <bool IN_SPATIAL, bool OUT_SPATIAL, int SPLIT , int NW , int MINW , bool OUT_ROWS = false, bool GATHER = false ,
+          bool IMG = false >
 __global__ __launch_bounds__(NW * 64, MINW) void ft_nonlin_kernel(NonlinParams p) {
     constexpr int NT = NW * 64;
     const int lane = threadIdx.x & 63;
@@ -1358,7 +1360,12 @@
     constexpr int NA1 = SPLIT ? 4 * 2 * NPL * 64 * 4 : 30 * 2 * 64, NA2 = SPLIT ? 4 * 2 * NPL * 64 * 4 : 32 * 2 * 64;
     __shared__ __attribute__((aligned(16))) float sA1[IN_SPATIAL ? 64 : NA1];
     __shared__ __attribute__((aligned(16))) float sA2[OUT_SPATIAL ? 64 : NA2];
-    __shared__ float sT[(IN_SPATIAL || OUT_SPATIAL || OUT_ROWS) ? NW * 32 * 65 : 64];
+    static_assert(!IMG || (NW == 8 && OUT_SPATIAL && SPLIT == 2 && !IN_SPATIAL), "the fragment image is written by eight waves, one channel of a k-octet each");
+    __shared__ float sT[(!IMG && (IN_SPATIAL || OUT_SPATIAL || OUT_ROWS)) ? NW * 32 * 65 : 64];
+    constexpr int IMG_SLOTS = 48, IMG_TS = IMG_SLOTS + 1, TS = IMG ? IMG_TS : 65;
+    extern __shared__ __attribute__((aligned(16))) float img_xb[];
+    if constexpr (IMG)
+        for (int i = threadIdx.x; i < 8 * 32 * IMG_TS; i += NT) img_xb[i] = 0.f;
     {
         const float *g1 = SPLIT == 3 ? reinterpret_cast<const float *>(p.A1s) : SPLIT == 2 ? reinterpret_cast<const float *>(p.A1h) : p.A1;
         const float *g2 = SPLIT == 3 ? reinterpret_cast<const float *>(p.A2s) : SPLIT == 2 ? reinterpret_cast<const float *>(p.A2h) : p.A2;
@@ -1369,7 +1376,14 @@
     }
     __shared__ float sBias[512], sScale[512], sShift[512];
     __shared__ int sGmap[64];
-    if (threadIdx.x < 64) sGmap[threadIdx.x] = (OUT_SPATIAL && p.g_map && threadIdx.x < ROREG_G) ? p.g_map[threadIdx.x] : (int)threadIdx.x;
+    if (threadIdx.x < 64) {
+        int go = (OUT_SPATIAL && p.g_map && threadIdx.x < ROREG_G) ? p.g_map[threadIdx.x] : (int)threadIdx.x;
+        if constexpr (IMG) {
+            if (go >= 0 && p.img_order) go = go < p.Lout ? p.img_order[go] : -1;
+            if (go >= IMG_SLOTS) go = -1;
+        }
+        sGmap[threadIdx.x] = go;
+    }
     __shared__ uint8_t sP8[GATHER ? ROREG_G * ROREG_G : 4];
     if constexpr (GATHER)
         for (int i = threadIdx.x; i < ROREG_G * ROREG_G; i += NT) sP8[i] = p.g_P8[i];
@@ -1580,7 +1594,8 @@
         const bool has_rs = OUT_SPATIAL && p.r_spatial;
         const bool rs_late = has_rs && !bn && !p.g_map && !p.out_rowmax;
         const size_t rs = ((size_t)bb * C + c) * ROREG_G;
-        float *tb = (OUT_SPATIAL || OUT_ROWS) ? sT + (threadIdx.x >> 6) * (32 * 65) : nullptr;
+        float *tb = IMG ? img_xb + (threadIdx.x >> 6) * (32 * IMG_TS)
+                        : (OUT_SPATIAL || OUT_ROWS) ? sT + (threadIdx.x >> 6) * (32 * 65) : nullptr;
         const bool sp_pack = OUT_SPATIAL && SPLIT == 2 && p.sp_pack;
         const float pk_scale = sp_pack ? ldexpf(1.f, bound_exp(cv[NCV])) : 1.f;
 #pragma unroll
@@ -1590,7 +1605,8 @@
                 const int g = t * 32 + (r & 3) + 8 * (r >> 2) + 4 * h;
                 float x = v[t][r] + bsum;
                 if (OUT_SPATIAL && has_rs && !rs_late && g < ROREG_G) x += ld_sp(p.r_spatial, rs + g);
-                if (sp_pack && p.raw_col && g == p.raw_g && valid) p.raw_col[(size_t)bb * C + c] = x;
+                if constexpr (IMG) { if (p.raw_col && g == p.raw_g) tb[jn * IMG_TS + IMG_SLOTS] = x; }
+                else if (sp_pack && p.raw_col && g == p.raw_g && valid) p.raw_col[(size_t)bb * C + c] = x;
                 if (bn) x = fmaxf(fmaf(x, sc, sh), 0.f);
                 if (g >= ROREG_G || !valid) x = 0.f;
                 v[t][r] = x;
@@ -1601,14 +1617,45 @@
                             const float xs = x * pk_scale;
                             const _Float16 h1 = (_Float16)xs;
                             const _Float16 l1 = (_Float16)(xs - (float)h1);
-                            tb[jn * 65 + go] = __uint_as_float((unsigned)__builtin_bit_cast(unsigned short, h1) | ((unsigned)__builtin_bit_cast(unsigned short, l1) << 16));
+                            tb[jn * TS + go] = __uint_as_float((unsigned)__builtin_bit_cast(unsigned short, h1) | ((unsigned)__builtin_bit_cast(unsigned short, l1) << 16));
                         } else {
-                            tb[jn * 65 + go] = x; wmax = fmaxf(wmax, fabsf(x));
+                            tb[jn * TS + go] = x; wmax = fmaxf(wmax, fabsf(x));
                         }
                     }
                 }
             }
-        if (OUT_SPATIAL) {
+        if constexpr (IMG) {
+            __syncthreads();
+            {
+                const int w8 = threadIdx.x >> 6, b0 = tbi * 32, oct = c >> 3;
+                const unsigned *xw = reinterpret_cast<const unsigned *>(img_xb);
+                char *img = reinterpret_cast<char *>(p.out_spatial);
+                const size_t row_bytes = (size_t)(C / 16) * (4 * IMG_SLOTS * 16);
+                struct Q4 { unsigned a, b, c, d; };
+#pragma unroll
+                for (int it = 0; it < 3; ++it) {
+                    const int idx = it * 64 + lane, kps = idx / IMG_SLOTS, slot = idx - kps * IMG_SLOTS, kp = 4 * w8 + kps;
+                    unsigned wv[8], hw[4], lw[4];
+#pragma unroll
+                    for (int e = 0; e < 8; ++e) wv[e] = xw[(e * 32 + kp) * IMG_TS + slot];
+#pragma unroll
+                    for (int e = 0; e < 4; ++e) {
+                        hw[e] = __builtin_amdgcn_perm(wv[2 * e + 1], wv[2 * e], 0x05040100u);
+                        lw[e] = __builtin_amdgcn_perm(wv[2 * e + 1], wv[2 * e], 0x07060302u);
+                    }
+                    if (b0 + kp < B) {
+                        char *dst = img + (size_t)(b0 + kp) * row_bytes + (size_t)(oct >> 1) * (4 * IMG_SLOTS * 16) + (oct & 1) * (IMG_SLOTS * 16) + slot * 16;
+                        *reinterpret_cast<Q4 *>(dst) = Q4{hw[0], hw[1], hw[2], hw[3]};
+                        *reinterpret_cast<Q4 *>(dst + 2 * IMG_SLOTS * 16) = Q4{lw[0], lw[1], lw[2], lw[3]};
+                    }
+                }
+                if (p.raw_col && lane < 32) {
+                    const int kp = 4 * w8 + (lane >> 3), e = lane & 7;
+                    if (b0 + kp < B) p.raw_col[(size_t)(b0 + kp) * C + 8 * oct + e] = img_xb[(e * 32 + kp) * IMG_TS + IMG_SLOTS];
+                }
+            }
+            __syncthreads();
+        } else if (OUT_SPATIAL) {
             asm volatile("s_waitcnt lgkmcnt(0)" ::: "memory");
             const int b0 = tbi * 32;
             if (b0 + 32 <= B) {
@@ -2214,6 +2261,42 @@
     return 0;
 }
 
+extern "C" int roreg_ft_nonlin_image(const float *Xin, const float *bias, const float *bn_scale, const float *bn_shift, uint32_t *out_image,
+                                     const int32_t *g_map, const int32_t *lds_order, int Lout, int B, int C, const float *out_bound, float *raw_col, int raw_g,
+                                     void *stream) {
+    ROREG_REQUIRE(g_A1 && g_A2, "roreg_ft_nonlin_image: roreg_set_fourier_tables has not been called");
+    ROREG_REQUIRE(Xin && out_image && out_bound && B > 0 && C > 0 && C <= 512 && C % 16 == 0 && (bn_scale == nullptr) == (bn_shift == nullptr),
+                  "roreg_ft_nonlin_image: bad arguments (C a multiple of 16, at most 512)");
+    ROREG_REQUIRE(!g_map || (Lout > 0 && Lout <= 64), "roreg_ft_nonlin_image: bad Lout");
+    ROREG_REQUIRE(!raw_col || (raw_g >= 0 && raw_g < ROREG_G), "roreg_ft_nonlin_image: raw_g out of range");
+    NonlinParams p;
+    memset(&p, 0, sizeof(p));
+    p.Xin = Xin; p.out_spatial = reinterpret_cast<float *>(out_image);
+    p.g_map = g_map; p.img_order = lds_order; p.Lout = g_map ? Lout : ROREG_G; p.Lvalid = p.Lout;
+    p.bias = bias; p.bn_scale = bn_scale; p.bn_shift = bn_shift; p.A1 = g_A1; p.A2 = g_A2;
+    p.A1s = reinterpret_cast<const bf16x8 *>(g_A1s); p.A2s = reinterpret_cast<const bf16x8 *>(g_A2s);
+    p.A1h = reinterpret_cast<const f16x8 *>(g_A1h); p.A2h = reinterpret_cast<const f16x8 *>(g_A2h); p.f_exp = g_f_exp;
+    p.out_bound = out_bound; p.sp_pack = 1; p.raw_col = raw_col; p.raw_g = raw_g;
+    p.B = B; p.Bp = (B + 31) / 32 * 32; p.C = C; p.tiles_per_c = (B + 31) / 32;
+    ROREG_REQUIRE((unsigned long long)C * p.Bp * 20ull < (1ull << 32), "roreg_ft_nonlin_image: C * round_up(B, 32) must stay below 2^32 / 20 (32-bit lane offsets)");
+    hipStream_t s = roreg::as_stream(stream);
+    roreg::ProfScope prof(roreg::PROF_FT_NONLIN, s);
+    void (*kern)(NonlinParams) = ft_nonlin_kernel<false, true, 2, 8, 4, false, false, true>;
+    constexpr int lds = 8 * 32 * 49 * 4;
+    hipError_t e = hipFuncSetAttribute(reinterpret_cast<const void *>(kern), hipFuncAttributeMaxDynamicSharedMemorySize, lds);
+    if (e != hipSuccess) { roreg::set_error("roreg_ft_nonlin_image: hipFuncSetAttribute(%d): %s", lds, hipGetErrorString(e)); return 1; }
+    static const int resident = [&] {
+        int per_cu = 0, dev = 0, cus = 256;
+        if (hipOccupancyMaxActiveBlocksPerMultiprocessor(&per_cu, kern, 512, lds) != hipSuccess || per_cu < 1) per_cu = 2;
+        if (hipGetDevice(&dev) == hipSuccess) (void)hipDeviceGetAttribute(&cus, hipDeviceAttributeMultiprocessorCount, dev);
+        return per_cu * cus;
+    }();
+    const long long want = (long long)C * p.tiles_per_c / 8, cap = (long long)resident * 4;
+    hipLaunchKernelGGL(kern, dim3((unsigned)(want > cap ? cap : want)), dim3(512), lds, s, p);
+    ROREG_CHECK_LAUNCH("roreg_ft_nonlin_image");
+    return 0;
+}
+
 extern "C" int roreg_ft_nonlin_gathered(const uint64_t *rows, const int64_t *dr, int feat_bf16, const float *bn_scale, const float *bn_shift, float *Xout,
                                         int B, const float *out_bound, int out_planes, void *stream) {
     ROREG_REQUIRE(g_A1 && g_A2, "roreg_ft_nonlin_gathered: roreg_set_fourier_tables has not been called");
diff --git a/roreg_amd/csrc/group_conv.hip b/roreg_amd/csrc/group_conv.hip
--- a/roreg_amd/csrc/group_conv.hip
+++ b/roreg_amd/csrc/group_conv.hip
@@ -209,11 +209,14 @@
     const int32_t *order;
     int S;
     int packed;
+    int line_stores;
 };
-
-template <int KS, int NP, int PK = 0>
+constexpr int GC_IMG_SLOTS = 48;
+
+template <int KS, int NP, int PK = 0, bool LS = false>
 __global__ __launch_bounds__(256, 2) void group_conv_split_kernel(GCSplitParams p) {
     constexpr bool PACKED = PK != 0;
+    static_assert(!LS || PACKED, "the line-store epilogue reuses the packed forms' staging area");
     static_assert(!PACKED || NP == 2, "packed input words are fp16 hi / lo pairs");
     using frag = typename std::conditional<NP == 3, bf16x8, f16x8>::type;
     extern __shared__ __attribute__((aligned(16))) char smem[];
@@ -270,10 +273,12 @@
     float *raw = reinterpret_cast<float *>(slab + (size_t)NP * plane_stride);
     const int raw_floats = p.nkp_max * 16 * Lin;
     float *bn_s = raw + raw_floats, *bn_h = bn_s + p.Cin, *kp_scale = bn_h + p.Cin;
-    for (int i = tid; i < p.Cin; i += 256) { bn_s[i] = has_bn ? p.bn_scale[i] : 1.f; bn_h[i] = has_bn ? p.bn_shift[i] : 0.f; }
-    if constexpr (NP == 2)
-        for (int i = tid; i < nkp; i += 256) kp_scale[i] = ldexpf(1.f, row_scale_exp(p.sc, b_first + i));
-    const int pieces = nkp * 4 * Lin;
+    if constexpr (PK != 2) {
+        for (int i = tid; i < p.Cin; i += 256) { bn_s[i] = has_bn ? p.bn_scale[i] : 1.f; bn_h[i] = has_bn ? p.bn_shift[i] : 0.f; }
+        if constexpr (NP == 2)
+            for (int i = tid; i < nkp; i += 256) kp_scale[i] = ldexpf(1.f, row_scale_exp(p.sc, b_first + i));
+    }
+    const int pieces = PK == 2 ? 4 * p.nkp_max * S : nkp * 4 * Lin;
     constexpr int RAW_ITERS = 9;
     int raw_off[RAW_ITERS];
 #pragma unroll
@@ -281,13 +286,18 @@
         const int pc = w * 64 + q * 256 + lane;
         raw_off[q] = -1;
         if (pc < pieces) {
-            const int kp = pc / (4 * Lin), r = pc - kp * (4 * Lin);
-            raw_off[q] = ((b_first + kp) * p.Cin) * Lin + 4 * r;
+            if constexpr (PK == 2) {
+                const int ph = pc / h_stride, r = pc - ph * h_stride, kp = r / S, slot = r - kp * S;
+                if (kp < nkp) raw_off[q] = ((b_first + kp) * p.Cin) * GC_IMG_SLOTS + (ph * GC_IMG_SLOTS + slot) * 4;
+            } else {
+                const int kp = pc / (4 * Lin), r = pc - kp * (4 * Lin);
+                raw_off[q] = ((b_first + kp) * p.Cin) * Lin + 4 * r;
+            }
         }
     }
     auto issue_raw = [&](int c0) {
-        const float *xc = p.x + (size_t)c0 * Lin;
-        float *dst0 = raw + (size_t)(w * 64) * 4;
+        const float *xc = p.x + (size_t)c0 * (PK == 2 ? GC_IMG_SLOTS : Lin);
+        float *dst0 = (PK == 2 ? reinterpret_cast<float *>(slab + (size_t)((c0 >> 4) & 1) * NP * plane_stride) : raw) + (size_t)(w * 64) * 4;
 #pragma unroll
         for (int q = 0; q < RAW_ITERS; ++q) {
             if (w * 64 + q * 256 < pieces) {
@@ -371,7 +381,8 @@
         }
     };
     auto convert = [&](int c0) {
-        if constexpr (PACKED) convert_packed(); else convert_float(c0);
+        if constexpr (PK == 2) return;
+        else if constexpr (PACKED) convert_packed(); else convert_float(c0);
     };
     issue_raw(0);
     asm volatile("s_waitcnt vmcnt(0)" ::: "memory");
@@ -383,8 +394,8 @@
 
     for (int c0 = 0; c0 < p.Cin; c0 += 16) {
         const bool more = c0 + 16 < p.Cin;
-        __syncthreads();
-        const frag *slab_cur = slab;
+        if constexpr (PK != 2) __syncthreads();
+        const frag *slab_cur = PK == 2 ? slab + (size_t)((c0 >> 4) & 1) * NP * plane_stride : slab;
 
         frag aw[2][2][NP];
         auto load_a = [&](int k, frag (&a)[2][NP]) {
@@ -466,6 +477,46 @@
             const int o = o_wave + ot * 32 + (r & 3) + 8 * (r >> 2) + 4 * h;
             bv[ot][r] = o < p.Cout ? p.bias[o] : 0.f;
         }
+    if constexpr (LS) {
+        constexpr int LO = 13, RUN4 = 32 * LO / 4;
+        __syncthreads();
+        float *stg = reinterpret_cast<float *>(smem + p.gt_bytes) + w * (32 * NCOL);
+        const int shift = col0 - b_first * LO;
+        const int ncl = col_last - col0 + 1;
+#pragma unroll
+        for (int ot = 0; ot < 2; ++ot) {
+#pragma unroll
+            for (int t = 0; t < 4; ++t)
+#pragma unroll
+                for (int r = 0; r < 16; ++r) {
+                    const float v = acc[ot][t][r] * oscale[t] + bv[ot][r];
+                    stg[((r & 3) + 8 * (r >> 2) + 4 * h) * NCOL + t * 32 + j] = v;
+                    if (valid[t]) wmax[t] = fmaxf(wmax[t], fabsf(v));
+                }
+            asm volatile("s_waitcnt lgkmcnt(0)" ::: "memory");
+            float *ob = p.out + ((size_t)b_first * p.Cout + o_wave + ot * 32) * LO;
+            for (int it = lane; it < nkp * RUN4; it += 64) {
+                const int kp = it / RUN4, f0 = (it - kp * RUN4) * 4;
+                float v4[4];
+                bool ok[4];
+#pragma unroll
+                for (int e = 0; e < 4; ++e) {
+                    const int o = (f0 + e) / LO, g = (f0 + e) - o * LO, cl = kp * LO + g - shift;
+                    ok[e] = cl >= 0 && cl < ncl;
+                    v4[e] = stg[o * NCOL + (ok[e] ? cl : 0)];
+                }
+                float *dst = ob + (size_t)kp * p.Cout * LO + f0;
+                if (ok[0] && ok[1] && ok[2] && ok[3]) {
+                    *reinterpret_cast<float4 *>(dst) = make_float4(v4[0], v4[1], v4[2], v4[3]);
+                } else {
+#pragma unroll
+                    for (int e = 0; e < 4; ++e)
+                        if (ok[e]) dst[e] = v4[e];
+                }
+            }
+            asm volatile("s_waitcnt lgkmcnt(0)" ::: "memory");
+        }
+    } else {
 #pragma unroll
     for (int ot = 0; ot < 2; ++ot) {
 #pragma unroll
@@ -481,6 +532,7 @@
                 }
             }
         }
+    }
     }
     if constexpr (NP == 2) {
         if (p.sc.out_rowmax) {
@@ -843,13 +895,22 @@
 
 template <int NP>
 static int launch_conv_split(GCSplitParams p, hipStream_t s) {
-    const size_t lds = (size_t)p.gt_bytes + (size_t)NP * 2 * p.nkp_max * p.S * 16 + (size_t)p.nkp_max * 16 * p.Lin * 4
-                       + (size_t)(2 * p.Cin + p.nkp_max) * 4;
+    size_t lds = p.packed == 2 ? (size_t)p.gt_bytes + 2 * ((size_t)NP * 2 * p.nkp_max * p.S * 16)
+                 : (size_t)p.gt_bytes + (size_t)NP * 2 * p.nkp_max * p.S * 16 + (size_t)p.nkp_max * 16 * p.Lin * 4
+                   + (size_t)(2 * p.Cin + p.nkp_max) * 4;
+    ROREG_REQUIRE(!p.line_stores || (p.packed && p.Lout == 13), "roreg_group_conv_split: the line-store epilogue belongs to the packed forms with 13 output columns");
+    ROREG_REQUIRE(!p.line_stores || (reinterpret_cast<uintptr_t>(p.out) & 15) == 0, "roreg_group_conv_split: the line-store epilogue needs `out` on a 16-byte boundary");
+    if (p.line_stores && lds < (size_t)p.gt_bytes + 4 * 32 * 128 * 4) lds = (size_t)p.gt_bytes + 4 * 32 * 128 * 4;
+    ROREG_REQUIRE(p.packed != 2 || (p.order && p.S <= GC_IMG_SLOTS && p.Lin == GC_IMG_SLOTS && (size_t)p.nkp_max * 4 * p.S <= 9 * 256),
+                  "roreg_group_conv_split: the fragment image has %d slots per keypoint and needs its slot order (Lin=%d S=%d)", GC_IMG_SLOTS, p.Lin, p.S);
     ROREG_REQUIRE(lds <= 160 * 1024, "roreg_group_conv_split: tile needs %zu B of LDS", lds);
     ROREG_REQUIRE((size_t)p.nkp_max * 2 * p.Lin <= 5 * 256 && (size_t)p.nkp_max * 4 * p.Lin <= 9 * 256, "roreg_group_conv_split: %d keypoints x %d columns per tile exceed the staging plan", p.nkp_max, p.Lin);
     ROREG_REQUIRE((long long)p.B * p.Cin * p.Lin < (1ll << 31), "roreg_group_conv_split: input tensor beyond 2^31 elements");
     void (*kern)(GCSplitParams) = group_conv_split_kernel<13, NP>;
-    if constexpr (NP == 2) { if (p.packed) kern = group_conv_split_kernel<13, 2, 1>; }
+    if constexpr (NP == 2) {
+        if (p.packed == 2) kern = p.line_stores ? group_conv_split_kernel<13, 2, 2, true> : group_conv_split_kernel<13, 2, 2>;
+        else if (p.packed) kern = p.line_stores ? group_conv_split_kernel<13, 2, 1, true> : group_conv_split_kernel<13, 2, 1>;
+    }
     hipError_t e = hipFuncSetAttribute(reinterpret_cast<const void *>(kern), hipFuncAttributeMaxDynamicSharedMemorySize, (int)lds);
     if (e != hipSuccess) { roreg::set_error("roreg_group_conv_split: hipFuncSetAttribute(%zu): %s", lds, hipGetErrorString(e)); return 1; }
     const int grid = ((p.ncols + 127) / 128) * (p.Cout / 256);
@@ -860,7 +921,7 @@
 
 static int conv_split_common(int np, const float *x, const void *wsplit, const float *bias, const float *bn_scale, const float *bn_shift,
                              float *out, const int32_t *gather, const int32_t *lds_order, int lds_stride, int B, int Cin, int Cout, int Lin, int Lout,
-                             int KS, SplitScale sc, void *stream, int packed = 0) {
+                             int KS, SplitScale sc, void *stream, int packed = 0, int line_stores = 0) {
     if (B == 0) return 0;
     ROREG_REQUIRE(x && wsplit && bias && out && gather && B > 0, "roreg_group_conv_split: bad arguments");
     ROREG_REQUIRE(!packed || (np == 2 && !bn_scale), "roreg_group_conv_split: packed input words go with the fp16 x 2 kernel and carry their activation");
@@ -876,7 +937,7 @@
     p.gt_bytes = round_up((Lout * KS + Lin) * 4, 16);
     p.nkp_max = (128 - 1) / Lout + 2;
     if (p.nkp_max > B) p.nkp_max = B;
-    p.sc = sc; p.packed = packed;
+    p.sc = sc; p.packed = packed; p.line_stores = line_stores;
     return np == 3 ? launch_conv_split<3>(p, roreg::as_stream(stream)) : launch_conv_split<2>(p, roreg::as_stream(stream));
 }
 
@@ -903,6 +964,15 @@
     SplitScale sc = {in_bound_dev, 1.f, 0.f, w_exp, out_rowmax_dev};
     return conv_split_common(2, reinterpret_cast<const float *>(x_words), wsplit2, bias, nullptr, nullptr, out, gather, lds_order, lds_stride, B, Cin, Cout, Lin,
                              Lout, KS, sc, stream, 1);
+}
+
+extern "C" int roreg_group_conv_f16x2_packed_ex(const uint32_t *x, const void *wsplit2, int w_exp, const float *bias, const float *in_bound_dev,
+                                                float *out, float *out_rowmax_dev, const int32_t *gather, const int32_t *lds_order, int lds_stride, int B,
+                                                int Cin, int Cout, int Lin, int Lout, int KS, int image, int line_stores, void *stream) {
+    ROREG_REQUIRE(in_bound_dev && (!image || lds_order), "roreg_group_conv_f16x2_packed_ex: in_bound_dev is required, and lds_order with the image");
+    SplitScale sc = {in_bound_dev, 1.f, 0.f, w_exp, out_rowmax_dev};
+    return conv_split_common(2, reinterpret_cast<const float *>(x), wsplit2, bias, nullptr, nullptr, out, gather, lds_order, lds_stride, B, Cin, Cout, Lin,
+                             Lout, KS, sc, stream, image ? 2 : 1, line_stores ? 1 : 0);
 }
 
 template <int NP>
diff --git a/roreg_amd/hip.py b/roreg_amd/hip.py
--- a/roreg_amd/hip.py
+++ b/roreg_amd/hip.py
@@ -18,6 +18,20 @@
     raise ValueError(f"ROREG_GEMM must be one of {GEMM_MODES}, got {GEMM_MODE!r}")
 XDMA = os.environ.get('ROREG_GEMM_XDMA', '1') == '1'
 MFMA16 = os.environ.get('ROREG_GEMM_MFMA16', '1') == '1'
+ET_IMAGE = os.environ.get('ROREG_ET_IMAGE', '1') != '0'
+CONV_LINE_STORES = os.environ.get('ROREG_CONV_LINE_STORES', '1') != '0'
+
+
+def set_conv_line_stores(on):
+    global CONV_LINE_STORES
+    prev, CONV_LINE_STORES = CONV_LINE_STORES, bool(on)
+    return prev
+
+
+def set_et_image(on):
+    global ET_IMAGE
+    prev, ET_IMAGE = ET_IMAGE, bool(on)
+    return prev
 
 
 def use_planes(O):
@@ -315,7 +329,7 @@
     return out
 
 
-def group_conv_packed(x_words, layer, in_bound, gather, want_rowmax=False, lds_order=None):
+def group_conv_packed(x_words, layer, in_bound, gather, want_rowmax=False, lds_order=None, image=False, line_stores=None):
     ensure_tables()
     B, Cin, Lin = x_words.shape
     assert Cin == layer.Cin and x_words.dtype == torch.int32, (Cin, layer.Cin, x_words.dtype)
@@ -330,6 +344,15 @@
     w2, w_exp, _, _ = _conv_wsplit2(layer)
     out = torch.empty((B, layer.Cout, Lout), dtype=torch.float32, device=x_words.device)
     amax = torch.zeros(B, dtype=torch.float32, device=x_words.device) if want_rowmax else None
+    if line_stores is None:
+        line_stores = CONV_LINE_STORES and Lout == 13
+    if image or line_stores:
+        if image and (order_t is None or Lin != 48 or order_s > 48):
+            raise HipError('group_conv_packed: the image form needs the lds_order the image was written with (48 slots, stride <= 48)')
+        _check(lib().roreg_group_conv_f16x2_packed_ex(_ptr(x_words, torch.int32), _ptr(w2), w_exp, _ptr(layer.bias), _ptr(in_bound, torch.float32), _ptr(out),
+                                                      _ptr(amax), _ptr(gather, torch.int32), _ptr(order_t, torch.int32), order_s, B, Cin, layer.Cout, Lin, Lout,
+                                                      layer.KS, int(bool(image)), int(bool(line_stores)), _stream()), 'roreg_group_conv_f16x2_packed_ex')
+        return (out, amax) if want_rowmax else out
     _check(lib().roreg_group_conv_f16x2_packed(_ptr(x_words, torch.int32), _ptr(w2), w_exp, _ptr(layer.bias), _ptr(in_bound, torch.float32), _ptr(out),
                                                _ptr(amax), _ptr(gather, torch.int32), _ptr(order_t, torch.int32), order_s, B, Cin, layer.Cout, Lin, Lout,
                                                layer.KS, _stream()), 'roreg_group_conv_f16x2_packed')
diff --git a/roreg_amd/network/eqv_trans.py b/roreg_amd/network/eqv_trans.py
--- a/roreg_amd/network/eqv_trans.py
+++ b/roreg_amd/network/eqv_trans.py
@@ -148,9 +148,11 @@
                         bn_t, nb_t = self._trunk_bn()
                         T0, b1 = hip.irrep_gemm(X0, None, 128, 256, B, f16x2=layer.wsplit2, x_bound=b0, next_bound=nb_t, x_planes=hip.use_planes(256))
                         del X0
-                        hw, h0 = hip.ft_nonlin_packed(B, 256, T0, layer.bias, bn_t, b1, g_map=gmap, Lout=self.LIVE_PAD, Lvalid=45, raw_g=0)
+                        lo = self._trunk_lds_order()
+                        hw, h0 = hip.ft_nonlin_packed(B, 256, T0, layer.bias, bn_t, b1, g_map=gmap, Lout=self.LIVE_PAD, Lvalid=45, raw_g=0,
+                                                      image_order=lo if hip.ET_IMAGE else None)
                         del T0
-                        m, am = hip.group_conv_packed(hw, res._b_in.plan(), b1, gb, want_rowmax=True, lds_order=self._trunk_lds_order())
+                        m, am = hip.group_conv_packed(hw, res._b_in.plan(), b1, gb, want_rowmax=True, lds_order=lo, image=hip.ET_IMAGE)
                         t, at = hip.dense_split(m.view(B, -1), d_out, residual=h0, in_rowmax=am, want_rowmax=True)
                     else:
                         T0 = hip.irrep_gemm(X0, None, 128, 256, B, f16x2=layer.wsplit2, x_bound=b0, x_planes=hip.use_planes(256))
```

Measured after the change: 1107 (median of 6 runs). 1.01x the previous value.
